# Annatk26/wire

Hardware: AMD Instinct MI355X
Metric: coord-samples/sec fwd+bwd, 4x256 complex WIRE MLP (higher is better)
Workload: dtype f32 (2xfp16 split operands with power-of-two scales, f16 MFMA, fp32 accumulate)

## Files before the change

wire_amd/csrc/wire_api.hip:

```cpp
#include <cmath>
#include <cstdarg>
#include <cstdio>
#include <string>

#include "wire_plan.h"

static thread_local std::string g_err;
int fail(int code, const char* fmt, ...) {
  char buf[512];
  va_list ap;
  va_start(ap, fmt);
  vsnprintf(buf, sizeof buf, fmt, ap);
  va_end(ap);
  g_err = buf;
  return code;
}
int wire_fail_(int code, const char* msg) { return fail(code, "%s", msg); }

extern "C" int wire_abi_version(void) { return WIRE_ABI_VERSION; }
extern "C" const char* wire_last_error(void) { return g_err.c_str(); }

std::mutex g_prof_mu;
std::atomic<bool> g_prof_on{false};
std::vector<ProfRec> g_prof_recs;
// ... 329 lines not shown
  const float* A; float* Sx;
  float* gcur = nullptr; float* gnext = nullptr;
  int chain_rows = 0;

  const float* out_l(int l) const { return A + a.out0 + (int64_t)l * a.np * p.P; }
  const float* lin_l(int l) const { return l == 0 ? A + a.lin0 : A + a.lin1 + (int64_t)(l - 1) * a.np * p.Pl; }
  const float* first(int q) const { return packed + first_native_off(p, q); }
  unsigned* gslots(int l) const { return reinterpret_cast<unsigned*>(Sx + sc.gamax) + l * WIRE_AMAX_SLOTS; }
  const unsigned* oslots(int l) const { return reinterpret_cast<const unsigned*>(A + a.amax) + l * WIRE_AMAX_SLOTS; }
  float* grad(int t) const { return grads ? (float*)grads[t] : nullptr; }
  void done(int t, int count) const { if (ready) ready(user, t, count); }
  int64_t crp_set() const { return (int64_t)prereduce_room(colreduce_blocks(n)) * p.ldu * 5; }
  int final_stage();
  int first_point();
  int chain();
  int wgrad_batch();
  int layers();
  int coords_grad();
  int first_params();
  hipError_t hidden_tn(int l);
};

int Bwd::final_stage() {
  ProfScope ps(s, 3, 0);
  if (!r.fuse) {
    const float wL = (p.L == 0) ? p.w1 : p.w;
    if (p.L == 0 && p.cplx)
      HIPCHK(launch_final_bwd(s, p.kind, 1, g_y, n, p.O, packed + p.off_wf, nullptr, out_l(0), p.K, p.P, wL, p.s, gcur,
                              Sx + sc.fpw, Sx + sc.fpb));
    else
      for (int k = 0; k < p.S2; ++k) {
        const int64_t ro = (int64_t)k * n1, bo = (int64_t)k * final_bwd_blocks(n1);
        HIPCHK(launch_final_bwd(s, p.kind, 0, g_y + ro * p.O, n1, p.O, packed + p.off_wf, lin_l(p.L) + ro * p.Pl,
                                out_l(p.L) + ro * p.P, p.K, p.P, wL, pass_c(p, k), gcur + ro * p.P,
                                Sx + sc.fpw + bo * p.O * p.P, Sx + sc.fpb + bo * p.O,
                                r.fam == FAM_X2 ? gslots(p.L) : nullptr));
      }
    if (!grads) return WIRE_OK;
  }
  const int nbf = r.fused_final ? (int)((n + 127) / 128) : p.S2 * final_bwd_blocks(n1);
  HIPCHK(launch_final_reduce(s, p.kind, Sx + sc.fpw, Sx + sc.fpb, nbf, p.O, p.K, p.P, grad(p.ntens - 2),
                             grad(p.ntens - 1)));
  done(p.ntens - 2, 2);
  return WIRE_OK;
}

int Bwd::first_point() {
  ProfScope ps(s, 3, 0);
  if (p.kind == WIRE_KIND_WIRE)
    HIPCHK(launch_gabor_bwd_first_point(s, gcur, out_l(0), coords, p.D, first(0), first(1), n, p.K, p.P, p.w1, p.s,
                                        Sx + sc.gu, p.ldu));
  else
    HIPCHK(launch_gabor2d_bwd_first_point(s, gcur, out_l(0), coords, p.D, first(0), first(1), first(2), first(3), n, p.K,
                                          p.P, p.w1, p.s, Sx + sc.gu, p.ldu));
  return WIRE_OK;
}

int Bwd::chain() {
  const bool relu = p.kind == WIRE_KIND_RELU;
  FusedBwdParams bp;
  bp.n = n;
  bp.g = Sx + sc.gch; bp.g_stride = sc.gch_stride;
  bp.gamax = gslots(0);
  bp.aux = relu ? A + a.out0 : A + a.lin1 - a.np * p.Pl;
  bp.aux_stride = relu ? a.np * p.P : a.np * p.Pl;
  bp.wimg = reinterpret_cast<const unsigned char*>(packed + p.off_fxd);
  bp.wamax = wamax_of(p, packed, 1); bp.wamax_stride = WIRE_AMAX_SLOTS;
  bp.L = p.L; bp.w = p.w; bp.s = p.s;
  bp.rstore = r.rstore ? 1 : 0; bp.c_hidden = fused_pre_scale(p.kind, p.w, p.s);
  bp.aux0 = relu ? A + a.out0 : A + a.lin0;
  bp.w1 = p.w1;
  if (!p.first_gemm) { bp.coords = coords; bp.D = p.D; bp.crp = Sx + sc.crp; bp.C = p.K; }
  if (p.m2) {
    bp.n = n1;
    for (int k = 0; k < p.S2; ++k) {
      const int64_t ro = (int64_t)k * n1;
      FusedBwdParams b = bp;
      b.g = bp.g + ro * p.P; b.aux = bp.aux + ro * p.P; b.aux0 = bp.aux0 + ro * p.P;
      b.s = pass_c(p, k); b.c_hidden = fused_pre_scale(p.kind, p.w, pass_c(p, k));
      if (k > 0) b.crp = bp.crp + (int64_t)k * ((n1 + chain_rows - 1) / chain_rows) * p.K * 5;
      ProfScope ps(s, 1, 2.0 * n1 * p.Pl * p.P * p.L);
      HIPCHK(launch_fused_bwd(s, p.kind, p.P, b, &chain_rows));
    }
    return WIRE_OK;
  }
  ProfScope ps(s, 1, 2.0 * n * p.Pl * p.P * p.L);
  HIPCHK(launch_fused_bwd(s, p.kind, p.P, bp, &chain_rows));
  return WIRE_OK;
}

static int rstore_zmode(int kind) { return kind == WIRE_KIND_SIREN ? 2 : kind == WIRE_KIND_GAUSS ? 3 : 4; }

int Bwd::wgrad_batch() {
  const int l0 = r.wb_l0, nb = r.wb_n;
  const bool rs = r.rstore;
  const float s_z = rs ? 0.f : r.out_scale[l0 - 1];
  ProfScope ps(s, 2, 2.0 * n * p.Pl * p.P * nb);
  HIPCHK(launch_gemmx2_tn(s, Sx + sc.gch + l0 * sc.gch_stride, p.Pl, rs ? lin_l(l0 - 1) : out_l(l0 - 1), rs ? p.Pl : p.P,
                          n, p.Pl, p.P, r.wb_S, Sx + sc.slab, Sx + sc.bslab, gslots(l0), oslots(l0 - 1),
                          rs ? 1.f / 16384.f : (s_z != 0.f ? 1.f / s_z : 0.f), rs ? rstore_zmode(p.kind) : 0,
                          nb, sc.gch_stride, rs ? a.np * p.Pl : a.np * p.P, WIRE_AMAX_SLOTS));
  return WIRE_OK;
}

hipError_t Bwd::hidden_tn(int l) {
  const int S = r.tn_S;
  float* slab = Sx + sc.slab;
  float* bslab = Sx + sc.bslab;
  switch (r.tn_fam) {
    case FAM_3M: return launch_gemm3m_tn(s, gcur, p.P, out_l(l - 1), p.P, n, p.Kp, p.Kp, S, slab, bslab);
    case FAM_X2:
      if (r.rstore)
        return launch_gemmx2_tn(s, gcur, p.Pl, lin_l(l - 1), p.Pl, n, p.Pl, p.P, S, slab, bslab, gslots(l), nullptr,
                                1.f / 16384.f, rstore_zmode(p.kind));
      return launch_gemmx2_tn(s, gcur, p.Pl, out_l(l - 1), p.P, n, p.Pl, p.P, S, slab, bslab, gslots(l), oslots(l - 1),
                              r.out_scale[l - 1] != 0.f ? 1.f / r.out_scale[l - 1] : 0.f);
    case FAM_X3: return launch_gemmx3_tn(s, gcur, p.Pl, out_l(l - 1), p.P, n, p.Pl, p.P, S, slab, bslab);
    default: return launch_gemm_tn(s, gcur, p.Pl, out_l(l - 1), p.P, n, p.Pl, p.P, S, slab, bslab);
  }
}

int Bwd::layers() {
  const int pl = p.per_layer;
  for (int l = p.L; l >= 1; --l) {
    if (r.chain) gcur = Sx + sc.gch + (int64_t)l * sc.gch_stride;
    if (grads) {
      const bool own = l < r.wb_l0;
      if (own) {
        ProfScope ps(s, 2, 2.0 * n * p.Pl * p.P);
        HIPCHK(hidden_tn(l));
      }
      const int S = own ? r.tn_S : r.wb_S;
      const int64_t m = own ? 0 : l - r.wb_l0;
      float* const slab = Sx + sc.slab + m * S * p.Pl * p.P;
      float* const bslab = Sx + sc.bslab + m * S * p.Pl;
      auto g = [&](int q) { return q < pl ? grad(p.t0 + pl * l + q) : nullptr; };
      ProfScope ps(s, 3, 0);
      if (r.tn_fam == FAM_3M)
        HIPCHK(launch_wgrad3m_reduce(s, slab, bslab, S, p.K, p.K, p.Kp, p.Kp, g(0), g(1)));
      else
        HIPCHK(launch_wgrad_reduce(s, p.kind, slab, bslab, S, p.K, p.K, p.Pl, p.P, g(0), g(1), g(2), g(3)));
      done(p.t0 + pl * l, pl);
    }
    if (r.chain) continue;
    const bool first_sums = grads && r.first_sums;
    GemmEpiParams ep;
    ep.scale = p.s; ep.kvalid = p.K; ep.ld1 = p.P; ep.i1 = out_l(l - 1);
    int epi;
    if (l > 1 || !p.cplx) {
      epi = epi_bwd(p.kind);
      ep.omega = (l - 1 == 0) ? p.w1 : p.w;
      ep.i0 = lin_l(l - 1); ep.o0 = gnext; ep.ld0 = p.Pl;
      ep.recompute_out = r.recompute_out && l >= 2;
      if (l == 1 && first_sums) { ep.coords = coords; ep.D = p.D; ep.cr_partial = Sx + sc.crp; ep.cr_C = p.K; }
    } else {
      epi = (p.kind == WIRE_KIND_WIRE) ? EPI_GABOR_BWD_FIRST : EPI_GABOR2D_BWD_FIRST;
      ep.omega = p.w1;
      ep.coords = coords; ep.D = p.D; ep.ldu = p.ldu; ep.o0 = Sx + sc.gu;
      if (first_sums) { ep.cr_partial = Sx + sc.crp; ep.cr_C = p.K; ep.cr_set = crp_set(); }
      ep.recompute_out = r.recompute_out0;
      ep.W0 = first(0); ep.b0 = first(1);
      if (pl == 4) { ep.W0b = first(2); ep.b0b = first(3); }
    }
    if (!p.cplx && l == 1) ep.ld0 = p.P;
    if (l == 1 && g_coords && r.cg_epi) {
      ep.cg_partial = Sx + cl.cgp; ep.D = p.D;
      if (!p.cplx) ep.W0 = first(0);
    }
    for (int k = 0; k < p.S2; ++k) {
      const int64_t ro = (int64_t)k * n1;
      GemmEpiParams e = ep;
      if (k > 0) { e.scale = pass_c(p, k); e.i0 += ro * p.Pl; e.i1 += ro * p.P; e.o0 += ro * e.ld0; }
      ProfScope ps(s, 1, 2.0 * n1 * p.Pl * p.P);
      HIPCHK(layer_nt(s, p, r.fam, packed, l, true, epi, gcur + ro * p.Pl, n1, e, gslots(l), wamax_of(p, packed, l),
                      l >= 2 || r.tn0 == FAM_X2 ? gslots(l - 1) : nullptr));
    }
    float* t = gcur; gcur = gnext; gnext = t;
  }
  return WIRE_OK;
}

int Bwd::coords_grad() {
  if (!g_coords) return WIRE_OK;
  const float* gu = Sx + sc.gu;
  if (r.cg_epi) {
    HIPCHK(launch_coordgrad_reduce(s, Sx + cl.cgp, cl.ntiles, n, p.D, g_coords));
  } else if (p.kind == WIRE_KIND_WIRE) {
    HIPCHK(launch_coordgrad_rows(s, gu, p.ldu, nullptr, first(0), nullptr, p.K, p.D, n, g_coords));
  } else if (p.kind == WIRE_KIND_WIRE2D) {
    HIPCHK(launch_coordgrad_rows(s, gu, 2 * p.ldu, gu + p.ldu, first(0), first(2), p.K, p.D, n, g_coords));
  } else if (p.m2) {
    HIPCHK(launch_coordgrad_rows(s, gcur, p.P, nullptr, first(0), nullptr, p.K, p.D, n, Sx + cl.cgp));
    HIPCHK(launch_m2_sum_passes(s, Sx + cl.cgp, p.S2, n1, p.D, g_coords));
  } else if (!p.first_gemm) {
    HIPCHK(launch_coordgrad_rows(s, gcur, p.P, nullptr, first(0), nullptr, p.K, p.D, n, g_coords));
  } else {
    GemmEpiParams ep;
    ep.o0 = Sx + cl.gpe; ep.ld0 = p.Pin0;
    HIPCHK(layer_nt(s, p, FAM_4M, packed, 0, true, EPI_STORE, gcur, n, ep));
    HIPCHK(launch_posenc_bwd(s, coords, n, p.D, p.F, Sx + cl.gpe, p.Pin0, g_coords));
  }
  return WIRE_OK;
}

int Bwd::first_params() {
  if (!grads) return WIRE_OK;
  float* const crp = Sx + sc.crp;
  if (p.cplx) {
    const float* gu = Sx + sc.gu;
    if (r.first_sums) {
      HIPCHK(launch_colreduce_final(s, p.K, p.D, n, crp, grad(0), grad(1)));
      if (p.kind == WIRE_KIND_WIRE2D) HIPCHK(launch_colreduce_final(s, p.K, p.D, n, crp + crp_set(), grad(2), grad(3)));
    } else if (p.kind == WIRE_KIND_WIRE) {
      HIPCHK(launch_colreduce(s, gu, p.ldu, p.K, coords, p.D, n, crp, grad(0), grad(1)));
    } else {
      HIPCHK(launch_colreduce(s, gu, 2 * p.ldu, p.K, coords, p.D, n, crp, grad(0), grad(1)));
      HIPCHK(launch_colreduce(s, gu + p.ldu, 2 * p.ldu, p.K, coords, p.D, n, crp, grad(2), grad(3)));
    }
  } else if (!p.first_gemm && r.chain) {
    HIPCHK(launch_colreduce_final_blocks(s, p.K, p.D, p.S2 * (int)((n1 + chain_rows - 1) / chain_rows), crp, grad(p.t0),
                                         grad(p.t0 + 1)));
  } else if (!p.first_gemm && r.first_sums) {
    HIPCHK(launch_colreduce_final(s, p.K, p.D, n, crp, grad(0), grad(1)));
  } else if (!p.first_gemm) {
    HIPCHK(launch_colreduce(s, gcur, p.P, p.K, coords, p.D, n, crp, grad(p.t0), grad(p.t0 + 1)));
  } else if (r.tn0 == FAM_X2) {
    const int S = gemmx2_tn_splits(n, p.P, p.Pin0, sc.S);
    HIPCHK(launch_gemmx2_tn(s, gcur, p.P, A + a.pe, p.Pin0, n, p.P, p.Pin0, S, Sx + sc.slab, Sx + sc.bslab, gslots(0),
                            nullptr, 1.f / r.pe_split));
    HIPCHK(launch_wgrad_reduce(s, p.kind, Sx + sc.slab, Sx + sc.bslab, S, p.K, p.Din, p.P, p.Pin0, grad(p.t0),
                               grad(p.t0 + 1), nullptr, nullptr));
  } else {
    const float* g0 = r.chain ? Sx + sc.gch : gcur;
    const bool x3 = r.tn0 == FAM_X3;
    const int S = x3 ? gemmx3_tn_splits(n, p.P, p.Pin0, sc.S) : gemm_tn_splits(n, p.P, p.Pin0, sc.S);
    HIPCHK(x3 ? launch_gemmx3_tn(s, g0, p.P, A + a.pe, p.Pin0, n, p.P, p.Pin0, S, Sx + sc.slab, Sx + sc.bslab)
              : launch_gemm_tn(s, g0, p.P, A + a.pe, p.Pin0, n, p.P, p.Pin0, S, Sx + sc.slab, Sx + sc.bslab));
    HIPCHK(launch_wgrad_reduce(s, p.kind, Sx + sc.slab, Sx + sc.bslab, S, p.K, p.Din, p.P, p.Pin0, grad(p.t0),
                               grad(p.t0 + 1), nullptr, nullptr));
  }
  done(p.t0, p.per_layer);
  if (p.ms) done(0, 2);
  return WIRE_OK;
}
}

static int mlp_bwd_core(void* stream, const Plan& p, const Route& r, const float* packed, const float* coords, int64_t n,
                        const float* g_y, const void* act, int64_t act_bytes, void* scratch, int64_t scratch_bytes,
                        void* const* grads, wire_grad_ready_fn ready = nullptr, void* user = nullptr,
                        float* g_coords = nullptr, bool comb_done = false) {
  if (n <= 0) return fail(WIRE_ERR_ARG, "backward needs n > 0");
  if (!packed || !coords || (!r.fuse && !g_y && !comb_done) || !act || !scratch || (!grads && !g_coords))
    return fail(WIRE_ERR_ARG, "null pointer");
  if (grads)
    for (int i = p.ms ? p.t0 : 0; i < p.ntens; ++i) if (!grads[i]) return fail(WIRE_ERR_ARG, "grads[%d] is null", i);
  if (p.ms && g_coords) return fail(WIRE_ERR_ARG, "no coordinate gradient through the frozen first stage of kind %d",
                                    (int)WIRE_KIND_BSPLINE_MS);
  Bwd c{p, r, (hipStream_t)stream, packed, coords, n * p.S2, n, g_y, grads, g_coords, ready, user, act_layout(p, n, 1),
        scratch_layout(p, n), coord_layout(p, n), (const float*)act, (float*)scratch};
  const int64_t need = g_coords ? c.cl.total : c.sc.total;
  if (act_bytes < c.a.total * 4) return fail(WIRE_ERR_SIZE, "act buffer too small");
  if (scratch_bytes < need * 4) return fail(WIRE_ERR_SIZE, "scratch %lld < %lld bytes",
                                            (long long)scratch_bytes, (long long)need * 4);
  c.gcur = c.Sx + c.sc.ga;
  c.gnext = c.Sx + c.sc.gb;
  if (p.m2) {
    ProfScope ps(c.s, 3, 0);
    float* const part = c.Sx + c.sc.cpart;
    if (!comb_done)
      HIPCHK(launch_m2_comb_bwd(c.s, comb_of(p, packed), p.S2, p.O, c.A + c.a.ytr, n, M2Loss{}, g_y, c.Sx + c.sc.gtr,
                                grads ? part : nullptr, nullptr));
    if (r.chain) c.gcur = c.Sx + c.sc.gch + (int64_t)p.L * c.sc.gch_stride;
    if (grads) {
      HIPCHK(launch_m2_comb_reduce(c.s, part, n, p.S2, p.O,
                                   M2Grads{c.grad(0), c.grad(1), c.grad(2), c.grad(3)}));
      c.done(0, 4);
      for (int k = 0; k < p.S2 && !r.chain; ++k)
        HIPCHK(hipMemcpyAsync(c.Sx + c.sc.crep + (int64_t)k * n * p.D, coords, (size_t)n * p.D * sizeof(float),
                              hipMemcpyDeviceToDevice, c.s));
      if (!r.chain) c.coords = c.Sx + c.sc.crep;
    }
    c.g_y = c.Sx + c.sc.gtr;
  }
  if (r.fam == FAM_X2 && !r.fuse)
    HIPCHK(hipMemsetAsync(c.gslots(0), 0, (size_t)(p.L + 2) * WIRE_AMAX_SLOTS * sizeof(unsigned), c.s));
  int rc = c.final_stage();
  if (!rc && p.L == 0 && p.cplx) rc = c.first_point();
  if (!rc && r.chain) rc = c.chain();
  if (!rc && r.wb_n > 0) rc = c.wgrad_batch();
  if (!rc) rc = c.layers();
  if (rc) return rc;
  ProfScope ps(c.s, 3, 0);
  rc = c.coords_grad();
  return rc ? rc : c.first_params();
}

extern "C" int wire_mlp_bwd(void* stream, const wire_net_desc* d, const float* packed,
                            const float* coords, int64_t n, const float* g_y, const void* act,
                            int64_t act_bytes, void* scratch, int64_t scratch_bytes,
                            void* const* grads) {
  Plan p; if (int rc = make_plan(d, p)) return rc;
  if (!grads) return fail(WIRE_ERR_ARG, "null pointer");
  if (p.hier)
    return hier_bwd_core(stream, p, hier_route(p, n, MODE_AUTOGRAD), packed, coords, n, g_y, act, act_bytes, scratch,
                         scratch_bytes, grads, nullptr, nullptr, nullptr);
  if (p.mfn)
    return mfn_bwd_core(stream, p, mfn_route(p, n, MODE_AUTOGRAD), packed, coords, n, g_y, act, act_bytes, scratch,
                        scratch_bytes, grads, nullptr, nullptr, nullptr);
  return mlp_bwd_core(stream, p, make_route(p, n, MODE_AUTOGRAD), packed, coords, n, g_y, act, act_bytes, scratch,
                      scratch_bytes, grads);
}

extern "C" int wire_mlp_bwd_coords(void* stream, const wire_net_desc* d, const float* packed, const float* coords,
// ... 110 lines not shown
```

wire_amd/csrc/wire_gemm.h:

```cpp
#pragma once
#include <hip/hip_runtime.h>
#include <stdint.h>

#include "wire_knobs.h"

enum WireFamily { FAM_4M = 0, FAM_3M = 1, FAM_X3 = 2, FAM_X2 = 3 };
WireFamily wire_family_(int kind);

enum WireEpi {
  EPI_STORE = 0,
  EPI_GABOR_FWD = 1,
  EPI_GABOR_BWD = 2,
  EPI_GABOR_BWD_FIRST = 3,
  EPI_SIREN_FWD = 4, EPI_GAUSS_FWD = 5, EPI_RELU_FWD = 6,
  EPI_SIREN_BWD = 7, EPI_GAUSS_BWD = 8, EPI_RELU_BWD = 9,
  EPI_GABOR2D_FWD = 10,
  EPI_GABOR2D_BWD = 11,
  EPI_GABOR2D_BWD_FIRST = 12,
  EPI_BSPLINE_FWD = 13,
  EPI_BSPLINE_BWD = 14,
  EPI_MFN_FWD = 15,
  EPI_MFN_BWD = 16,
  EPI_CG = 64
};

constexpr bool epi_real_fwd(int e) {
  return e == EPI_SIREN_FWD || e == EPI_GAUSS_FWD || e == EPI_RELU_FWD || e == EPI_BSPLINE_FWD;
}
constexpr bool epi_real_bwd(int e) {
  return e == EPI_SIREN_BWD || e == EPI_GAUSS_BWD || e == EPI_RELU_BWD || e == EPI_BSPLINE_BWD;
}
constexpr int epi_real_act(int e) {
  return (e == EPI_BSPLINE_FWD || e == EPI_BSPLINE_BWD) ? 3 : epi_real_fwd(e) ? e - EPI_SIREN_FWD : e - EPI_SIREN_BWD;
}

struct GemmEpiParams {
  const float* bias = nullptr;
  float* o0 = nullptr;
  float* o1 = nullptr;
  const float* i0 = nullptr;
  const float* i1 = nullptr;
  int ld0 = 0;
  int ld1 = 0;
  float omega = 0.f, scale = 0.f;
  int kvalid = 0;
  const float* coords = nullptr;
  const float* W0 = nullptr;
  const float* b0 = nullptr;
  const float* W0b = nullptr;
  const float* b0b = nullptr;
  int D = 0;
  int ldu = 0;
  int wide = 0;
  float* cr_partial = nullptr;
  int cr_C = 0;
  int64_t cr_set = 0;
  float* cg_partial = nullptr;
  int recompute_out = 0;
  int stagger = 0, stagger_lo = 0, stagger_hi = 0;
  const unsigned* amax_a = nullptr;
  const unsigned* amax_b = nullptr;
  unsigned* amax_out = nullptr;
  float o1_split = 0.f;
  float a_split_inv = 0.f;
  const float* ftab = nullptr;
#ifdef WIRE_ABLATE
  int ablate = 0;
#endif
};

hipError_t launch_gemm_nt(hipStream_t s, int epi, const float* A, int lda, const float* Bt,
                          int ldb, int64_t M, int Nc, int Kd, const GemmEpiParams& ep);

int gemm_tn_splits(int64_t n, int Pm, int Pn, int max_splits);
hipError_t launch_gemm_tn(hipStream_t s, const float* G, int ldg, const float* Z, int ldz,
                          int64_t n, int Pm, int Pn, int splits, float* slab, float* bslab);

hipError_t launch_gemm3m_nt(hipStream_t s, int epi, const float* A, int lda, const float* B, int ldb,
                            int64_t M, int Kp_out, int Kp_in, const GemmEpiParams& ep);
int gemm3m_tn_splits(int64_t n, int Kp_o, int Kp_i, int max_splits);
hipError_t launch_gemm3m_tn(hipStream_t s, const float* G, int ldg, const float* Z, int ldz, int64_t n,
                            int Kp_o, int Kp_i, int splits, float* slab, float* bslab);

int64_t gemmx3_b_image_floats(int Nc, int Kd);
hipError_t launch_x3_split_b(hipStream_t s, const float* Bt, int ldb, int Nc, int Kd, void* Bx3);
#define X3_SPLIT_MAXB 32
struct X3SplitBatch { const float* src[X3_SPLIT_MAXB]; void* dst[X3_SPLIT_MAXB]; };
hipError_t launch_x3_split_b_batch(hipStream_t s, const X3SplitBatch& sb, int nb, int ldb, int Nc, int Kd);
hipError_t launch_gemmx3_nt(hipStream_t s, int epi, const float* A, int lda, const void* Bx3, int64_t M,
                            int Nc, int Kd, const GemmEpiParams& ep);
bool gemmx3_nt_is_h16(int epi, int64_t M);
int gemmx3_tn_splits(int64_t n, int Pm, int Pn, int max_splits);
int gemmx3_tn_splits_max(int64_t n, int Pm, int Pn, int max_splits);
hipError_t launch_gemmx3_tn(hipStream_t s, const float* G, int ldg, const float* Z, int ldz, int64_t n,
                            int Pm, int Pn, int splits, float* slab, float* bslab);

void gemmx3_register_glds(bool (*handles)(int, int64_t),
                          hipError_t (*launch)(hipStream_t, int, const float*, int, const void*, int64_t, int, int,
                                               const GemmEpiParams&),
                          int (*tune)(const char*, int));
extern int (*g_glds_tune)(const char*, int);
bool gemmx3g_handles(int epi, int64_t M);
int gemmx3g_tune_set(const char* key, int value);
int gemmx3g_mode();
hipError_t launch_gemmx3g_nt(hipStream_t s, int epi, const float* A, int lda, const void* Bx3, int64_t M,
                             int Nc, int Kd, const GemmEpiParams& ep);

bool gemmx3h_handles(int epi, int64_t M);
hipError_t launch_gemmx3h_nt(hipStream_t s, int epi, const float* A, int lda, const void* Bx3, int64_t M,
                             int Nc, int Kd, const GemmEpiParams& ep);

#define X2_AMAX_MAXB 32
struct X2AmaxBatch { const float* src[X2_AMAX_MAXB]; unsigned* slots[X2_AMAX_MAXB]; };
hipError_t launch_amax_batch(hipStream_t s, const X2AmaxBatch& ab, int nb, int64_t count);
hipError_t launch_amax(hipStream_t s, const float* src, int64_t count, unsigned* slots);
int64_t gemmx2_b_image_floats(int Nc, int Kd);
#define X2_SPLIT_MAXB 32
struct X2SplitBatch { const float* src[X2_SPLIT_MAXB]; void* dst[X2_SPLIT_MAXB]; const unsigned* slots[X2_SPLIT_MAXB]; };
hipError_t launch_x2_split_b_batch(hipStream_t s, const X2SplitBatch& sb, int nb, int ldb, int Nc, int Kd);
hipError_t launch_gemmx2h_nt(hipStream_t s, int epi, const float* A, int lda, const void* Bx2, int64_t M, int Nc,
                             int Kd, const GemmEpiParams& ep);
bool gemmx2_tn_applies(int Pm, int Pn);
int gemmx2_tn_splits(int64_t n, int Pm, int Pn, int max_splits);
hipError_t launch_gemmx2_tn(hipStream_t s, const float* G, int ldg, const float* Z, int ldz, int64_t n, int Pm,
                            int Pn, int splits, float* slab, float* bslab, const unsigned* amax_g,
                            const unsigned* amax_z, float z_pre_inv = 0.f, int z_act = 0, int batch = 1,
                            long long g_step = 0, long long z_step = 0, int amax_step = 0);
int gemmx2_tn_batch_splits(int64_t n, int Pm, int Pn, int max_splits, int batch);

#define FX_SPLIT_MAXB 32
struct FxSplitBatch { const float* src[FX_SPLIT_MAXB]; void* dst[FX_SPLIT_MAXB]; const unsigned* slots[FX_SPLIT_MAXB]; };
int64_t fused_b_image_floats(int P);
hipError_t launch_fx_split_b_batch(hipStream_t s, const FxSplitBatch& sb, int nb, int ldb, int P, float c, int Kd = 0);
struct FusedFwdParams {
  const float* coords = nullptr; long long n = 0;
  const float* W0 = nullptr; const float* b0 = nullptr;
  const unsigned char* wimg = nullptr;
  const float* bias = nullptr; long long bias_stride = 0;
  const unsigned* wamax = nullptr; int wamax_stride = 0;
  const float* wf = nullptr; const float* bfr = nullptr;
  float* y = nullptr;
  int D = 0, K = 0, L = 0, O = 0;
  float w1 = 0.f, w = 0.f, s = 0.f;
  float c_first = 1.f, c_hidden = 1.f, k2_first = 0.f, k2 = 0.f;
  float* lin0 = nullptr;
  float* lin = nullptr; long long lin_stride = 0;
  float* out = nullptr; long long out_stride = 0;
  unsigned* amax_out = nullptr;
  float inv_c_first = 1.f, inv_c_hidden = 1.f;
  int pe_F = 0; const float* bias0 = nullptr; const unsigned* wamax0 = nullptr;
  int rstore = 0;
  const float* target = nullptr; const int64_t* idx = nullptr; long long first = 0; float gscale = 0.f;
  float* rec = nullptr;
  float* g_lin = nullptr;
  float* part_w = nullptr; float* part_b = nullptr;
  float* loss_partial = nullptr;
  unsigned* amax_g = nullptr;
};
float fused_pre_scale(int kind, float omega0, float scale0);
bool fused_fwd_shape(int kind, int P);
hipError_t launch_fused_fwd(hipStream_t s, int kind, int P, const FusedFwdParams& fp);

struct FusedBwdParams {
  long long n = 0;
  float* g = nullptr; long long g_stride = 0;
  unsigned* gamax = nullptr;
  const float* aux = nullptr; long long aux_stride = 0;
  const float* aux0 = nullptr;
  const unsigned char* wimg = nullptr;
  const unsigned* wamax = nullptr; int wamax_stride = 0;
  int L = 0;
  float w = 0.f, s = 0.f;
  int rstore = 0; float c_hidden = 1.f;
  float w1 = 0.f;
  const float* coords = nullptr; int D = 0;
  float* crp = nullptr; int C = 0;
};
bool fused_bwd_shape(int kind, int P);
hipError_t launch_fused_bwd(hipStream_t s, int kind, int P, const FusedBwdParams& fp, int* tile_rows);
```

wire_amd/csrc/wire_gemmh_epi.h:

```cpp
#pragma once
#include "wire_dev.h"
#include "wire_gemm.h"

WIRE_DEVINL void h_pair_rows(const f32x4& X, const f32x4& Y, f32x4& Xp, f32x4& Yp) {
#pragma unroll
  for (int q = 0; q < 4; ++q) {
    const int x = __float_as_int(X[q]), y = __float_as_int(Y[q]);
    Xp[q] = __int_as_float(__builtin_amdgcn_update_dpp(x, y, 0x128, 0xf, 0xc, false));
    Yp[q] = __int_as_float(__builtin_amdgcn_update_dpp(y, x, 0x128, 0xf, 0x3, false));
  }
}

WIRE_DEVINL void h_amax4(float& m, const f32x4& v) {
  m = __builtin_fmaxf(m, __builtin_fmaxf(__builtin_fmaxf(__builtin_fabsf(v[0]), __builtin_fabsf(v[1])),
                                         __builtin_fmaxf(__builtin_fabsf(v[2]), __builtin_fabsf(v[3]))));
}

WIRE_DEVINL void h_cg_add(float (&cg)[4], const float (&t)[4], const int e, const int lane) {
#pragma unroll
  for (int d = 0; d < 4; ++d) {
    float v = t[d];
    v += __shfl_xor(v, 8); v += __shfl_xor(v, 16); v += __shfl_xor(v, 32);
    cg[d] += (lane >> 3) == e ? v : 0.f;
  }
}
template <int NRB>
WIRE_DEVINL void h_cg_store(const float (&cg)[4], const GemmEpiParams& ep, const int M, const int m_w, const int n_w,
                            const int lane) {
  const int j = lane >> 3;
  if (j >= 2 * NRB) return;
  const int row = m_w + 16 * (j >> 1) + 8 * (j & 1) + (lane & 7);
  if (row >= M) return;
  float* dst = ep.cg_partial + ((size_t)(n_w >> 7) * (size_t)M + (size_t)row) * ep.D;
  for (int d = 0; d < ep.D; ++d) dst[d] = cg[d];
}

template <int EPIX, bool X2 = false, int NRB = 4>
WIRE_DEVINL void h_epilogue(f32x4 (&acc)[NRB][8], const GemmEpiParams& ep, const int M, const int m_w, const int n_w,
                            const int Nc, const int lane, unsigned char* lds, const int wave, const int rt,
                            const float acc_scale = 1.f) {
  constexpr int EPI = EPIX & ~EPI_CG;
  constexpr bool CG = (EPIX & EPI_CG) != 0;
  const int rr = lane & 7, ch = (lane >> 3) & 1, g = lane >> 4;
  float amx = 0.f;
  if constexpr (X2) {
#pragma unroll
    for (int i = 0; i < NRB; ++i)
#pragma unroll
      for (int j = 0; j < 8; ++j)
#pragma unroll
        for (int q = 0; q < 4; ++q) acc[i][j][q] *= acc_scale;
  }
  const int cq = 16 * ch + 4 * g;
  if constexpr (EPI == EPI_STORE) {
#pragma unroll
    for (int sp = 0; sp < 4; ++sp) {
      const int col = n_w + 32 * sp + cq;
      if (n_w + 32 * sp >= Nc) continue;
#pragma unroll
      for (int rb = 0; rb < NRB; ++rb) {
        f32x4 xp, yp;
        h_pair_rows(acc[rb][2 * sp], acc[rb][2 * sp + 1], xp, yp);
        const int row = m_w + 16 * rb + rr;
        if (row < M) *reinterpret_cast<f32x4*>(ep.o0 + (size_t)row * ep.ld0 + col) = xp;
        if (row + 8 < M) *reinterpret_cast<f32x4*>(ep.o0 + (size_t)(row + 8) * ep.ld0 + col) = yp;
      }
    }
  } else if constexpr (epi_real_fwd(EPI)) {
    constexpr int ACT = epi_real_act(EPI);
#pragma unroll
    for (int sp = 0; sp < 4; ++sp) {
      if (n_w + 32 * sp >= Nc) continue;
      const int col = n_w + 32 * sp + cq;
      const f32x4 bv = *reinterpret_cast<const f32x4*>(ep.bias + col);
#pragma unroll
      for (int rb = 0; rb < NRB; ++rb) {
        f32x4 a2[2];
        h_pair_rows(acc[rb][2 * sp], acc[rb][2 * sp + 1], a2[0], a2[1]);
#pragma unroll
        for (int hr = 0; hr < 2; ++hr) {
          const int row = m_w + 16 * rb + 8 * hr + rr;
          f32x4 lin;
#pragma unroll
          for (int q = 0; q < 4; ++q) lin[q] = a2[hr][q] + bv[q];
          if (ep.o0 && row < M) *reinterpret_cast<f32x4*>(ep.o0 + (size_t)row * ep.ld0 + col) = lin;
          if (ep.o1) {
            f32x4 o;
#pragma unroll
            for (int q = 0; q < 4; ++q) {
              const float v = real_act_fwd_lean<ACT>(lin[q], ep.omega, ep.scale);
              o[q] = col + q < ep.kvalid ? v : 0.f;
            }
            if constexpr (X2) h_amax4(amx, o);
            if (row < M) wire_store_out4(ep.o1 + (size_t)row * ep.ld1 + col, o, X2 ? ep.o1_split : 0.f);
          }
        }
      }
    }
  } else if constexpr (epi_real_bwd(EPI)) {
    constexpr int ACT = epi_real_act(EPI);
    float cg[4] = {0.f, 0.f, 0.f, 0.f};
#pragma unroll
    for (int sp = 0; sp < 4; ++sp) {
      if (n_w + 32 * sp >= Nc) continue;
      const int col = n_w + 32 * sp + cq;
      float crs[4][5];
#pragma unroll
      for (int q = 0; q < 4; ++q)
#pragma unroll
        for (int d = 0; d < 5; ++d) crs[q][d] = 0.f;
#pragma unroll
      for (int rp = 0; rp < NRB; rp += 2) {
        f32x4 lv[4], ov[4], a2[4];
#pragma unroll
        for (int r2 = 0; r2 < 2; ++r2) {
          h_pair_rows(acc[rp + r2][2 * sp], acc[rp + r2][2 * sp + 1], a2[2 * r2], a2[2 * r2 + 1]);
#pragma unroll
          for (int hr = 0; hr < 2; ++hr) {
            int row = m_w + 16 * (rp + r2) + 8 * hr + rr;
            row = row < M ? row : M - 1;
            lv[2 * r2 + hr] = (ACT != ACT_RELU) ? *reinterpret_cast<const f32x4*>(ep.i0 + (size_t)row * ep.ld0 + col)
                                                : f32x4{0.f, 0.f, 0.f, 0.f};
            const bool load_out = ACT == ACT_RELU || (ACT == ACT_GAUSS && !ep.recompute_out);
            ov[2 * r2 + hr] = load_out ? *reinterpret_cast<const f32x4*>(ep.i1 + (size_t)row * ep.ld1 + col)
                                       : f32x4{0.f, 0.f, 0.f, 0.f};
          }
        }
        if (ACT == ACT_GAUSS && ep.recompute_out) {
#pragma unroll
          for (int e = 0; e < 4; ++e)
#pragma unroll
            for (int q = 0; q < 4; ++q) {
              const float v = real_act_fwd_lean<ACT>(lv[e][q], ep.omega, ep.scale);
              ov[e][q] = col + q < ep.kvalid ? v : 0.f;
            }
        }
#pragma unroll
        for (int e = 0; e < 4; ++e) {
          const int row = m_w + 16 * (rp + (e >> 1)) + 8 * (e & 1) + rr;
          f32x4 gl;
#pragma unroll
          for (int q = 0; q < 4; ++q) gl[q] = real_act_bwd_lean<ACT>(a2[e][q], lv[e][q], ov[e][q], ep.omega, ep.scale);
          if constexpr (X2) h_amax4(amx, gl);
          if constexpr (CG) {
            float t[4] = {0.f, 0.f, 0.f, 0.f};
            if (row < M) {
#pragma unroll
              for (int q = 0; q < 4; ++q) {
                if (col + q >= ep.kvalid) continue;
                for (int d = 0; d < ep.D; ++d) t[d] = __builtin_fmaf(gl[q], ep.W0[(col + q) * ep.D + d], t[d]);
              }
            }
            h_cg_add(cg, t, 2 * (rp + (e >> 1)) + (e & 1), lane);
          }
          if (row < M) {
            if (ep.cr_partial) {
              float x[4] = {0.f, 0.f, 0.f, 0.f};
              for (int d = 0; d < ep.D; ++d) x[d] = ep.coords[(size_t)row * ep.D + d];
#pragma unroll
              for (int q = 0; q < 4; ++q) {
#pragma unroll
                for (int d = 0; d < 4; ++d) crs[q][d] = __builtin_fmaf(gl[q], x[d], crs[q][d]);
                crs[q][4] += gl[q];
              }
            } else {
              *reinterpret_cast<f32x4*>(ep.o0 + (size_t)row * ep.ld0 + col) = gl;
            }
          }
        }
      }
      if (ep.cr_partial) {
        float* red = reinterpret_cast<float*>(lds);
#pragma unroll
        for (int q = 0; q < 4; ++q)
#pragma unroll
          for (int d = 0; d < 5; ++d) {
            float v = crs[q][d];
            v += __shfl_xor(v, 1); v += __shfl_xor(v, 2); v += __shfl_xor(v, 4);
            if (rr == 0) red[(wave * 128 + 32 * sp + cq + q) * 5 + d] = v;
          }
      }
    }
    if (ep.cr_partial) {
      __syncthreads();
      const float* red = reinterpret_cast<const float*>(lds);
      for (int e = threadIdx.x; e < 128 * 5; e += 256) {
        const int c = e / 5, d = e - 5 * c;
        const float v = (red[e] + red[128 * 5 + e]) + (red[2 * 128 * 5 + e] + red[3 * 128 * 5 + e]);
        if (n_w + c < ep.cr_C) ep.cr_partial[((size_t)rt * ep.cr_C + n_w + c) * 5 + d] = v;
      }
    }
    if constexpr (CG) h_cg_store<NRB>(cg, ep, M, m_w, n_w, lane);
  } else if constexpr (EPI == EPI_MFN_FWD || EPI == EPI_MFN_BWD) {
#pragma unroll 1
    for (int sp = 0; sp < 4; ++sp) {
      if (n_w + 32 * sp >= Nc) continue;
      const int col = n_w + 32 * sp + cq;
      const bool filt = EPI == EPI_MFN_FWD || ep.i0 != nullptr;
      MfnCol fc[4];
      f32x4 bv = {0.f, 0.f, 0.f, 0.f};
      if (filt) {
#pragma unroll
        for (int q = 0; q < 4; ++q) fc[q] = mfn_load(ep.ftab, col + q);
      }
      if constexpr (EPI == EPI_MFN_FWD) bv = *reinterpret_cast<const f32x4*>(ep.bias + col);
#pragma unroll
      for (int rb = 0; rb < NRB; ++rb) {
        f32x4 a2[2];
        f32x4 ax = acc[rb][0], ay = acc[rb][1];
        if (sp == 1) { ax = acc[rb][2]; ay = acc[rb][3]; }
        if (sp == 2) { ax = acc[rb][4]; ay = acc[rb][5]; }
        if (sp == 3) { ax = acc[rb][6]; ay = acc[rb][7]; }
        h_pair_rows(ax, ay, a2[0], a2[1]);
#pragma unroll
        for (int hr = 0; hr < 2; ++hr) {
          const int row = m_w + 16 * rb + 8 * hr + rr;
          const int rowc = row < M ? row : M - 1;
          float x[4] = {0.f, 0.f, 0.f, 0.f};
          f32x4 g = {0.f, 0.f, 0.f, 0.f};
          if (filt) {
            mfn_load_x(ep.coords, rowc, ep.D, x);
#pragma unroll
            for (int q = 0; q < 4; ++q) g[q] = mfn_g(fc[q], x);
          }
          if constexpr (EPI == EPI_MFN_FWD) {
            f32x4 lin, o;
#pragma unroll
            for (int q = 0; q < 4; ++q) {
              lin[q] = a2[hr][q] + bv[q];
              o[q] = col + q < ep.kvalid ? lin[q] * g[q] : 0.f;
            }
            if constexpr (X2) h_amax4(amx, o);
            if (row < M) {
              if (ep.o0) *reinterpret_cast<f32x4*>(ep.o0 + (size_t)row * ep.ld0 + col) = lin;
              *reinterpret_cast<f32x4*>(ep.o1 + (size_t)row * ep.ld1 + col) = o;
            }
          } else {
            if (filt) {
              const f32x4 lin = *reinterpret_cast<const f32x4*>(ep.i0 + (size_t)rowc * ep.ld0 + col);
              f32x4 gl, hh;
#pragma unroll
              for (int q = 0; q < 4; ++q) { gl[q] = a2[hr][q] * g[q]; hh[q] = a2[hr][q] * lin[q]; }
              if constexpr (X2) h_amax4(amx, gl);
              if (row < M) {
                *reinterpret_cast<f32x4*>(ep.o0 + (size_t)row * ep.ld0 + col) = gl;
                *reinterpret_cast<f32x4*>(ep.o1 + (size_t)row * ep.ld1 + col) = hh;
              }
            } else if (row < M) {
              *reinterpret_cast<f32x4*>(ep.o1 + (size_t)row * ep.ld1 + col) = a2[hr];
            }
          }
        }
      }
    }
  } else if constexpr (EPI == EPI_GABOR2D_FWD) {
    const int grp = n_w >> 7;
    const int f0 = (grp << 5) + cq;
    const int oc = (grp << 6) + cq;
    f32x4 bv[4];
#pragma unroll
    for (int k = 0; k < 4; ++k) bv[k] = *reinterpret_cast<const f32x4*>(ep.bias + n_w + 32 * k + cq);
#pragma unroll
    for (int rb = 0; rb < NRB; ++rb) {
      f32x4 part[4][2];
#pragma unroll
      for (int k = 0; k < 4; ++k) h_pair_rows(acc[rb][2 * k], acc[rb][2 * k + 1], part[k][0], part[k][1]);
#pragma unroll
      for (int hr = 0; hr < 2; ++hr) {
        const int row = m_w + 16 * rb + 8 * hr + rr;
        f32x4 u, v, pp, qq;
#pragma unroll
        for (int q = 0; q < 4; ++q) {
          u[q] = part[0][hr][q] + bv[0][q];
          v[q] = part[1][hr][q] + bv[1][q];
          pp[q] = part[2][hr][q] + bv[2][q];
          qq[q] = part[3][hr][q] + bv[3][q];
        }
        if (ep.o0 && row < M) {
          float* Lp = ep.o0 + (size_t)row * ep.ld0 + n_w + cq;
          *reinterpret_cast<f32x4*>(Lp) = u;
          *reinterpret_cast<f32x4*>(Lp + 32) = v;
          *reinterpret_cast<f32x4*>(Lp + 64) = pp;
          *reinterpret_cast<f32x4*>(Lp + 96) = qq;
        }
        if (ep.o1) {
          f32x4 o_re, o_im;
#pragma unroll
          for (int q = 0; q < 4; ++q) {
            float a, b;
            gabor2d_fwd_lean(u[q], v[q], pp[q], qq[q], ep.omega, ep.scale, a, b);
            const bool valid = f0 + q < ep.kvalid;
            o_re[q] = valid ? a : 0.f;
            o_im[q] = valid ? b : 0.f;
          }
          if constexpr (X2) { h_amax4(amx, o_re); h_amax4(amx, o_im); }
          if (row < M) {
            float* Op = ep.o1 + (size_t)row * ep.ld1 + oc;
            wire_store_out4(Op, o_re, X2 ? ep.o1_split : 0.f);
            wire_store_out4(Op + 32, o_im, X2 ? ep.o1_split : 0.f);
          }
        }
      }
    }
  } else if constexpr (EPI == EPI_GABOR2D_BWD || EPI == EPI_GABOR2D_BWD_FIRST) {
    const float m2s2 = -2.f * ep.scale * ep.scale, w0 = ep.omega;
    float cg[4] = {0.f, 0.f, 0.f, 0.f};
#pragma unroll
    for (int G = 0; G < 2; ++G) {
      if (n_w + 64 * G >= Nc) continue;
      const int c0 = n_w + 64 * G + cq;
      const int grp = c0 >> 6;
      const int f0 = (grp << 5) + (c0 & 31);
      const int lc = (grp << 7) + (c0 & 31);
      float w[4][4], wv[4][4], bb[4], bv2[4];
      float cru[4][5], crp2[4][5];
#pragma unroll
      for (int q = 0; q < 4; ++q)
#pragma unroll
        for (int d = 0; d < 5; ++d) { cru[q][d] = 0.f; crp2[q][d] = 0.f; }
      if constexpr (EPI == EPI_GABOR2D_BWD_FIRST) {
#pragma unroll
        for (int q = 0; q < 4; ++q) {
          const bool valid = f0 + q < ep.kvalid;
          bb[q] = valid ? ep.b0[f0 + q] : 0.f;
          bv2[q] = valid ? ep.b0b[f0 + q] : 0.f;
#pragma unroll
          for (int d = 0; d < 4; ++d) {
            w[q][d] = (valid && d < ep.D) ? ep.W0[(f0 + q) * ep.D + d] : 0.f;
            wv[q][d] = (valid && d < ep.D) ? ep.W0b[(f0 + q) * ep.D + d] : 0.f;
          }
        }
      }
#pragma unroll
      for (int rb = 0; rb < NRB; ++rb) {
        f32x4 are[2], aim[2];
        h_pair_rows(acc[rb][4 * G], acc[rb][4 * G + 1], are[0], are[1]);
        h_pair_rows(acc[rb][4 * G + 2], acc[rb][4 * G + 3], aim[0], aim[1]);
        f32x4 u[2], v[2], pp[2], qq[2], pr[2], pi[2];
        float xs[2][4];
#pragma unroll
        for (int hr = 0; hr < 2; ++hr) {
          int row = m_w + 16 * rb + 8 * hr + rr;
          row = row < M ? row : M - 1;
          const bool recompute = EPI == EPI_GABOR2D_BWD && ep.recompute_out != 0;
          if (!recompute) {
            const float* Op = ep.i1 + (size_t)row * ep.ld1 + c0;
            pr[hr] = *reinterpret_cast<const f32x4*>(Op);
            pi[hr] = *reinterpret_cast<const f32x4*>(Op + 32);
          }
          if constexpr (EPI == EPI_GABOR2D_BWD) {
            const float* Lp = ep.i0 + (size_t)row * ep.ld0 + lc;
            u[hr] = *reinterpret_cast<const f32x4*>(Lp);
            v[hr] = *reinterpret_cast<const f32x4*>(Lp + 32);
            pp[hr] = *reinterpret_cast<const f32x4*>(Lp + 64);
            qq[hr] = *reinterpret_cast<const f32x4*>(Lp + 96);
            if (recompute) {
#pragma unroll
              for (int q = 0; q < 4; ++q) {
                float a, b;
                gabor2d_fwd_lean(u[hr][q], v[hr][q], pp[hr][q], qq[hr][q], ep.omega, ep.scale, a, b);
                const bool valid = f0 + q < ep.kvalid;
                pr[hr][q] = valid ? a : 0.f;
                pi[hr][q] = valid ? b : 0.f;
              }
            }
          } else {
            float x[4] = {0.f, 0.f, 0.f, 0.f};
            for (int d = 0; d < ep.D; ++d) x[d] = ep.coords[(size_t)row * ep.D + d];
#pragma unroll
            for (int d = 0; d < 4; ++d) xs[hr][d] = x[d];
#pragma unroll
            for (int q = 0; q < 4; ++q) {
              float uu = bb[q], p2 = bv2[q];
#pragma unroll
              for (int d = 0; d < 4; ++d) { uu = __builtin_fmaf(x[d], w[q][d], uu); p2 = __builtin_fmaf(x[d], wv[q][d], p2); }
              u[hr][q] = uu; pp[hr][q] = p2; v[hr][q] = 0.f; qq[hr][q] = 0.f;
            }
          }
        }
#pragma unroll
        for (int hr = 0; hr < 2; ++hr) {
          const int row = m_w + 16 * rb + 8 * hr + rr;
          f32x4 g0, g1, g2, g3;
#pragma unroll
          for (int q = 0; q < 4; ++q) {
            const float gr = are[hr][q], gi = aim[hr][q];
            const float c_r = __builtin_fmaf(pr[hr][q], gr, pi[hr][q] * gi);
            const float c_i = __builtin_fmaf(pr[hr][q], gi, -(pi[hr][q] * gr));
            const float tt = m2s2 * c_r;
            g0[q] = __builtin_fmaf(tt, u[hr][q], w0 * c_i);
            g1[q] = __builtin_fmaf(tt, v[hr][q], -(w0 * c_r));
            g2[q] = tt * pp[hr][q];
            g3[q] = tt * qq[hr][q];
          }
          if constexpr (X2 && EPI == EPI_GABOR2D_BWD) { h_amax4(amx, g0); h_amax4(amx, g1); h_amax4(amx, g2); h_amax4(amx, g3); }
          if constexpr (EPI == EPI_GABOR2D_BWD_FIRST) {
            if constexpr (CG) {
              float t[4] = {0.f, 0.f, 0.f, 0.f};
              if (row < M) {
#pragma unroll
                for (int q = 0; q < 4; ++q)
#pragma unroll
                  for (int d = 0; d < 4; ++d) t[d] = __builtin_fmaf(g2[q], wv[q][d], __builtin_fmaf(g0[q], w[q][d], t[d]));
              }
              h_cg_add(cg, t, 2 * rb + hr, lane);
            }
          }
          if (row < M) {
            if constexpr (EPI == EPI_GABOR2D_BWD) {
              float* Gp = ep.o0 + (size_t)row * ep.ld0 + lc;
              *reinterpret_cast<f32x4*>(Gp) = g0;
              *reinterpret_cast<f32x4*>(Gp + 32) = g1;
              *reinterpret_cast<f32x4*>(Gp + 64) = g2;
              *reinterpret_cast<f32x4*>(Gp + 96) = g3;
            } else {
#pragma unroll
              for (int q = 0; q < 4; ++q)
                if (!(f0 + q < ep.kvalid)) { g0[q] = 0.f; g2[q] = 0.f; }
              if (ep.cr_partial) {
#pragma unroll
                for (int q = 0; q < 4; ++q) {
#pragma unroll
                  for (int d = 0; d < 4; ++d) {
                    cru[q][d] = __builtin_fmaf(g0[q], xs[hr][d], cru[q][d]);
                    crp2[q][d] = __builtin_fmaf(g2[q], xs[hr][d], crp2[q][d]);
                  }
                  cru[q][4] += g0[q];
                  crp2[q][4] += g2[q];
                }
              } else {
                float* Gp = ep.o0 + (size_t)row * (2 * ep.ldu);
                *reinterpret_cast<f32x4*>(Gp + f0) = g0;
                *reinterpret_cast<f32x4*>(Gp + ep.ldu + f0) = g2;
              }
            }
          }
        }
      }
      if constexpr (EPI == EPI_GABOR2D_BWD_FIRST) {
        if (ep.cr_partial) {
          float* red = reinterpret_cast<float*>(lds);
#pragma unroll
          for (int q = 0; q < 4; ++q)
#pragma unroll
            for (int d = 0; d < 5; ++d) {
              float a = cru[q][d], b = crp2[q][d];
              a += __shfl_xor(a, 1); a += __shfl_xor(a, 2); a += __shfl_xor(a, 4);
              b += __shfl_xor(b, 1); b += __shfl_xor(b, 2); b += __shfl_xor(b, 4);
              if (rr == 0) {
                red[(wave * 64 + 32 * G + cq + q) * 5 + d] = a;
                red[4 * 64 * 5 + (wave * 64 + 32 * G + cq + q) * 5 + d] = b;
              }
            }
        }
      }
    }
// ... 224 lines not shown
```

wire_amd/csrc/wire_gemmx2h.hip:

```cpp
#include <cstdlib>
#include <atomic>
#include <cstring>

#include "wire_dev.h"
#include "wire_gemm.h"
#include "wire_gemmh_epi.h"

typedef _Float16 f16x8 __attribute__((ext_vector_type(8)));
typedef _Float16 f16x2 __attribute__((ext_vector_type(2)));
typedef unsigned x2u32x4 __attribute__((ext_vector_type(4)));
typedef unsigned x2u32x2 __attribute__((ext_vector_type(2)));

#define X2_BK 32
#define X2_TBM 256
#define X2_TBN 128
#define X2_AWAVE (64 * 128)
#define X2_ABYTES (4 * X2_AWAVE)
#define X2_BPLANE (X2_TBN * 64)
#define X2_BSTAGE (2 * X2_BPLANE)

#define X2_MFMA(a, b, c) c = __builtin_amdgcn_mfma_f32_16x16x32_f16(a, b, c, 0, 0, 0)

WIRE_DEVINL void x2_dma16(const void* gsrc, unsigned char* lds_piece) {
#ifdef WIRE_X2_DMA_BUILTIN
// ... 188 lines not shown
        x2_split2(ar[rb][0][0], ar[rb][0][1], s_a, H[0], L[0]);
        x2_split2(ar[rb][0][2], ar[rb][0][3], s_a, H[1], L[1]);
        x2_split2(ar[rb][1][0], ar[rb][1][1], s_a, H[2], L[2]);
        x2_split2(ar[rb][1][2], ar[rb][1][3], s_a, H[3], L[3]);
        ah[rb] = __builtin_bit_cast(f16x8, x2u32x4{H[0], H[1], H[2], H[3]});
        al[rb] = __builtin_bit_cast(f16x8, x2u32x4{L[0], L[1], L[2], L[3]});
      }
      __builtin_amdgcn_sched_barrier(0);
      const bool more = kt + 2 < nk;
      if (more) { issue(kt + 2, (kt + 2) % 3); aload_to(ar, kt + 2); }
      __builtin_amdgcn_sched_barrier(0);
      const unsigned char* S = smem + b_rd + (kt % 3) * X2_BSTAGE;
#pragma unroll
      for (int hb = 0; hb < 2; ++hb) {
        if (hb == 1 && half_tile) break;
        f16x8 bh[4], bl[4];
#pragma unroll
        for (int cq = 0; cq < 4; ++cq) {
          bh[cq] = *reinterpret_cast<const f16x8*>(S + (4 * hb + cq) * 1024);
          bl[cq] = *reinterpret_cast<const f16x8*>(S + X2_BPLANE + (4 * hb + cq) * 1024);
        }
#pragma unroll
        for (int rb = 0; rb < NRB; ++rb)
#pragma unroll
          for (int cq = 0; cq < 4; ++cq) {
            X2_MFMA(bl[cq], ah[rb], acc[rb][4 * hb + cq]);
            X2_MFMA(bh[cq], al[rb], acc[rb][4 * hb + cq]);
            X2_MFMA(bh[cq], ah[rb], acc[rb][4 * hb + cq]);
          }
      }
      __builtin_amdgcn_sched_barrier(0);
      if (more) asm volatile("s_waitcnt vmcnt(8)" ::: "memory");
      else asm volatile("s_waitcnt vmcnt(0)" ::: "memory");
      __builtin_amdgcn_s_barrier();
      __builtin_amdgcn_sched_barrier(0);
    };
    static_assert(2 * NRB + 4 == 8, "the in-flight count of the end-of-stage wait");
    issue(0, 0); aload_to(araw, 0);
    issue(1, 1); aload_to(ar1, 1);
    asm volatile("s_waitcnt vmcnt(8)" ::: "memory");
    __builtin_amdgcn_s_barrier();
    for (int kt = 0; kt < nk; kt += 2) {
      half_stage(araw, kt);
      half_stage(ar1, kt + 1);
    }
    h_epilogue<EPI, true, NRB>(acc, ep, M, m_base + wave * (16 * NRB), n_base, Nc, lane, smem, wave, rt, inv_a * inv_b);
    return;
  }

  issue(0, 0);
  if constexpr (BRING) { if (nk > 1) issue(1, 1); }
  if constexpr (AMODE == 1) aload(0);
  asm volatile("s_waitcnt vmcnt(0)" ::: "memory");
  __builtin_amdgcn_s_barrier();

  int buf = 0;
  for (int kt = 0; kt < nk; ++kt) {
    if constexpr (AMODE == 0 || AMODE == 2) {
#pragma unroll
      for (int rb = 0; rb < NRB; ++rb) {
        if constexpr (AMODE == 2) {
          araw[rb][0] = *reinterpret_cast<const f32x4*>(smem + a2_rd0 + rb * 2048);
          araw[rb][1] = *reinterpret_cast<const f32x4*>(smem + a2_rd1 + rb * 2048);
        } else {
          araw[rb][0] = *reinterpret_cast<const f32x4*>(smem + a_rd + rb * 2048);
          araw[rb][1] = *reinterpret_cast<const f32x4*>(smem + a_rd + rb * 2048 + 256);
        }
      }
      asm volatile("s_waitcnt lgkmcnt(0)" ::: "memory");
      __builtin_amdgcn_sched_barrier(0);
      if (kt + 1 < nk) issue(kt + 1, buf ^ 1);
      __builtin_amdgcn_sched_barrier(0);
    }
    f16x8 ah[NRB], al[NRB];
#pragma unroll
    for (int rb = 0; rb < NRB; ++rb) {
      if constexpr (APRE) {
        const x2u32x4 u0 = __builtin_bit_cast(x2u32x4, araw[rb][0]), u1 = __builtin_bit_cast(x2u32x4, araw[rb][1]);
        ah[rb] = __builtin_bit_cast(f16x8, x2u32x4{u0[0], u0[1], u1[0], u1[1]});
        al[rb] = __builtin_bit_cast(f16x8, x2u32x4{u0[2], u0[3], u1[2], u1[3]});
      } else {
        unsigned H[4], L[4];
        x2_split2(araw[rb][0][0], araw[rb][0][1], s_a, H[0], L[0]);
        x2_split2(araw[rb][0][2], araw[rb][0][3], s_a, H[1], L[1]);
        x2_split2(araw[rb][1][0], araw[rb][1][1], s_a, H[2], L[2]);
        x2_split2(araw[rb][1][2], araw[rb][1][3], s_a, H[3], L[3]);
        ah[rb] = __builtin_bit_cast(f16x8, x2u32x4{H[0], H[1], H[2], H[3]});
        al[rb] = __builtin_bit_cast(f16x8, x2u32x4{L[0], L[1], L[2], L[3]});
      }
    }
    if constexpr (AMODE == 1) {
      __builtin_amdgcn_sched_barrier(0);
      if constexpr (BRING) {
        if (kt + 1 < nk) aload(kt + 1);
        __builtin_amdgcn_sched_barrier(0);
        if (kt + 2 < nk) issue(kt + 2, buf == 0 ? 2 : buf - 1);
      } else
      if (kt + 1 < nk) { issue(kt + 1, buf ^ 1); aload(kt + 1); }
      __builtin_amdgcn_sched_barrier(0);
    }
    const unsigned char* S = smem + b_rd + buf * X2_BSTAGE;
#pragma unroll
    for (int hb = 0; hb < 2; ++hb) {
      if (hb == 1 && half_tile) break;
      f16x8 bh[4], bl[4];
#pragma unroll
      for (int cq = 0; cq < 4; ++cq) {
        bh[cq] = *reinterpret_cast<const f16x8*>(S + (4 * hb + cq) * 1024);
        bl[cq] = *reinterpret_cast<const f16x8*>(S + X2_BPLANE + (4 * hb + cq) * 1024);
      }
#pragma unroll
      for (int rb = 0; rb < NRB; ++rb)
#pragma unroll
        for (int cq = 0; cq < 4; ++cq) {
          X2_MFMA(bl[cq], ah[rb], acc[rb][4 * hb + cq]);
          X2_MFMA(bh[cq], al[rb], acc[rb][4 * hb + cq]);
          X2_MFMA(bh[cq], ah[rb], acc[rb][4 * hb + cq]);
        }
    }
    __builtin_amdgcn_sched_barrier(0);
    {
    if (BRING && kt + 2 < nk) asm volatile("s_waitcnt vmcnt(4)" ::: "memory");
    else asm volatile("s_waitcnt vmcnt(0)" ::: "memory");
    __builtin_amdgcn_s_barrier();
    }
    __builtin_amdgcn_sched_barrier(0);
    if constexpr (BRING) buf = buf == 2 ? 0 : buf + 1; else buf ^= 1;
  }
  h_epilogue<EPI, true, NRB>(acc, ep, M, m_base + wave * (16 * NRB), n_base, Nc, lane, smem, wave, rt, inv_a * inv_b);
}

template <int EPI>
static hipError_t launchx2h_t(hipStream_t s, const float* A, int lda, const unsigned short* Bx2, int64_t M, int Nc,
                              int Kd, const GemmEpiParams& ep) {
  const int tbm = X2_TBM;
  const int tiles_m = (int)((M + tbm - 1) / tbm);
  const int tiles_n = (Nc + X2_TBN - 1) / X2_TBN;
  const int tiles_m_pad = (tiles_m + 7) & ~7;
  const dim3 grid((unsigned)(tiles_m_pad * tiles_n));
  if (ep.a_split_inv != 0.f) {
    if constexpr (EPI == EPI_STORE || EPI == EPI_GABOR_FWD || EPI == EPI_GABOR2D_FWD || EPI == EPI_SIREN_FWD ||
                  EPI == EPI_GAUSS_FWD || EPI == EPI_BSPLINE_FWD) {
      if (knob(K_X2_AMODE) == 2)
        hipLaunchKernelGGL((gemmx2h_nt_kernel<EPI, 2, 4, 1, true>), grid, dim3(256), 0, s, A, lda, Bx2, (int)M, Nc, Kd, tiles_m,
                           tiles_n, ep);
      else
        hipLaunchKernelGGL((gemmx2h_nt_kernel<EPI, 1, 4, 1, true>), grid, dim3(256), 0, s, A, lda, Bx2, (int)M, Nc, Kd, tiles_m,
                           tiles_n, ep);
      return hipGetLastError();
    } else {
      return hipErrorInvalidValue;
    }
  }
  if (knob(K_X2_AMODE) == 2)
    hipLaunchKernelGGL((gemmx2h_nt_kernel<EPI, 2, 4>), grid, dim3(256), 0, s, A, lda, Bx2, (int)M, Nc, Kd, tiles_m, tiles_n, ep);
  else if (knob(K_X2_AMODE) == 1)
    hipLaunchKernelGGL((gemmx2h_nt_kernel<EPI, 1, 4>), grid, dim3(256), 0, s, A, lda, Bx2, (int)M, Nc, Kd, tiles_m, tiles_n, ep);
  else
    hipLaunchKernelGGL((gemmx2h_nt_kernel<EPI, 0, 4>), grid, dim3(256), 0, s, A, lda, Bx2, (int)M, Nc, Kd, tiles_m, tiles_n, ep);
  return hipGetLastError();
}

hipError_t launch_gemmx2h_nt(hipStream_t s, int epi, const float* A, int lda, const void* Bx2v, int64_t M, int Nc,
                             int Kd, const GemmEpiParams& ep) {
  if (M <= 0) return hipSuccess;
  if ((Nc & 63) || (Kd & 31) || (lda & 3) || M > 0x7fffff00LL || (!ep.amax_a && ep.a_split_inv == 0.f) || !ep.amax_b)
    return hipErrorInvalidValue;
  if ((int64_t)lda * 4 * X2_TBM > 0x7fffffffLL) return hipErrorInvalidValue;
  const unsigned short* Bx2 = (const unsigned short*)Bx2v;
  switch (epi) {
    case EPI_STORE: return launchx2h_t<EPI_STORE>(s, A, lda, Bx2, M, Nc, Kd, ep);
    case EPI_GABOR_FWD: return launchx2h_t<EPI_GABOR_FWD>(s, A, lda, Bx2, M, Nc, Kd, ep);
    case EPI_GABOR_BWD: return launchx2h_t<EPI_GABOR_BWD>(s, A, lda, Bx2, M, Nc, Kd, ep);
    case EPI_GABOR_BWD_FIRST:
      return ep.cg_partial ? launchx2h_t<EPI_GABOR_BWD_FIRST | EPI_CG>(s, A, lda, Bx2, M, Nc, Kd, ep)
                           : launchx2h_t<EPI_GABOR_BWD_FIRST>(s, A, lda, Bx2, M, Nc, Kd, ep);
    case EPI_SIREN_FWD: return launchx2h_t<EPI_SIREN_FWD>(s, A, lda, Bx2, M, Nc, Kd, ep);
    case EPI_GAUSS_FWD: return launchx2h_t<EPI_GAUSS_FWD>(s, A, lda, Bx2, M, Nc, Kd, ep);
    case EPI_RELU_FWD: return launchx2h_t<EPI_RELU_FWD>(s, A, lda, Bx2, M, Nc, Kd, ep);
    case EPI_SIREN_BWD:
      return ep.cg_partial ? launchx2h_t<EPI_SIREN_BWD | EPI_CG>(s, A, lda, Bx2, M, Nc, Kd, ep)
                           : launchx2h_t<EPI_SIREN_BWD>(s, A, lda, Bx2, M, Nc, Kd, ep);
    case EPI_GAUSS_BWD:
      return ep.cg_partial ? launchx2h_t<EPI_GAUSS_BWD | EPI_CG>(s, A, lda, Bx2, M, Nc, Kd, ep)
                           : launchx2h_t<EPI_GAUSS_BWD>(s, A, lda, Bx2, M, Nc, Kd, ep);
    case EPI_RELU_BWD:
      return ep.cg_partial ? launchx2h_t<EPI_RELU_BWD | EPI_CG>(s, A, lda, Bx2, M, Nc, Kd, ep)
                           : launchx2h_t<EPI_RELU_BWD>(s, A, lda, Bx2, M, Nc, Kd, ep);
    case EPI_BSPLINE_FWD: return launchx2h_t<EPI_BSPLINE_FWD>(s, A, lda, Bx2, M, Nc, Kd, ep);
    case EPI_BSPLINE_BWD:
      return ep.cg_partial ? launchx2h_t<EPI_BSPLINE_BWD | EPI_CG>(s, A, lda, Bx2, M, Nc, Kd, ep)
                           : launchx2h_t<EPI_BSPLINE_BWD>(s, A, lda, Bx2, M, Nc, Kd, ep);
    case EPI_MFN_FWD: return launchx2h_t<EPI_MFN_FWD>(s, A, lda, Bx2, M, Nc, Kd, ep);
    case EPI_MFN_BWD: return launchx2h_t<EPI_MFN_BWD>(s, A, lda, Bx2, M, Nc, Kd, ep);
    case EPI_GABOR2D_FWD:
      if (Nc & 127) return hipErrorInvalidValue;
      return launchx2h_t<EPI_GABOR2D_FWD>(s, A, lda, Bx2, M, Nc, Kd, ep);
    case EPI_GABOR2D_BWD: return launchx2h_t<EPI_GABOR2D_BWD>(s, A, lda, Bx2, M, Nc, Kd, ep);
    case EPI_GABOR2D_BWD_FIRST:
      return ep.cg_partial ? launchx2h_t<EPI_GABOR2D_BWD_FIRST | EPI_CG>(s, A, lda, Bx2, M, Nc, Kd, ep)
                           : launchx2h_t<EPI_GABOR2D_BWD_FIRST>(s, A, lda, Bx2, M, Nc, Kd, ep);
    default: return hipErrorInvalidValue;
  }
}

typedef short x2s16x4 __attribute__((ext_vector_type(4)));
#define X2T_TK 32

WIRE_DEVINL x2s16x4 x2_lds_tr16(const unsigned char* p) {
  return __builtin_amdgcn_ds_read_tr16_b64_v4i16(
      (x2s16x4 __attribute__((address_space(3)))*)(const_cast<unsigned char*>(p)));
}

template <int WM, int WN, int ZMODE, int RB = 4>
__global__ __launch_bounds__(64 * WM * WN, 2) void gemmx2_tn16_kernel(
    const float* __restrict__ G, int ldg, const float* __restrict__ Z, int ldz, long long n, int Pm, int Pn,
    int tiles_n, int nsplit, long long chunk, float* __restrict__ slab, float* __restrict__ bslab, int tiles,
    const unsigned* __restrict__ amax_g, const unsigned* __restrict__ amax_z, const float z_pre_inv,
    const long long g_step, const long long z_step, const int amax_step) {
  {
    const int by = blockIdx.y;
    G += (size_t)by * g_step; Z += (size_t)by * z_step;
    slab += (size_t)by * nsplit * Pm * Pn;
    if (bslab) bslab += (size_t)by * nsplit * Pm;
    amax_g += by * amax_step;
    if (amax_z) amax_z += by * amax_step;
  }
  constexpr int NW = WM * WN;
  constexpr int TM = 16 * RB * WM, TN = 128 * WN;
  constexpr bool G3 = RB == 3;
  static_assert(RB == 4 || (RB == 3 && WM == 8 && WN == 1), "wave tiles: 64 x 128, or 48 x 128 in the 8-wave P = 384 shape");
  constexpr int GPLANE = X2T_TK * TM * 2, ZPLANE = X2T_TK * TN * 2;
  constexpr int STAGE = 2 * GPLANE + 2 * ZPLANE;
  constexpr int UG = TM / 8, UZ = 16 * WN;
  constexpr int IG = (UG + NW - 1) / NW, IZ = (UZ + NW - 1) / NW;
  constexpr int PG = TM / 32, PZ = TN / 32;
  extern __shared__ __attribute__((aligned(16))) unsigned char smem_t[];
  const int tid = threadIdx.x;
  const int lane = tid & 63, wave = tid >> 6;
  const int wave_m = wave / WN, wave_n = wave % WN;
  const int bb = blockIdx.x;
  const int xcd = bb & 7, idx = bb >> 3;
  const int tile = idx % tiles;
  const int split = (idx / tiles) * 8 + xcd;
  if (split >= nsplit) return;
  const int tm = tile / tiles_n, tn = tile % tiles_n;
  const int m_base = tm * TM, n_base = tn * TN;
  const long long row0 = (long long)split * chunk;
  long long row1 = row0 + chunk;
  if (row1 > n) row1 = n;
  if (row1 <= row0) return;

  float s_g, inv_g, s_z, inv_z;
  wire_x2_scales(wire_amax_read(amax_g, lane), s_g, inv_g);
  constexpr bool ZPRE = ZMODE == 1;
  if constexpr (ZMODE >= 1) { s_z = 1.f / z_pre_inv; inv_z = z_pre_inv; }
  else wire_x2_scales(wire_amax_read(amax_z, lane), s_z, inv_z);

  const int l_hb = lane >> 5, l_rs = (lane >> 2) & 7, l_p = lane & 3;
  const int l_row0 = (l_rs & 3) + 8 * (l_rs >> 2);
  auto pass_row = [](const int t) { return 16 * (t & 1) + 4 * (t >> 1); };
  const int l_feat = 16 * l_hb + 4 * l_p;
  const int l_st = l_hb * 1024 + l_rs * 32 + l_p * 8;
  const bool do_bias = (bslab != nullptr) && (tn == 0);
  const bool z_edge = WN == 1 && n_base + TN > Pn;

  f32x4 acc[RB][8];
#pragma unroll
  for (int i = 0; i < RB; ++i)
#pragma unroll
    for (int j = 0; j < 8; ++j) acc[i][j] = f32x4{0.f, 0.f, 0.f, 0.f};
  static_assert(G3 || (PG % NW == 0 && IG == 4 * (PG / NW)), "the block pairs of G must deal out evenly to the waves");
  static_assert(!G3 || (PG == 12 && IG == 6), "8 waves x 6 units = 12 block pairs x 4 passes");
  static_assert(PZ == NW || PZ == 4, "Z units: one block pair per wave, or 4 block pairs dealt round-robin");
  constexpr int NB = G3 ? 3 : PG / NW;
  const int hiw = wave >= 4 ? 1 : 0;
  const int g3_pb = hiw ? wave - 4 : wave + 8;
  auto g3_pair = [&](const int i) { return (i % 3) == 0 ? wave : ((i % 3) == 1 ? g3_pb : wave + 4); };
  auto g3_row = [&](const int i) { return (i % 3) == 1 ? 16 * hiw + (i >= 3 ? 4 : 0) : (i == 0 ? 0 : i == 2 ? 16 : i == 3 ? 4 : 20); };
  auto g3_pass = [&](const int i) { return (i % 3) == 1 ? hiw + (i >= 3 ? 2 : 0) : (i == 0 ? 0 : i == 2 ? 1 : i == 3 ? 2 : 3); };
  constexpr bool ZFIX = (PZ == NW);
  f32x4 bsum[NB];
#pragma unroll
  for (int i = 0; i < NB; ++i) bsum[i] = f32x4{0.f, 0.f, 0.f, 0.f};

  const int nrows = (int)(row1 - row0);
  const int nk = (nrows + X2T_TK - 1) / X2T_TK;
  const int nk_full = nrows / X2T_TK;
  const f32x4 zero4 = {0.f, 0.f, 0.f, 0.f};

  struct Staged { f32x4 g[IG], z[IZ]; };
  Staged st;
  const unsigned g_off = (unsigned)l_row0 * (unsigned)ldg + (unsigned)(m_base + l_feat);
  const unsigned z_off = (unsigned)l_row0 * (unsigned)ldz + (unsigned)(n_base + l_feat);
  const float* const g_base = G + (size_t)row0 * ldg;
  const float* const z_base = Z + (size_t)row0 * ldz;
  auto gload = [&](Staged& R, int kt, const bool tail) {
    int ks = tail ? nk_full : (kt < nk_full ? kt : nk_full - 1);
    ks = ks < 0 ? 0 : ks;
    const float* gb = g_base + (size_t)ks * (X2T_TK * (size_t)ldg);
    const float* zb = z_base + (size_t)ks * (X2T_TK * (size_t)ldz);
    const int rbase = ks * X2T_TK + l_row0;
#pragma unroll
    for (int i = 0; i < IG; ++i) {
      if constexpr (G3) {
        const int fp = g3_pair(i), pr = g3_row(i);
        const bool ok = !tail || rbase + pr < nrows;
        R.g[i] = ok ? *reinterpret_cast<const f32x4*>(gb + (size_t)pr * ldg + 32 * fp + g_off) : zero4;
      } else {
        const int fp = wave + NW * (i % NB), t = i / NB;
        const bool ok = !tail || rbase + pass_row(t) < nrows;
        R.g[i] = ok ? *reinterpret_cast<const f32x4*>(gb + (size_t)pass_row(t) * ldg + 32 * fp + g_off) : zero4;
      }
    }
#pragma unroll
    for (int i = 0; i < IZ; ++i) {
      const int u = wave + NW * i;
      if (ZFIX || u < UZ) {
        const int fp = ZFIX ? wave : (u & 3), t = ZFIX ? i : (u >> 2);
        bool ok = !tail || rbase + pass_row(t) < nrows;
        if (z_edge) ok = ok && (n_base + 32 * fp + l_feat < Pn);
        R.z[i] = ok ? *reinterpret_cast<const f32x4*>(zb + (size_t)pass_row(t) * ldz + 32 * fp + z_off) : zero4;
      }
    }
  };
  auto lstore = [&](const Staged& R, int buf) {
    unsigned char* S = smem_t + buf * STAGE + l_st;
#pragma unroll
    for (int i = 0; i < IG; ++i) {
      const int fp = G3 ? g3_pair(i) : wave + NW * (i % NB), t = G3 ? g3_pass(i) : i / NB;
      const f32x4 gv = R.g[i];
      unsigned h0, l0, h1, l1;
      x2_split2(gv[0], gv[1], s_g, h0, l0);
      x2_split2(gv[2], gv[3], s_g, h1, l1);
      unsigned char* d = S + fp * 2048 + t * 256;
      *reinterpret_cast<x2u32x2*>(d) = x2u32x2{h0, h1};
      *reinterpret_cast<x2u32x2*>(d + GPLANE) = x2u32x2{l0, l1};
      if (do_bias) { bsum[i % NB][0] += gv[0]; bsum[i % NB][1] += gv[1]; bsum[i % NB][2] += gv[2]; bsum[i % NB][3] += gv[3]; }
    }
#pragma unroll
    for (int i = 0; i < IZ; ++i) {
      const int u = wave + NW * i;
      if (ZFIX || u < UZ) {
        const int fp = ZFIX ? wave : (u & 3), t = ZFIX ? i : (u >> 2);
        const f32x4 zv = R.z[i];
        unsigned h0, l0, h1, l1;
        if constexpr (ZPRE) {
          const x2u32x4 zu = __builtin_bit_cast(x2u32x4, zv);
          h0 = zu[0]; h1 = zu[1]; l0 = zu[2]; l1 = zu[3];
        } else {
          f32x4 zz = zv;
          if constexpr (ZMODE == 2) {
#pragma unroll
            for (int e = 0; e < 4; ++e) zz[e] = __builtin_amdgcn_sinf(__builtin_amdgcn_fractf(zv[e]));
// ... 229 lines not shown
```

wire_amd/csrc/wire_gemmx3h.hip:

```cpp
#include <cstdlib>
#include <atomic>
#include <cstring>

#include "wire_dev.h"
#include "wire_gemm.h"
#include "wire_gemmh_epi.h"

typedef __bf16 hbf16x8 __attribute__((ext_vector_type(8)));
typedef __bf16 hbf16x2 __attribute__((ext_vector_type(2)));
typedef unsigned hu32x4 __attribute__((ext_vector_type(4)));

#define H_BK 16
#define H_TBM 256
#define H_TBN 128
#define H_ABYTES (H_TBM * 64)
#define H_BPLANE (H_TBN * 32)
#define H_STAGE (H_ABYTES + 3 * H_BPLANE)
#define H_PPW 7

WIRE_DEVINL unsigned h_cvt_pk_bf16(float a, float b) {
  const hbf16x2 v = {(__bf16)a, (__bf16)b};
  return __builtin_bit_cast(unsigned, v);
}
WIRE_DEVINL float h_bf16_lo(unsigned packed) {
// ... 13 lines not shown
  a = r[0];
  b = r[1];
}
WIRE_DEVINL int h_gray(int x) { return x ^ (x >> 1); }

#define H_MFMA(a, b, c) c = __builtin_amdgcn_mfma_f32_16x16x32_bf16(a, b, c, 0, 0, 0)

WIRE_DEVINL void h_dma16(const void* gsrc, unsigned char* lds_piece) {
  __builtin_amdgcn_global_load_lds((const __attribute__((address_space(1))) void*)gsrc,
                                   (__attribute__((address_space(3))) void*)lds_piece, 16, 0, 0);
}

template <int EPI>
__global__ __launch_bounds__(256, 2) void gemmx3h_nt_kernel(const float* __restrict__ A, int lda,
                                                            const unsigned short* __restrict__ Bu, int M, int Nc,
                                                            int Kd, int tiles_m, int tiles_n, GemmEpiParams ep) {
  __shared__ __attribute__((aligned(1024))) unsigned char smem[2 * H_STAGE];
  const int tid = threadIdx.x;
  const int lane = tid & 63, wave = __builtin_amdgcn_readfirstlane(tid >> 6);
  const int up = lane >> 5, r16 = lane & 15, kc = (lane >> 4) & 1;

  const int b = blockIdx.x;
  const int xcd = b & 7, idx = b >> 3;
  const int ct = idx % tiles_n;
  const int rt = (idx / tiles_n) * 8 + xcd;
  if (rt >= tiles_m) return;
  const int m_base = rt * H_TBM, n_base = ct * H_TBN;
  const int nk = Kd / H_BK;
  if (ep.stagger > 0 && b >= ep.stagger_lo && b < ep.stagger_hi) {
    const unsigned long long t0 = __builtin_amdgcn_s_memrealtime();
    while (__builtin_amdgcn_s_memrealtime() - t0 < (unsigned long long)ep.stagger) __builtin_amdgcn_s_sleep(32);
  }

  const char* src[H_PPW];
  int adv[H_PPW], loff[H_PPW];
#pragma unroll
  for (int j = 0; j < H_PPW; ++j) {
    const int q = wave + 4 * j;
    if (q < 16) {
      const int r = 16 * q + (lane >> 2);
      const int c = (lane & 3) ^ h_gray((r >> 2) & 3);
      int row = m_base + r;
      row = row < M ? row : M - 1;
      src[j] = reinterpret_cast<const char*>(A + (size_t)row * lda + c * 4);
      adv[j] = H_BK * 4;
      loff[j] = q * 1024;
    } else {
      const int bq = q - 16;
      const int p = bq >> 2, cb = bq & 3;
      src[j] = reinterpret_cast<const char*>(Bu + ((size_t)ct * nk * 3 + p) * (128 * 16) + cb * (32 * 16) + lane * 8);
      adv[j] = 3 * 128 * 16 * 2;
      loff[j] = H_ABYTES + p * H_BPLANE + cb * 1024;
    }
  }
  auto issue = [&](int kt, int buf) {
    unsigned char* S = smem + buf * H_STAGE;
#pragma unroll
    for (int j = 0; j < H_PPW; ++j) h_dma16(src[j] + (size_t)kt * adv[j], S + loff[j]);
  };

  f32x4 acc[4][8];
#pragma unroll
  for (int i = 0; i < 4; ++i)
#pragma unroll
    for (int j = 0; j < 8; ++j) acc[i][j] = f32x4{0.f, 0.f, 0.f, 0.f};

  int a_rd[2][2];
#pragma unroll
  for (int p = 0; p < 2; ++p) {
    const int rr = wave * 64 + p * 32 + up * 16 + r16;
    const int sw = h_gray((rr >> 2) & 3);
    a_rd[p][0] = rr * 64 + (((2 * kc) ^ sw) << 4);
    a_rd[p][1] = rr * 64 + (((2 * kc + 1) ^ sw) << 4);
  }
  const int b_col = H_ABYTES + r16 * 32 + kc * 16;
  const int b_g1 = b_col + (up ? 0 : 2 * H_BPLANE);
  const int b_g2 = b_col + H_BPLANE;
  const int b_g3 = b_col;

  issue(0, 0);
  asm volatile("s_waitcnt vmcnt(0)" ::: "memory");
  __builtin_amdgcn_s_barrier();

  int buf = 0;
  for (int kt = 0; kt < nk; ++kt) {
    const unsigned char* S = smem + buf * H_STAGE;
    f32x4 araw[2][2];
#pragma unroll
    for (int p = 0; p < 2; ++p) {
      araw[p][0] = *reinterpret_cast<const f32x4*>(S + a_rd[p][0]);
      araw[p][1] = *reinterpret_cast<const f32x4*>(S + a_rd[p][1]);
    }
    __builtin_amdgcn_sched_barrier(0);
    if (kt + 1 < nk) issue(kt + 1, buf ^ 1);
    __builtin_amdgcn_sched_barrier(0);
    hbf16x8 f1[4], f2[4];
#pragma unroll
    for (int p = 0; p < 2; ++p) {
      unsigned H[4], Mi[4], L[4], H2[4];
      h_split2(araw[p][0][0], araw[p][0][1], H[0], Mi[0], L[0]);
      h_split2(araw[p][0][2], araw[p][0][3], H[1], Mi[1], L[1]);
      h_split2(araw[p][1][0], araw[p][1][1], H[2], Mi[2], L[2]);
      h_split2(araw[p][1][2], araw[p][1][3], H[3], Mi[3], L[3]);
#pragma unroll
      for (int e = 0; e < 4; ++e) {
        H2[e] = H[e];
        h_swap_halves(H[e], L[e]);
        h_swap_halves(Mi[e], H2[e]);
      }
      f1[2 * p] = __builtin_bit_cast(hbf16x8, hu32x4{H[0], H[1], H[2], H[3]});
      f1[2 * p + 1] = __builtin_bit_cast(hbf16x8, hu32x4{L[0], L[1], L[2], L[3]});
      f2[2 * p] = __builtin_bit_cast(hbf16x8, hu32x4{Mi[0], Mi[1], Mi[2], Mi[3]});
      f2[2 * p + 1] = __builtin_bit_cast(hbf16x8, hu32x4{H2[0], H2[1], H2[2], H2[3]});
    }
#pragma unroll
    for (int hb = 0; hb < 2; ++hb) {
      hbf16x8 g1[4], g2[4], g3[4];
#pragma unroll
      for (int cq = 0; cq < 4; ++cq) {
        const int cb = 4 * hb + cq;
        g1[cq] = *reinterpret_cast<const hbf16x8*>(S + b_g1 + cb * 512);
        g2[cq] = *reinterpret_cast<const hbf16x8*>(S + b_g2 + cb * 512);
        g3[cq] = *reinterpret_cast<const hbf16x8*>(S + b_g3 + cb * 512);
      }
#pragma unroll
      for (int rb = 0; rb < 4; ++rb)
#pragma unroll
        for (int cq = 0; cq < 4; ++cq) {
          H_MFMA(g1[cq], f1[rb], acc[rb][4 * hb + cq]);
          H_MFMA(g2[cq], f2[rb], acc[rb][4 * hb + cq]);
          H_MFMA(g3[cq], f2[rb], acc[rb][4 * hb + cq]);
        }
    }
    __builtin_amdgcn_sched_barrier(0);
    asm volatile("s_waitcnt vmcnt(0)" ::: "memory");
    __builtin_amdgcn_s_barrier();
    __builtin_amdgcn_sched_barrier(0);
    buf ^= 1;
  }
  h_epilogue<EPI, true>(acc, ep, M, m_base + wave * 64, n_base, Nc, lane, smem, wave, rt, 1.f);
}

template <int EPI>
static hipError_t launchx3h_t(hipStream_t s, const float* A, int lda, const unsigned short* Bu, int64_t M, int Nc,
                              int Kd, const GemmEpiParams& ep) {
  const int tiles_m = (int)((M + H_TBM - 1) / H_TBM);
  const int tiles_n = (Nc + H_TBN - 1) / H_TBN;
  const int tiles_m_pad = (tiles_m + 7) & ~7;
  hipLaunchKernelGGL((gemmx3h_nt_kernel<EPI>), dim3((unsigned)(tiles_m_pad * tiles_n)), dim3(256), 0, s, A, lda, Bu,
                     (int)M, Nc, Kd, tiles_m, tiles_n, ep);
  return hipGetLastError();
}

bool gemmx3h_handles(int epi, int64_t M) {
  const int h16 = knob(K_X3_H16);
  if (!h16 || M < 4096) return false;
  if (epi == EPI_STORE || epi == EPI_GABOR_FWD) return (h16 & 1) != 0;
  if (epi == EPI_GABOR_BWD || epi == EPI_GABOR_BWD_FIRST) return (h16 & 2) != 0;
  if (epi_real_fwd(epi) || epi_real_bwd(epi) || epi == EPI_MFN_FWD || epi == EPI_MFN_BWD) return (h16 & 4) != 0;
  if (epi >= EPI_GABOR2D_FWD && epi <= EPI_GABOR2D_BWD_FIRST) return (h16 & 8) != 0;
  return false;
}

hipError_t launch_gemmx3h_nt(hipStream_t s, int epi, const float* A, int lda, const void* Bx3, int64_t M, int Nc,
                             int Kd, const GemmEpiParams& ep_in) {
  if (M <= 0) return hipSuccess;
  if ((Nc & 63) || (Kd & 31) || (lda & 3) || M > 0x7fffff00LL) return hipErrorInvalidValue;
  GemmEpiParams ep = ep_in;
  ep.stagger = knob(K_X3H_STAGGER); ep.stagger_lo = 256; ep.stagger_hi = 512;
  const unsigned short* Bu = (const unsigned short*)Bx3 + (size_t)gemmx3_b_image_floats(Nc, Kd);
  switch (epi) {
    case EPI_STORE: return launchx3h_t<EPI_STORE>(s, A, lda, Bu, M, Nc, Kd, ep);
    case EPI_GABOR_FWD: return launchx3h_t<EPI_GABOR_FWD>(s, A, lda, Bu, M, Nc, Kd, ep);
    case EPI_GABOR_BWD: return launchx3h_t<EPI_GABOR_BWD>(s, A, lda, Bu, M, Nc, Kd, ep);
    case EPI_GABOR_BWD_FIRST:
      return ep.cg_partial ? launchx3h_t<EPI_GABOR_BWD_FIRST | EPI_CG>(s, A, lda, Bu, M, Nc, Kd, ep)
                           : launchx3h_t<EPI_GABOR_BWD_FIRST>(s, A, lda, Bu, M, Nc, Kd, ep);
    case EPI_SIREN_FWD: return launchx3h_t<EPI_SIREN_FWD>(s, A, lda, Bu, M, Nc, Kd, ep);
    case EPI_GAUSS_FWD: return launchx3h_t<EPI_GAUSS_FWD>(s, A, lda, Bu, M, Nc, Kd, ep);
    case EPI_RELU_FWD: return launchx3h_t<EPI_RELU_FWD>(s, A, lda, Bu, M, Nc, Kd, ep);
    case EPI_SIREN_BWD:
      return ep.cg_partial ? launchx3h_t<EPI_SIREN_BWD | EPI_CG>(s, A, lda, Bu, M, Nc, Kd, ep)
                           : launchx3h_t<EPI_SIREN_BWD>(s, A, lda, Bu, M, Nc, Kd, ep);
    case EPI_GAUSS_BWD:
      return ep.cg_partial ? launchx3h_t<EPI_GAUSS_BWD | EPI_CG>(s, A, lda, Bu, M, Nc, Kd, ep)
                           : launchx3h_t<EPI_GAUSS_BWD>(s, A, lda, Bu, M, Nc, Kd, ep);
    case EPI_RELU_BWD:
      return ep.cg_partial ? launchx3h_t<EPI_RELU_BWD | EPI_CG>(s, A, lda, Bu, M, Nc, Kd, ep)
                           : launchx3h_t<EPI_RELU_BWD>(s, A, lda, Bu, M, Nc, Kd, ep);
    case EPI_BSPLINE_FWD: return launchx3h_t<EPI_BSPLINE_FWD>(s, A, lda, Bu, M, Nc, Kd, ep);
    case EPI_BSPLINE_BWD:
      return ep.cg_partial ? launchx3h_t<EPI_BSPLINE_BWD | EPI_CG>(s, A, lda, Bu, M, Nc, Kd, ep)
                           : launchx3h_t<EPI_BSPLINE_BWD>(s, A, lda, Bu, M, Nc, Kd, ep);
    case EPI_MFN_FWD: return launchx3h_t<EPI_MFN_FWD>(s, A, lda, Bu, M, Nc, Kd, ep);
    case EPI_MFN_BWD: return launchx3h_t<EPI_MFN_BWD>(s, A, lda, Bu, M, Nc, Kd, ep);
    case EPI_GABOR2D_FWD:
      if (Nc & 127) return hipErrorInvalidValue;
      return launchx3h_t<EPI_GABOR2D_FWD>(s, A, lda, Bu, M, Nc, Kd, ep);
    case EPI_GABOR2D_BWD: return launchx3h_t<EPI_GABOR2D_BWD>(s, A, lda, Bu, M, Nc, Kd, ep);
    case EPI_GABOR2D_BWD_FIRST:
      return ep.cg_partial ? launchx3h_t<EPI_GABOR2D_BWD_FIRST | EPI_CG>(s, A, lda, Bu, M, Nc, Kd, ep)
                           : launchx3h_t<EPI_GABOR2D_BWD_FIRST>(s, A, lda, Bu, M, Nc, Kd, ep);
    default: return hipErrorInvalidValue;
  }
}
```

wire_amd/csrc/wire_hier_api.hip:

```cpp
#include "wire_plan.h"

static inline int hier_sets(const Plan& p) { return p.HS * (p.HL + 2); }
HierAct hier_act(const Plan& p, int64_t n, int save) {
  HierAct a;
  const int S = p.HS, per = p.HL + 2;
  const int64_t nP = n * p.P;
  int64_t off = 0;
  a.amax = off; off += (int64_t)hier_sets(p) * WIRE_AMAX_SLOTS;
  a.lin.resize(S); a.out.resize(S); a.cat.assign(S, -1);
  int64_t tmp[2] = {-1, -1}, catb[2] = {-1, -1};
  if (!save) {
    tmp[0] = off; off += nP; tmp[1] = off; off += nP;
    if (S > 1) { catb[0] = off; off += 2 * nP; catb[1] = off; off += 2 * nP; }
  }
  for (int st = 1; st < S; ++st) {
    if (save) { a.cat[st] = off; off += 2 * nP; } else a.cat[st] = catb[st & 1];
  }
  for (int st = 0; st < S; ++st) {
    const int last = hier_last(p, st);
    a.lin[st].assign(last + 1, -1);
    a.out[st].resize(last + 1);
    for (int l = 0; l <= last; ++l) {
      if (save) { a.lin[st][l] = off; off += nP; }
      HierOut o{};
// ... 80 lines not shown
  unsigned* const slots = reinterpret_cast<unsigned*>(A + a.amax);
  auto sl = [&](int aset) -> unsigned* { return (x2 && aset >= 0) ? slots + (int64_t)aset * WIRE_AMAX_SLOTS : nullptr; };
  if (x2) HIPCHK(hipMemsetAsync(slots, 0, (size_t)hier_sets(p) * WIRE_AMAX_SLOTS * sizeof(unsigned), s));
  for (int st = 0; st < p.HS; ++st) {
    const float c = p.sc_c[st];
    const HierNat nat = hier_nat(p, packed, st);
    const int last = hier_last(p, st);
    auto lin = [&](int l) -> float* { return a.lin[st][l] >= 0 ? A + a.lin[st][l] : nullptr; };
    {
      const HierOut& o = a.out[st][0];
      ProfScope ps(s, 3, 0);
      HIPCHK(launch_hier_first_fwd(s, coords, n, p.D, nat.W0, nat.b0, p.K, p.P, c, lin(0), A + o.off, o.ld, sl(o.aset)));
    }
    for (int l = 1; l <= last; ++l) {
      const HierOut& o = a.out[st][l];
      GemmEpiParams ep;
      ep.o0 = lin(l); ep.o1 = A + o.off; ep.ld0 = p.P; ep.ld1 = o.ld; ep.omega = p.w; ep.scale = c; ep.kvalid = p.K;
      if (st > 0 && l == 1) {
        ep.bias = packed + p.hj_bias[st];
        ProfScope ps(s, 0, 2.0 * n * p.P * 2 * p.P);
        HIPCHK(hier_join_nt(s, p, r.fam, packed, st, A + a.cat[st], n, ep, sl(a.out[st][0].aset), sl(o.aset)));
      } else {
        const int v = hier_v(p, st, l);
        const HierOut& in = a.out[st][l - 1];
        ep.bias = packed + p.off_bias[v];
        ProfScope ps(s, 0, 2.0 * n * p.P * p.P);
        HIPCHK(layer_nt(s, p, r.fam, packed, v, false, EPI_BSPLINE_FWD, A + in.off, n, ep, sl(in.aset), wamax_of(p, packed, v),
                        sl(o.aset)));
      }
    }
    const HierOut& xl = a.out[st][last];
    const bool fin = loss && st == p.HS - 1;
    ProfScope ps(s, 3, 0);
    HIPCHK(launch_hier_head_fwd(s, A + xl.off, xl.ld, nat.Wh, nat.bh, n, p.K, p.P, p.O, st > 0, y, fin ? *loss : M2Loss{},
                                fin ? loss_part : nullptr));
  }
  return WIRE_OK;
}

int hier_bwd_core(void* stream, const Plan& p, const Route& r, const float* packed, const float* coords, int64_t n,
                  const float* g_y, const void* act, int64_t act_bytes, void* scratch, int64_t scratch_bytes,
                  void* const* grads, wire_grad_ready_fn ready, void* user, float* g_coords) {
  if (n <= 0) return fail(WIRE_ERR_ARG, "backward needs n > 0");
  if (!packed || !coords || !g_y || !act || !scratch || (!grads && !g_coords)) return fail(WIRE_ERR_ARG, "null pointer");
  if (grads)
    for (int i = 0; i < p.ntens; ++i) if (!grads[i]) return fail(WIRE_ERR_ARG, "grads[%d] is null", i);
  const HierAct a = hier_act(p, n, 1);
  const HierScratch sc = hier_scratch(p, n);
  const int64_t need = g_coords ? sc.total_coords : sc.total;
  if (act_bytes < a.total * 4) return fail(WIRE_ERR_SIZE, "act buffer too small");
  if (scratch_bytes < need * 4) return fail(WIRE_ERR_SIZE, "scratch %lld < %lld bytes", (long long)scratch_bytes,
                                            (long long)need * 4);
  hipStream_t s = (hipStream_t)stream;
  const float* A = (const float*)act;
  float* Sx = (float*)scratch;
  const int S = p.HS, per = p.HL + 2;
  const bool x2 = r.fam == FAM_X2;
  const WireFamily tnj = (x2 && gemmx2_tn_applies(p.P, 2 * p.P)) ? FAM_X2 : p.x3 ? FAM_X3 : FAM_4M;
  const WireFamily tnk = r.tn_fam == FAM_3M ? FAM_4M : r.tn_fam;
  const int tnk_S = hier_tn_splits(tnk, n, p.P, p.P, sc.S), tnj_S = hier_tn_splits(tnj, n, p.P, 2 * p.P, sc.S);
  unsigned* const gs = reinterpret_cast<unsigned*>(Sx + sc.gamax);
  const unsigned* const os = reinterpret_cast<const unsigned*>(A + a.amax);
  auto gsl = [&](int st, int l) -> unsigned* { return x2 ? gs + (int64_t)(st * per + l) * WIRE_AMAX_SLOTS : nullptr; };
  auto osl = [&](int aset) -> const unsigned* { return (x2 && aset >= 0) ? os + (int64_t)aset * WIRE_AMAX_SLOTS : nullptr; };
  auto grad = [&](int t) -> float* { return (float*)grads[t]; };
  auto done = [&](int t, int cnt) { if (ready) ready(user, t, cnt); };
  if (x2) HIPCHK(hipMemsetAsync(gs, 0, (size_t)hier_sets(p) * WIRE_AMAX_SLOTS * sizeof(unsigned), s));
  if (grads) {
    ProfScope ps(s, 3, 0);
    for (int st = 0; st < S; ++st) {
      const HierOut& xl = a.out[st][hier_last(p, st)];
      HIPCHK(launch_hier_head_bwd(s, g_y, n, p.O, hier_nat(p, packed, st).Wh, A + xl.off, xl.ld, nullptr, nullptr, p.K, p.P,
                                  p.sc_c[st], nullptr, Sx + sc.fpw, Sx + sc.fpb, nullptr));
      HIPCHK(launch_final_reduce(s, WIRE_KIND_BSPLINE, Sx + sc.fpw, Sx + sc.fpb, final_bwd_blocks(n), p.O, p.K, p.P,
                                 grad(hier_th(p, st)), grad(hier_th(p, st) + 1)));
    }
    done(hier_th(p, 0), 2 * S);
  }
  float* gcur = Sx + sc.g[0];
  float* gnext = Sx + sc.g[1];
  float* const T = Sx + sc.g[2];
  for (int st = S - 1; st >= 0; --st) {
    const float c = p.sc_c[st];
    const HierNat nat = hier_nat(p, packed, st);
    const int last = hier_last(p, st);
    {
      ProfScope ps(s, 3, 0);
      HIPCHK(launch_hier_head_bwd(s, g_y, n, p.O, nat.Wh, nullptr, 0, A + a.lin[st][last], st + 1 < S ? T : nullptr, p.K,
                                  p.P, c, gcur, nullptr, nullptr, gsl(st, last)));
    }
    for (int l = last; l >= 1; --l) {
      const bool join = st > 0 && l == 1;
      if (grads) {
        const int t = hier_t(p, st, l);
        if (join) {
          { ProfScope ps(s, 2, 2.0 * n * p.P * 2 * p.P);
            HIPCHK(hier_tn(s, p, tnj, gcur, A + a.cat[st], 2 * p.P, 2 * p.P, n, tnj_S, Sx + sc.slab, Sx + sc.bslab, gsl(st, l),
                           osl(st * per))); }
          ProfScope ps(s, 3, 0);
          HIPCHK(launch_hier_join_reduce(s, Sx + sc.slab, Sx + sc.bslab, tnj_S, p.K, p.P, grad(t), grad(t + 1)));
        } else {
          const HierOut& in = a.out[st][l - 1];
          { ProfScope ps(s, 2, 2.0 * n * p.P * p.P);
            HIPCHK(hier_tn(s, p, tnk, gcur, A + in.off, in.ld, p.P, n, tnk_S, Sx + sc.slab, Sx + sc.bslab, gsl(st, l),
                           osl(in.aset))); }
          ProfScope ps(s, 3, 0);
          HIPCHK(launch_wgrad_reduce(s, WIRE_KIND_BSPLINE, Sx + sc.slab, Sx + sc.bslab, tnk_S, p.K, p.K, p.P, p.P, grad(t),
                                     grad(t + 1), nullptr, nullptr));
        }
        done(t, 2);
      }
      GemmEpiParams ep;
      ep.kvalid = p.K; ep.ld0 = p.P; ep.ld1 = p.P; ep.omega = p.w;
      if (join) {
        ep.scale = c; ep.i0 = A + a.lin[st][0]; ep.o0 = gnext;
        { ProfScope ps(s, 1, 2.0 * n * p.P * p.P);
          const int v = hier_vhalf(p, st, 0);
          HIPCHK(layer_nt(s, p, r.fam, packed, v, true, EPI_BSPLINE_BWD, gcur, n, ep, gsl(st, l), wamax_of(p, packed, v),
                          nullptr)); }
        ep.scale = p.sc_c[st - 1]; ep.i0 = A + a.lin[st - 1][hier_last(p, st - 1)]; ep.o0 = T;
        ProfScope ps(s, 1, 2.0 * n * p.P * p.P);
        const int v = hier_vhalf(p, st, 1);
        HIPCHK(layer_nt(s, p, r.fam, packed, v, true, EPI_BSPLINE_BWD, gcur, n, ep, gsl(st, l), wamax_of(p, packed, v),
                        nullptr));
      } else {
        ep.scale = c; ep.i0 = A + a.lin[st][l - 1]; ep.o0 = gnext;
        const int v = hier_v(p, st, l);
        ProfScope ps(s, 1, 2.0 * n * p.P * p.P);
        HIPCHK(layer_nt(s, p, r.fam, packed, v, true, EPI_BSPLINE_BWD, gcur, n, ep, gsl(st, l), wamax_of(p, packed, v),
                        l >= 2 ? gsl(st, l - 1) : nullptr));
      }
      float* t = gcur; gcur = gnext; gnext = t;
    }
    ProfScope ps(s, 3, 0);
    if (grads) {
      HIPCHK(launch_colreduce(s, gcur, p.P, p.K, coords, p.D, n, Sx + sc.crp, grad(hier_t(p, st, 0)),
                              grad(hier_t(p, st, 0) + 1)));
      done(hier_t(p, st, 0), 2);
    }
    if (g_coords)
      HIPCHK(launch_coordgrad_rows(s, gcur, p.P, nullptr, nat.W0, nullptr, p.K, p.D, n,
                                   S == 1 ? g_coords : Sx + sc.cgp + (int64_t)st * n * p.D));
  }
  if (g_coords && S > 1) {
    ProfScope ps(s, 3, 0);
    HIPCHK(launch_m2_sum_passes(s, Sx + sc.cgp, S, n, p.D, g_coords));
  }
  return WIRE_OK;
}

Route hier_route(const Plan& p, int64_t n, RouteMode mode) {
  Route r = make_route(p, n, mode);
  r.fused_fwd = r.fuse = r.fused_train = r.fused_final = r.chain = r.rstore = r.skip_out_L = false;
  r.first_sums = r.cg_epi = false;
  r.wb_l0 = p.L + 1; r.wb_n = 0;
  for (float& v : r.out_scale) v = 0.f;
  return r;
}

int hier_pack(hipStream_t s, const Plan& p, const void* const* params, float* packed) {
  std::vector<const float*> hW(p.L + 1, nullptr), hb(p.L + 1, nullptr);
  HIPCHK(hipMemsetAsync(packed + p.hj_wamax, 0, (size_t)p.HS * WIRE_AMAX_SLOTS * sizeof(float), s));
  for (int l = 1; l <= p.HL; ++l) {
    hW[l] = (const float*)params[hier_t(p, 0, l)]; hb[l] = (const float*)params[hier_t(p, 0, l) + 1];
  }
  for (int st = 1; st < p.HS; ++st) {
    const float* Wj = (const float*)params[hier_t(p, st, 1)];
    const float* bj = (const float*)params[hier_t(p, st, 1) + 1];
    float* Wa = packed + p.hj_half[st];
    float* Wb = Wa + rup(p.K * p.K, 4);
    float* img = packed + p.hj_fwd[st];
    HIPCHK(launch_hier_pack_join(s, Wj, bj, p.K, p.P, img, packed + p.hj_bias[st], Wa, Wb));
    HIPCHK(launch_x3_split_b(s, img, 2 * p.P, p.P, 2 * p.P, packed + p.hj_fwd_x3[st]));
    X2AmaxBatch ab{};
    X2SplitBatch xf{};
    ab.src[0] = xf.src[0] = img;
    ab.slots[0] = reinterpret_cast<unsigned*>(packed + p.hj_wamax) + st * WIRE_AMAX_SLOTS;
    xf.dst[0] = packed + p.hj_fwd_x2[st]; xf.slots[0] = ab.slots[0];
    HIPCHK(launch_amax_batch(s, ab, 1, (int64_t)p.P * 2 * p.P));
    HIPCHK(launch_x2_split_b_batch(s, xf, 1, 2 * p.P, p.P, 2 * p.P));
    hW[hier_v(p, st, 2)] = (const float*)params[hier_t(p, st, 2)];
    hb[hier_v(p, st, 2)] = (const float*)params[hier_t(p, st, 2) + 1];
    hW[hier_vhalf(p, st, 0)] = Wa; hb[hier_vhalf(p, st, 0)] = bj;
    hW[hier_vhalf(p, st, 1)] = Wb; hb[hier_vhalf(p, st, 1)] = bj;
  }
  if (int rc = pack_hidden(s, p, params, packed, hW, hb)) return rc;
  for (int st = 0; st < p.HS; ++st) {
    const HierNat h = hier_nat(p, packed, st);
    const float* dst[4] = {h.W0, h.b0, h.Wh, h.bh};
    const int src[4] = {hier_t(p, st, 0), hier_t(p, st, 0) + 1, hier_th(p, st), hier_th(p, st) + 1};
    for (int q = 0; q < 4; ++q)
      HIPCHK(hipMemcpyAsync(const_cast<float*>(dst[q]), params[src[q]], p.tfloats[src[q]] * 4, hipMemcpyDeviceToDevice,
                            s));
  }
  return WIRE_OK;
}
```

wire_amd/csrc/wire_knobs.h:

```cpp
#pragma once
#include <atomic>

enum Knob {
  K_COMPLEX_3M, K_SPLIT_BF16, K_SPLIT_F16, K_SPLIT_OUT, K_RECOMPUTE_OUT, K_FIRST_SUMS, K_FUSED_RSTORE, K_WGRAD_BATCH,
  K_FUSED_FWD, K_FUSED_TRAIN, K_FUSED_TRAIN_P384, K_FUSED_FINAL, K_FUSED_BWD, K_FUSED_BWD_W,
  K_NT_BK, K_X2_AMODE, K_X2_TN_ROWS, K_X2_TN_P384, K_X3_TALL, K_X3_TALL_REAL, K_X3_TN_TALL, K_X3_TN16, K_X3_H16,
  K_X3H_STAGGER,
  K_FX_ABLATE, K_FXB_ABLATE, K_TN_ABL,
  K_COUNT
};

extern std::atomic<int> g_knob[K_COUNT];
inline int knob(Knob k) { return g_knob[k].load(std::memory_order_relaxed); }

int knob_get(const char* key);
int knob_set(const char* key, int value);
```

wire_amd/csrc/wire_knobs.hip:

```cpp
#include <cerrno>
#include <climits>
#include <cstdio>
#include <cstdlib>
#include <cstring>
#include <string>

#include "wire_knobs.h"

std::atomic<int> g_knob[K_COUNT];

namespace {
struct KnobDef {
  Knob id;
  const char* key;
  const char* env;
  int dflt;
  bool flag;
  int lo, hi;
  int a, b;
};
constexpr KnobDef flag_knob(Knob id, const char* key, const char* env, int dflt) { return {id, key, env, dflt, true, 0, 1, -1, -1}; }
constexpr KnobDef range_knob(Knob id, const char* key, const char* env, int dflt, int lo, int hi, int a = -1) {
  return {id, key, env, dflt, false, lo, hi, a, -1};
}
constexpr KnobDef choice_knob(Knob id, const char* key, const char* env, int dflt, int a, int b) { return {id, key, env, dflt, false, 1, 0, a, b}; }
constexpr bool accepts(const KnobDef& d, int v) {
  return d.flag || (d.lo <= v && v <= d.hi) || (v >= 0 && (v == d.a || v == d.b));
}
#ifdef WIRE_FX_ABLATE
#define FX_ABLATE_KEY(k) k
#else
#define FX_ABLATE_KEY(k) nullptr
#endif

constexpr KnobDef kKnobs[] = {
    flag_knob(K_COMPLEX_3M, "complex_3m", nullptr, 1),
    flag_knob(K_SPLIT_BF16, "split_bf16", "WIRE_SPLIT_BF16", 1),
    flag_knob(K_SPLIT_F16, "split_f16", "WIRE_SPLIT_F16", 1),
    flag_knob(K_SPLIT_OUT, "split_out", "WIRE_SPLIT_OUT", 1),
    flag_knob(K_RECOMPUTE_OUT, "recompute_out", "WIRE_RECOMPUTE_OUT", 1),
    flag_knob(K_FIRST_SUMS, "first_sums", "WIRE_FIRST_SUMS", 1),
    flag_knob(K_FUSED_RSTORE, "fused_rstore", "WIRE_FUSED_RSTORE", 1),
    flag_knob(K_WGRAD_BATCH, "wgrad_batch", "WIRE_WGRAD_BATCH", 1),
    range_knob(K_FUSED_FWD, "fused_fwd", "WIRE_FUSED_FWD", 1, 0, 1),
    range_knob(K_FUSED_TRAIN, "fused_train", "WIRE_FUSED_TRAIN", 1, 0, 1),
    flag_knob(K_FUSED_TRAIN_P384, "fused_train_p384", "WIRE_FUSED_TRAIN_P384", 0),
    range_knob(K_FUSED_FINAL, "fused_final", "WIRE_FUSED_FINAL", 0, 0, 1),
    range_knob(K_FUSED_BWD, "fused_bwd", "WIRE_FUSED_BWD", 1, 0, 1),
    choice_knob(K_FUSED_BWD_W, "fused_bwd_w", "WIRE_FUSED_BWD_W", 8, 4, 8),
    choice_knob(K_NT_BK, "nt_bk", "WIRE_NT_BK", 16, 16, 32),
    range_knob(K_X2_AMODE, "x2_amode", "WIRE_X2_AMODE", 2, 0, 2),
    range_knob(K_X2_TN_ROWS, "x2_tn_rows", "WIRE_X2_TN_ROWS", 0, 256, INT_MAX, 0),
    choice_knob(K_X2_TN_P384, "x2_tn_p384", "WIRE_X2_TN_P384", 8, 6, 8),
    range_knob(K_X3_TALL, "x3_tall", "WIRE_X3_TALL", 1, 0, 1),
    range_knob(K_X3_TALL_REAL, "x3_tall_real", "WIRE_X3_TALL_REAL", 0, 0, 1),
    range_knob(K_X3_TN_TALL, "x3_tn_tall", "WIRE_X3_TN_TALL", 0, 0, 1),
    range_knob(K_X3_TN16, "x3_tn16", "WIRE_X3_TN16", 1, 0, 1),
    range_knob(K_X3_H16, "x3_h16", "WIRE_X3_H16", 15, 0, 15),
    range_knob(K_X3H_STAGGER, "x3h_stagger", "WIRE_X3H_STAGGER", 0, 0, INT_MAX),
    range_knob(K_FX_ABLATE, FX_ABLATE_KEY("fx_ablate"), nullptr, 0, 0, 15),
    range_knob(K_FXB_ABLATE, FX_ABLATE_KEY("fxb_ablate"), nullptr, 0, 0, 127),
    range_knob(K_TN_ABL, nullptr, "WIRE_TN_ABL", 0, 0, 15),
};

constexpr bool rows_valid() {
  for (int i = 0; i < K_COUNT; ++i)
    if (kKnobs[i].id != i || !accepts(kKnobs[i], kKnobs[i].dflt)) return false;
  return true;
}
static_assert(sizeof kKnobs / sizeof kKnobs[0] == K_COUNT && rows_valid(), "one row per Knob, in enum order, default accepted");

const KnobDef* find(const char* key) {
  for (const KnobDef& d : kKnobs)
    if (d.key && !strcmp(d.key, key)) return &d;
  return nullptr;
}
std::string accepted(const KnobDef& d) {
  if (d.flag) return "any integer, 0 = off";
  std::string s;
  for (const int v : {d.a, d.b})
    if (v >= 0) s += (s.empty() ? "" : " or ") + std::to_string(v);
  if (d.lo <= d.hi) s += (s.empty() ? "" : " or ") + std::to_string(d.lo) + (d.hi == INT_MAX ? ".." : ".." + std::to_string(d.hi));
  return s;
}
int from_env(const KnobDef& d) {
  const char* s = d.env ? getenv(d.env) : nullptr;
  if (!s) return d.dflt;
  char* end = nullptr;
  errno = 0;
  const long v = strtol(s, &end, 10);
  if (end != s && *end == '\0' && errno == 0 && v >= INT_MIN && v <= INT_MAX && accepts(d, (int)v))
    return d.flag ? v != 0 : (int)v;
  fprintf(stderr, "libwire_hip: ignoring %s=%s (accepted: %s); using the default %d\n", d.env, s, accepted(d).c_str(), d.dflt);
  return d.dflt;
}
struct KnobLoader {
  KnobLoader() {
    for (const KnobDef& d : kKnobs) g_knob[d.id].store(from_env(d), std::memory_order_relaxed);
  }
} g_knob_loader;
}

int knob_get(const char* key) {
  const KnobDef* d = find(key);
  return d ? knob(d->id) : -1;
}
int knob_set(const char* key, int value) {
  const KnobDef* d = find(key);
  if (!d || !accepts(*d, value)) return -1;
  g_knob[d->id].store(d->flag ? value != 0 : value, std::memory_order_relaxed);
  return 0;
}
```

wire_amd/csrc/wire_mfn_api.hip:

```cpp
#include "wire_plan.h"

Route mfn_route(const Plan& p, int64_t n, RouteMode mode) {
  Route r = make_route(p, n, mode);
  r.fused_fwd = r.fuse = r.fused_train = r.fused_final = r.chain = r.rstore = r.skip_out_L = false;
  r.first_sums = r.cg_epi = r.recompute_out = r.recompute_out0 = false;
  r.wb_l0 = p.L + 1; r.wb_n = 0;
  for (float& v : r.out_scale) v = 0.f;
  return r;
}

int mfn_pack(hipStream_t s, const Plan& p, const void* const* params, float* packed) {
  std::vector<const float*> hW(p.L + 1, nullptr), hb(p.L + 1, nullptr);
  for (int l = 1; l <= p.L; ++l) { hW[l] = (const float*)params[mfn_tw(p, l)]; hb[l] = (const float*)params[mfn_tw(p, l) + 1]; }
  if (int rc = pack_hidden(s, p, params, packed, hW, hb)) return rc;
  HIPCHK(launch_pack_final(s, p.kind, (const float*)params[p.ntens - 2], (const float*)params[p.ntens - 1], p.K, p.P, p.O,
                           packed + p.off_wf, packed + p.off_bf));
  for (int i = 0; i <= p.L; ++i)
    HIPCHK(launch_mfn_pack_table(s, (const float*)params[4 * i], (const float*)params[4 * i + 1],
                                 (const float*)params[4 * i + 2], (const float*)params[4 * i + 3], p.K, p.D, p.P,
                                 const_cast<float*>(mfn_tab(p, packed, i))));
  return WIRE_OK;
}

int mfn_fwd_core(void* stream, const Plan& p, const Route& r, const float* packed, const float* coords, int64_t n, float* y,
                 void* act, int64_t act_bytes) {
  const bool save = r.mode != MODE_INFER;
  if (n < 0) return fail(WIRE_ERR_ARG, "negative n");
  if (n == 0) return WIRE_OK;
  if (!packed || !coords || !y || !act) return fail(WIRE_ERR_ARG, "null pointer");
  const ActLayout a = act_layout(p, n, save);
  if (act_bytes < a.total * 4) return fail(WIRE_ERR_SIZE, "act buffer %lld < %lld bytes", (long long)act_bytes,
                                           (long long)a.total * 4);
  hipStream_t s = (hipStream_t)stream;
  float* A = (float*)act;
  const bool x2 = r.fam == FAM_X2;
  unsigned* const amax = reinterpret_cast<unsigned*>(A + a.amax);
  if (x2) HIPCHK(hipMemsetAsync(amax, 0, (size_t)(p.L + 2) * WIRE_AMAX_SLOTS * sizeof(unsigned), s));
  auto z_l = [&](int l) { return save ? A + a.out0 + (int64_t)l * a.np * p.P : A + ((l & 1) ? a.pong : a.ping); };
  auto lin_l = [&](int l) -> float* { return save ? A + a.lin1 + (int64_t)(l - 1) * a.np * p.Pl : nullptr; };
  {
    ProfScope ps(s, 3, 0);
    HIPCHK(launch_mfn_filter_fwd(s, mfn_tab(p, packed, 0), coords, n, p.D, p.K, p.P, nullptr, z_l(0), x2 ? amax : nullptr));
  }
  for (int l = 1; l <= p.L; ++l) {
    GemmEpiParams ep;
    ep.bias = packed + p.off_bias[l]; ep.o0 = lin_l(l); ep.o1 = z_l(l); ep.ld0 = p.P; ep.ld1 = p.P; ep.kvalid = p.K;
    ep.coords = coords; ep.D = p.D; ep.ftab = mfn_tab(p, packed, l);
    ProfScope ps(s, 0, 2.0 * n * p.P * p.P);
    HIPCHK(layer_nt(s, p, r.fam, packed, l, false, EPI_MFN_FWD, z_l(l - 1), n, ep, amax + (l - 1) * WIRE_AMAX_SLOTS,
                    wamax_of(p, packed, l), amax + l * WIRE_AMAX_SLOTS));
  }
  ProfScope ps(s, 3, 0);
  HIPCHK(launch_final_fwd(s, z_l(p.L), n, p.P, p.O, packed + p.off_wf, packed + p.off_bf, y));
  return WIRE_OK;
}

int mfn_bwd_core(void* stream, const Plan& p, const Route& r, const float* packed, const float* coords, int64_t n,
                 const float* g_y, const void* act, int64_t act_bytes, void* scratch, int64_t scratch_bytes,
                 void* const* grads, wire_grad_ready_fn ready, void* user, float* g_coords) {
  if (n <= 0) return fail(WIRE_ERR_ARG, "backward needs n > 0");
  if (!packed || !coords || !g_y || !act || !scratch || (!grads && !g_coords)) return fail(WIRE_ERR_ARG, "null pointer");
  if (grads)
    for (int i = 0; i < p.ntens; ++i) if (!grads[i]) return fail(WIRE_ERR_ARG, "grads[%d] is null", i);
  const ActLayout a = act_layout(p, n, 1);
  const ScratchLayout sc = scratch_layout(p, n);
  const int64_t need = g_coords ? coord_layout(p, n).total : sc.total;
  if (act_bytes < a.total * 4) return fail(WIRE_ERR_SIZE, "act buffer too small");
  if (scratch_bytes < need * 4) return fail(WIRE_ERR_SIZE, "scratch %lld < %lld bytes", (long long)scratch_bytes,
                                            (long long)need * 4);
  hipStream_t s = (hipStream_t)stream;
  const float* A = (const float*)act;
  float* Sx = (float*)scratch;
  const bool x2 = r.fam == FAM_X2;
  auto z_l = [&](int l) { return A + a.out0 + (int64_t)l * a.np * p.P; };
  auto lin_l = [&](int l) { return A + a.lin1 + (int64_t)(l - 1) * a.np * p.Pl; };
  auto gslots = [&](int l) { return reinterpret_cast<unsigned*>(Sx + sc.gamax) + l * WIRE_AMAX_SLOTS; };
  auto oslots = [&](int l) { return reinterpret_cast<const unsigned*>(A + a.amax) + l * WIRE_AMAX_SLOTS; };
  auto grad = [&](int t) -> float* { return (float*)grads[t]; };
  auto done = [&](int t, int cnt) { if (ready) ready(user, t, cnt); };
  float* gcur = Sx + sc.ga;
  float* gnext = Sx + sc.gb;
  float* const H = Sx + sc.mh;
  bool gx_started = false;
  auto filter = [&](int i) -> int {
    ProfScope ps(s, 3, 0);
    if (grads)
      HIPCHK(launch_mfn_filter_sums(s, mfn_tab(p, packed, i), coords, n, p.D, p.K, H, p.P, Sx + sc.mfp, grad(4 * i),
                                    grad(4 * i + 1), grad(4 * i + 2), grad(4 * i + 3)));
    if (g_coords) {
      HIPCHK(launch_mfn_filter_gx(s, mfn_tab(p, packed, i), coords, n, p.D, p.K, H, p.P, gx_started ? 1 : 0, g_coords));
      gx_started = true;
    }
    return WIRE_OK;
  };
  if (x2) HIPCHK(hipMemsetAsync(gslots(0), 0, (size_t)(p.L + 2) * WIRE_AMAX_SLOTS * sizeof(unsigned), s));
  {
    ProfScope ps(s, 3, 0);
    HIPCHK(launch_mfn_final_bwd(s, g_y, n, p.O, packed + p.off_wf, z_l(p.L), p.L >= 1 ? lin_l(p.L) : nullptr,
                                mfn_tab(p, packed, p.L), coords, p.D, p.P, gcur, H, grads ? Sx + sc.fpw : nullptr,
                                grads ? Sx + sc.fpb : nullptr, x2 ? gslots(p.L) : nullptr));
    if (grads) {
      HIPCHK(launch_final_reduce(s, p.kind, Sx + sc.fpw, Sx + sc.fpb, final_bwd_blocks(n), p.O, p.K, p.P, grad(p.ntens - 2),
                                 grad(p.ntens - 1)));
      done(p.ntens - 2, 2);
    }
  }
  if (int rc = filter(p.L)) return rc;
  for (int l = p.L; l >= 1; --l) {
    if (grads) {
      {
        ProfScope ps(s, 2, 2.0 * n * p.P * p.P);
        float* slab = Sx + sc.slab;
        float* bslab = Sx + sc.bslab;
        switch (r.tn_fam) {
          case FAM_X2:
            HIPCHK(launch_gemmx2_tn(s, gcur, p.P, z_l(l - 1), p.P, n, p.P, p.P, r.tn_S, slab, bslab, gslots(l), oslots(l - 1)));
            break;
          case FAM_X3: HIPCHK(launch_gemmx3_tn(s, gcur, p.P, z_l(l - 1), p.P, n, p.P, p.P, r.tn_S, slab, bslab)); break;
          default: HIPCHK(launch_gemm_tn(s, gcur, p.P, z_l(l - 1), p.P, n, p.P, p.P, r.tn_S, slab, bslab)); break;
        }
      }
      ProfScope ps(s, 3, 0);
      HIPCHK(launch_wgrad_reduce(s, p.kind, Sx + sc.slab, Sx + sc.bslab, r.tn_S, p.K, p.K, p.P, p.P, grad(mfn_tw(p, l)),
                                 grad(mfn_tw(p, l) + 1), nullptr, nullptr));
      done(mfn_tw(p, l), 2);
      done(4 * l, 4);
    }
    {
      GemmEpiParams ep;
      ep.kvalid = p.K; ep.ld0 = p.P; ep.ld1 = p.P; ep.coords = coords; ep.D = p.D;
      ep.i0 = l >= 2 ? lin_l(l - 1) : nullptr; ep.o0 = gnext; ep.o1 = H; ep.ftab = mfn_tab(p, packed, l - 1);
      ProfScope ps(s, 1, 2.0 * n * p.P * p.P);
      HIPCHK(layer_nt(s, p, r.fam, packed, l, true, EPI_MFN_BWD, gcur, n, ep, gslots(l), wamax_of(p, packed, l),
                      l >= 2 ? gslots(l - 1) : nullptr));
    }
    if (int rc = filter(l - 1)) return rc;
    float* t = gcur; gcur = gnext; gnext = t;
  }
  if (grads) done(0, 4);
  return WIRE_OK;
}

static int mfn_layer_args(int64_t n, int D, int K) {
  if (n <= 0) return fail(WIRE_ERR_ARG, "wire_mfn_filter: n must be positive");
  if (D < 1 || D > 4) return fail(WIRE_ERR_ARG, "in_features %d outside 1..4", D);
  if (K < 1 || K > 4096) return fail(WIRE_ERR_ARG, "out_features %d outside 1..4096", K);
  return WIRE_OK;
}
extern "C" int wire_mfn_filter_fwd(void* stream, const float* x, const float* mu, const float* gamma, const float* w,
                                   const float* c, int64_t n, int in_features, int out_features, float* out) {
  if (int rc = mfn_layer_args(n, in_features, out_features)) return rc;
  if (!x || !mu || !gamma || !w || !c || !out) return fail(WIRE_ERR_ARG, "null pointer");
  hipStream_t s = (hipStream_t)stream;
  ProfScope ps(s, 3, 0);
  HIPCHK(launch_mfn_filter_fwd_native(s, mu, gamma, w, c, x, n, in_features, out_features, out));
  return WIRE_OK;
}
extern "C" int64_t wire_mfn_filter_ws_bytes(int64_t n, int out_features) {
// ... 19 lines not shown
```

wire_amd/csrc/wire_plan.h:

```cpp
#pragma once
#include <hip/hip_runtime.h>

#include <atomic>
#include <mutex>
#include <utility>
#include <vector>

#include "../../include/wire_hip.h"
#include "wire_gemm.h"
#include "wire_point.h"

#ifndef WIRE_AMAX_SLOTS
#define WIRE_AMAX_SLOTS 64
#endif

int fail(int code, const char* fmt, ...);
int wire_fail_(int code, const char* msg);
#define HIPCHK(expr)                                                                   \
  do {                                                                                 \
    hipError_t e_ = (expr);                                                            \
    if (e_ != hipSuccess)                                                              \
      return fail(WIRE_ERR_HIP, "%s failed: %s (%s:%d)", #expr, hipGetErrorString(e_), \
                  __FILE__, __LINE__);                                                 \
  } while (0)

struct ProfRec { hipEvent_t a, b; int cls; double flops; };
extern std::mutex g_prof_mu;
extern std::atomic<bool> g_prof_on;
extern std::vector<ProfRec> g_prof_recs;
extern std::vector<std::pair<hipEvent_t, hipEvent_t>> g_prof_pool;

struct ProfScope {
  hipStream_t s; int cls; double flops; bool on; hipEvent_t a{}, b{};
  ProfScope(hipStream_t s_, int cls_, double flops_) : s(s_), cls(cls_), flops(flops_), on(false) {
    if (!g_prof_on.load(std::memory_order_relaxed)) return;
    std::lock_guard<std::mutex> lk(g_prof_mu);
    if (!g_prof_on.load(std::memory_order_relaxed)) return;
    on = true;
    if (!g_prof_pool.empty()) {
      a = g_prof_pool.back().first; b = g_prof_pool.back().second; g_prof_pool.pop_back();
    } else {
      (void)hipEventCreate(&a); (void)hipEventCreate(&b);
    }
    (void)hipEventRecord(a, s);
  }
  ~ProfScope() {
    if (!on) return;
    (void)hipEventRecord(b, s);
    std::lock_guard<std::mutex> lk(g_prof_mu);
    g_prof_recs.push_back({a, b, cls, flops});
  }
};

inline int rup(int v, int m) { return (v + m - 1) / m * m; }

struct Plan {
  int kind, D, K, L, O, F;
  float w1, w, s;
  bool cplx, first_gemm, m3, x3, x2;
  int P, Pl, Din, Pin0, ldu, ntens, per_layer, Kp;
  int nsc = 0;
  float sc_c[WIRE_MS_MAX_SCALES] = {};
  bool ms = false;
  int SHF = 0, T = 0, ms_split = 0, t0 = 0;
  bool m2 = false;
  int S2 = 1;
  int64_t off_comb = -1;
  bool hier = false;
  int HS = 0, HL = 0;
  int64_t hj_fwd[WIRE_MS_MAX_SCALES] = {}, hj_fwd_x3[WIRE_MS_MAX_SCALES] = {}, hj_fwd_x2[WIRE_MS_MAX_SCALES] = {},
          hj_bias[WIRE_MS_MAX_SCALES] = {}, hj_half[WIRE_MS_MAX_SCALES] = {}, hj_wamax = -1, h_nat = -1;
  bool mfn = false;
  int64_t mf_tab = -1;
  std::vector<int64_t> off_fwd, off_dg, off_bias, off_fwd_x3, off_dg_x3, off_fwd_3m, off_dg_3m, off_fwd_x2, off_dg_x2;
  int64_t off_wf, off_bf, off_first, off_wamax, total_packed;
  int64_t off_fx;
  bool k_split_out, k_recompute_out, k_first_sums, k_rstore, k_wgrad_batch, k_fused_fwd, k_fused_train, k_fused_bwd, k_fused_final,
       k_fused_train_p384;
  int64_t off_fxd;
  std::vector<int64_t> tfloats;
};

inline int first_tensor(const Plan& p, int q) { return p.ms ? q : p.t0 + q; }

inline int mfn_tw(const Plan& p, int l) { return 4 * (p.L + 1) + 2 * (l - 1); }
inline const float* mfn_tab(const Plan& p, const float* packed, int i) { return packed + p.mf_tab + (int64_t)i * p.P * 12; }

inline int hier_last(const Plan& p, int st) { return st == 0 ? p.HL : 2; }
inline int hier_t(const Plan& p, int st, int l) {
  return st == 0 ? 2 * l : 2 * (p.HL + 1) + 6 * (st - 1) + 2 * l;
}
inline int hier_th(const Plan& p, int st) { return 2 * (p.HL + 1) + 6 * (p.HS - 1) + 2 * st; }
inline int hier_v(const Plan& p, int st, int l) { return st == 0 ? l : p.HL + 3 * (st - 1) + 1; }
inline int hier_vhalf(const Plan& p, int st, int half) { return p.HL + 3 * (st - 1) + 2 + half; }
inline int64_t hier_nat_stride(const Plan& p) {
  return rup(p.K * p.D, 4) + rup(p.K, 4) + rup(p.O * p.K, 4) + rup(p.O, 4);
}
struct HierNat { const float* W0; const float* b0; const float* Wh; const float* bh; };
inline HierNat hier_nat(const Plan& p, const float* packed, int st) {
  HierNat h;
  const float* c = packed + p.h_nat + (int64_t)st * hier_nat_stride(p);
  h.W0 = c; c += rup(p.K * p.D, 4);
  h.b0 = c; c += rup(p.K, 4);
  h.Wh = c; c += rup(p.O * p.K, 4);
  h.bh = c;
  return h;
}

int make_plan(const wire_net_desc* d, Plan& p);

inline int64_t fx_hidden_off(const Plan& p) { return p.off_fx + (p.first_gemm ? (int64_t)p.P * p.Pin0 : 0); }
inline int64_t fx_pass_off(const Plan& p, int k) { return fx_hidden_off(p) + (int64_t)k * p.L * fused_b_image_floats(p.P); }
inline float pass_c(const Plan& p, int k) { return p.m2 ? p.sc_c[k] : p.s; }
inline int64_t first_native_off(const Plan& p, int q) {
  int64_t off = p.off_first;
  for (int i = 0; i < q; ++i) off += rup((int)p.tfloats[first_tensor(p, i)], 4);
  return off;
}
inline M2Comb comb_of(const Plan& p, const float* packed) {
  M2Comb w;
  const float* c = packed + p.off_comb;
  w.W1 = c; c += rup((int)p.tfloats[0], 4);
  w.b1 = c; c += rup((int)p.tfloats[1], 4);
  w.W2 = c; c += rup((int)p.tfloats[2], 4);
  w.b2 = c;
  return w;
}

struct ActLayout {
  int64_t pe, out0, lin0, lin1, total;
  int64_t ping, pong;
  int64_t amax;
  int64_t pe_amax;
  int64_t ytr;
  int64_t np;
};
ActLayout act_layout(const Plan& p, int64_t n1, int save);

struct ScratchLayout { int64_t ga, gb, gu, slab, bslab, fpw, fpb, crp, gamax, gch, gch_stride, gtr, cpart, crep, mh, mfp, total; int S; };
ScratchLayout scratch_layout(const Plan& p, int64_t n1);

struct CoordLayout { int64_t cgp, gpe, total; int ntiles; };
CoordLayout coord_layout(const Plan& p, int64_t n);

int epi_fwd(int kind);
int epi_bwd(int kind);

enum RouteMode { MODE_INFER, MODE_AUTOGRAD, MODE_TRAIN };
struct Route {
  RouteMode mode;
  WireFamily fam;
  WireFamily fam0;
  WireFamily tn0;
  float pe_split;
  WireFamily tn_fam;
  int tn_S;
  bool fused_fwd;
  bool fuse;
  bool fused_train;
  bool fused_final;
  bool chain;
  bool rstore;
  bool skip_out_L;
  bool recompute_out;
  bool recompute_out0;
  bool first_sums;
  bool cg_epi;
  int wb_l0, wb_n, wb_S;
  float act_scale;
  float out_scale[65];
};
Route make_route(const Plan& p, int64_t n, RouteMode mode);

inline const unsigned* wamax_of(const Plan& p, const float* packed, int l) {
  return reinterpret_cast<const unsigned*>(packed + p.off_wamax + (int64_t)l * WIRE_AMAX_SLOTS);
}
hipError_t layer_nt(hipStream_t s, const Plan& p, WireFamily f, const float* packed, int l, bool dg, int epi,
                    const float* A, int64_t n, GemmEpiParams ep, const unsigned* amax_a = nullptr,
                    const unsigned* amax_b = nullptr, unsigned* amax_out = nullptr);

Route mfn_route(const Plan& p, int64_t n, RouteMode mode);
int mfn_pack(hipStream_t s, const Plan& p, const void* const* params, float* packed);
int mfn_fwd_core(void* stream, const Plan& p, const Route& r, const float* packed, const float* coords, int64_t n, float* y,
                 void* act, int64_t act_bytes);
int mfn_bwd_core(void* stream, const Plan& p, const Route& r, const float* packed, const float* coords, int64_t n,
                 const float* g_y, const void* act, int64_t act_bytes, void* scratch, int64_t scratch_bytes,
                 void* const* grads, wire_grad_ready_fn ready, void* user, float* g_coords);

struct HierOut { int64_t off; int ld; int aset; };
struct HierAct {
  int64_t amax, total;
  std::vector<std::vector<int64_t>> lin;
  std::vector<std::vector<HierOut>> out;
  std::vector<int64_t> cat;
};
struct HierScratch { int64_t gamax, g[3], slab, bslab, fpw, fpb, crp, lpart, total, cgp, total_coords; int S; };

HierAct hier_act(const Plan& p, int64_t n, int save);
HierScratch hier_scratch(const Plan& p, int64_t n);
Route hier_route(const Plan& p, int64_t n, RouteMode mode);
int pack_hidden(hipStream_t s, const Plan& p, const void* const* params, float* packed, const std::vector<const float*>& hW,
                const std::vector<const float*>& hb);
int hier_pack(hipStream_t s, const Plan& p, const void* const* params, float* packed);
int hier_fwd_core(void* stream, const Plan& p, const Route& r, const float* packed, const float* coords, int64_t n, float* y,
                  void* act, int64_t act_bytes, const M2Loss* loss = nullptr, float* loss_part = nullptr);
int hier_bwd_core(void* stream, const Plan& p, const Route& r, const float* packed, const float* coords, int64_t n,
                  const float* g_y, const void* act, int64_t act_bytes, void* scratch, int64_t scratch_bytes,
                  void* const* grads, wire_grad_ready_fn ready, void* user, float* g_coords);
```

wire_amd/csrc/wire_plan.hip:

```cpp
#include <cmath>

#include "wire_plan.h"

static int read_scales(const wire_net_desc_ms* m, int kind, int lo, Plan& p) {
  if (kind == WIRE_KIND_BSPLINE_MS) {
    p.SHF = m->first_width;
    if (p.SHF < 1 || p.SHF > 4096) return fail(WIRE_ERR_ARG, "first_width %d outside 1..4096", p.SHF);
  } else if (m->first_width != 0) {
    return fail(WIRE_ERR_ARG, "first_width %d: kind %d has no first stage", m->first_width, kind);
  }
  p.nsc = m->nscales;
  if (p.nsc < lo || p.nsc > WIRE_MS_MAX_SCALES)
    return fail(WIRE_ERR_ARG, "nscales %d outside %d..%d", p.nsc, lo, WIRE_MS_MAX_SCALES);
  if (p.SHF > 256) {
    p.ms_split = (p.SHF - 256) / (p.nsc - 1);
    if (p.ms_split < 1 || 256 + (p.nsc - 1) * p.ms_split != p.SHF)
      return fail(WIRE_ERR_ARG, "first_width %d is not 256 + %d equal column groups", p.SHF, p.nsc - 1);
  }
  for (int k = 0; k < p.nsc; ++k) {
    const float sk = m->scales[k];
    if (!(std::isfinite(sk) && sk != 0.f)) return fail(WIRE_ERR_ARG, "scales[%d] %g is zero or not finite", k, (double)sk);
    p.sc_c[k] = (float)(1.0 / fabs((double)sk));
  }
  return WIRE_OK;
}

int make_plan(const wire_net_desc* d, Plan& p) {
  if (!d) return fail(WIRE_ERR_ARG, "null descriptor");
  p.kind = d->kind; p.D = d->in_features; p.K = d->width; p.L = d->hidden_layers;
  p.O = d->out_features; p.F = d->posenc_freqs;
  p.w1 = d->first_omega0; p.w = d->hidden_omega0; p.s = d->scale0;
  if (p.kind < WIRE_KIND_WIRE || (p.kind > WIRE_KIND_BSPLINE_MS && p.kind != WIRE_KIND_BSPLINE_M2 &&
                                  p.kind != WIRE_KIND_BSPLINE_HIER && p.kind != WIRE_KIND_MFN))
    return fail(WIRE_ERR_ARG, "unknown kind %d", p.kind);
  if (p.kind == WIRE_KIND_MFN) {
    p.mfn = true;
    p.kind = WIRE_KIND_RELU;
    p.F = 0;
  }
  if (p.kind == WIRE_KIND_BSPLINE_HIER) {
    const wire_net_desc_ms* m = reinterpret_cast<const wire_net_desc_ms*>(d);
    if (int rc = read_scales(m, WIRE_KIND_BSPLINE_HIER, 1, p)) return rc;
    p.HS = p.nsc;
    p.HL = p.L;
    if (p.HL < 1 || p.HL > 40) return fail(WIRE_ERR_ARG, "hidden_layers %d outside 1..40 (kind %d)", p.HL,
                                           (int)WIRE_KIND_BSPLINE_HIER);
    if (p.HL == 1 && p.HS > 1)
      return fail(WIRE_ERR_ARG, "hidden_layers 1 with %d scales: a later stage runs its layers 0, 1 and 2", p.HS);
    if (p.O >= 1 && p.O <= 8 && p.K >= 1 && p.K <= 4096 && (int64_t)p.O * rup(p.K, 64) > 16384)
      return fail(WIRE_ERR_ARG, "out_features %d x padded width %d > 16384 (kind %d)", p.O, rup(p.K, 64),
                  (int)WIRE_KIND_BSPLINE_HIER);
    p.hier = true;
    p.kind = WIRE_KIND_BSPLINE;
    p.s = m->scales[0];
    p.L = p.HL + 3 * (p.HS - 1);
  }
  if (p.kind == WIRE_KIND_BSPLINE_M2) {
    const wire_net_desc_ms* m = reinterpret_cast<const wire_net_desc_ms*>(d);
    if (int rc = read_scales(m, WIRE_KIND_BSPLINE_M2, 1, p)) return rc;
    p.S2 = p.nsc;
    p.m2 = true;
    p.kind = WIRE_KIND_BSPLINE;
    p.s = m->scales[0];
    p.t0 = 4;
  }
  if (p.kind == WIRE_KIND_BSPLINE_MS) {
    const wire_net_desc_ms* m = reinterpret_cast<const wire_net_desc_ms*>(d);
    if (int rc = read_scales(m, WIRE_KIND_BSPLINE_MS, 2, p)) return rc;
    p.ms = true; p.T = p.nsc;
    if (p.L < 0 || p.L > 65) return fail(WIRE_ERR_ARG, "hidden_layers %d outside 0..65", p.L);
    p.L = p.L > 1 ? p.L - 1 : 0;
    p.kind = WIRE_KIND_BSPLINE;
    p.t0 = 2;
  }
  if (p.kind == WIRE_KIND_BSPLINE) {
    if (!(std::isfinite(p.s) && p.s != 0.f)) return fail(WIRE_ERR_ARG, "bspline scale0 %g is zero or not finite", (double)p.s);
    p.s = (float)(1.0 / fabs((double)p.s));
  }
  if (p.D < 1 || p.D > 4) return fail(WIRE_ERR_ARG, "in_features %d outside 1..4", p.D);
  if (p.K < 1 || p.K > 4096) return fail(WIRE_ERR_ARG, "width %d outside 1..4096", p.K);
  if (p.L < 0 || p.L > 64) return fail(WIRE_ERR_ARG, "hidden_layers %d outside 0..64", p.L);
  if (p.O < 1 || p.O > 8) return fail(WIRE_ERR_ARG, "out_features %d outside 1..8", p.O);
  if (p.F < 0 || (p.F > 0 && p.kind != WIRE_KIND_RELU)) return fail(WIRE_ERR_ARG, "posenc only with relu");
  p.cplx = (p.kind == WIRE_KIND_WIRE || p.kind == WIRE_KIND_WIRE2D);
  p.P = p.cplx ? rup(2 * p.K, 64) : rup(p.K, 64);
  p.Pl = (p.kind == WIRE_KIND_WIRE2D) ? 2 * p.P : p.P;
  p.ldu = p.P / 2;
  p.Kp = p.P / 2;
  p.x3 = knob(K_SPLIT_BF16) != 0;
  p.x2 = p.x3 && knob(K_SPLIT_F16) != 0;
  p.m3 = (p.kind == WIRE_KIND_WIRE) && knob(K_COMPLEX_3M) && !p.x3;
  p.k_split_out = knob(K_SPLIT_OUT) != 0; p.k_recompute_out = knob(K_RECOMPUTE_OUT) != 0;
  p.k_first_sums = knob(K_FIRST_SUMS) != 0; p.k_rstore = knob(K_FUSED_RSTORE) != 0; p.k_wgrad_batch = knob(K_WGRAD_BATCH) != 0;
  p.k_fused_fwd = knob(K_FUSED_FWD) != 0; p.k_fused_train = p.k_fused_fwd && knob(K_FUSED_TRAIN);
  p.k_fused_train_p384 = knob(K_FUSED_TRAIN_P384) != 0;
  p.k_fused_bwd = p.k_fused_train && knob(K_FUSED_BWD); p.k_fused_final = p.k_fused_train && knob(K_FUSED_FINAL);
  p.first_gemm = p.F > 0 || p.ms;
  p.Din = p.ms ? p.SHF : p.first_gemm ? p.D + 2 * p.D * p.F : p.D;
  p.Pin0 = p.first_gemm ? rup(p.Din, 64) : 0;
  p.per_layer = (p.kind == WIRE_KIND_WIRE2D) ? 4 : 2;
  p.ntens = p.t0 + p.per_layer * (p.L + 1) + 2;
  p.tfloats.assign(p.ntens, 0);
  if (p.ms) { p.tfloats[0] = (int64_t)p.SHF * p.D; p.tfloats[1] = p.SHF; }
  if (p.m2) {
    p.tfloats[0] = (int64_t)M2_H * p.S2 * p.O; p.tfloats[1] = M2_H; p.tfloats[2] = (int64_t)p.O * M2_H; p.tfloats[3] = p.O;
  }
  const int64_t K = p.K, cm = p.cplx ? 2 : 1;
  for (int l = 0; l <= p.L; ++l) {
    const int64_t in = (l == 0) ? p.Din : K;
    const int64_t m = (l == 0) ? 1 : cm;
    for (int q = 0; q < p.per_layer; q += 2) {
      p.tfloats[p.t0 + p.per_layer * l + q] = m * K * in;
      p.tfloats[p.t0 + p.per_layer * l + q + 1] = m * K;
    }
  }
  p.tfloats[p.ntens - 2] = cm * p.O * K;
  p.tfloats[p.ntens - 1] = cm * p.O;
  if (p.mfn) {
    p.ntens = 4 * (p.L + 1) + 2 * p.L + 2;
    p.tfloats.assign(p.ntens, 0);
    for (int i = 0; i <= p.L; ++i) {
      p.tfloats[4 * i] = K * p.D; p.tfloats[4 * i + 1] = K; p.tfloats[4 * i + 2] = K * p.D; p.tfloats[4 * i + 3] = K;
    }
    for (int l = 1; l <= p.L; ++l) { p.tfloats[mfn_tw(p, l)] = K * K; p.tfloats[mfn_tw(p, l) + 1] = K; }
    p.tfloats[p.ntens - 2] = p.O * K; p.tfloats[p.ntens - 1] = p.O;
  }
  if (p.hier) {
    p.ntens = 2 * (p.HL + 1) + 6 * (p.HS - 1) + 2 * p.HS;
    p.tfloats.assign(p.ntens, 0);
    for (int st = 0; st < p.HS; ++st)
      for (int l = 0; l <= hier_last(p, st); ++l) {
        p.tfloats[hier_t(p, st, l)] = K * (l == 0 ? p.D : (st > 0 && l == 1) ? 2 * K : K);
        p.tfloats[hier_t(p, st, l) + 1] = K;
      }
    for (int st = 0; st < p.HS; ++st) { p.tfloats[hier_th(p, st)] = p.O * K; p.tfloats[hier_th(p, st) + 1] = p.O; }
  }
  int64_t off = 0;
  p.off_fwd.assign(p.L + 1, -1); p.off_dg.assign(p.L + 1, -1); p.off_bias.assign(p.L + 1, -1);
  p.off_fwd_x3.assign(p.L + 1, -1); p.off_dg_x3.assign(p.L + 1, -1);
  p.off_fwd_3m.assign(p.L + 1, -1); p.off_dg_3m.assign(p.L + 1, -1);
  p.off_fwd_x2.assign(p.L + 1, -1); p.off_dg_x2.assign(p.L + 1, -1);
  for (int l = p.first_gemm ? 0 : 1; l <= p.L; ++l) {
    const int64_t pin = (l == 0) ? p.Pin0 : p.P;
    const int64_t img = (int64_t)p.Pl * pin;
    p.off_fwd[l] = off; off += img;
    p.off_dg[l] = off; off += img;
    p.off_bias[l] = off; off += p.Pl;
    p.off_fwd_x3[l] = off; off += gemmx3_b_image_floats(p.Pl, (int)pin);
    p.off_dg_x3[l] = off; off += gemmx3_b_image_floats((int)pin, p.Pl);
    if (p.kind == WIRE_KIND_WIRE && l >= 1) {
      p.off_fwd_3m[l] = off; off += (int64_t)p.Kp * p.P;
      p.off_dg_3m[l] = off; off += (int64_t)p.Kp * p.P;
    }
    if (l >= 1) {
      p.off_fwd_x2[l] = off; off += gemmx2_b_image_floats(p.Pl, (int)pin);
      p.off_dg_x2[l] = off; off += gemmx2_b_image_floats((int)pin, p.Pl);
    } else if (p.ms) {
      p.off_fwd_x2[l] = off; off += gemmx2_b_image_floats(p.Pl, (int)pin);
    }
  }
  p.off_wamax = off; off += (int64_t)(p.L + 1) * WIRE_AMAX_SLOTS;
  p.off_fx = -1;
  const bool fx_ok = !p.hier && !p.mfn && p.L >= 1 && fused_fwd_shape(p.kind, p.P) &&
                     (!p.first_gemm || (p.kind == WIRE_KIND_RELU && p.Pin0 == 64));
  if (fx_ok) {
    p.off_fx = off;
    off += (p.first_gemm ? (int64_t)p.P * p.Pin0 : 0) + (int64_t)p.S2 * p.L * fused_b_image_floats(p.P);
  }
  p.off_fxd = -1;
  if (fx_ok && p.L >= 1 && fused_bwd_shape(p.kind, p.P)) { p.off_fxd = off; off += (int64_t)p.L * fused_b_image_floats(p.P); }
  p.off_wf = off; off += (int64_t)p.O * p.P;
  p.off_bf = off; off += 64;
  p.off_first = off;
  if (p.hier) {
    for (int st = 1; st < p.HS; ++st) {
      const int64_t img = (int64_t)p.P * 2 * p.P;
      p.hj_fwd[st] = off; off += img;
      p.hj_bias[st] = off; off += p.P;
      p.hj_fwd_x3[st] = off; off += gemmx3_b_image_floats(p.P, 2 * p.P);
      p.hj_fwd_x2[st] = off; off += gemmx2_b_image_floats(p.P, 2 * p.P);
      p.hj_half[st] = off; off += 2 * rup(p.K * p.K, 4);
    }
    p.hj_wamax = off; off += (int64_t)p.HS * WIRE_AMAX_SLOTS;
    p.h_nat = off;
    off += (int64_t)p.HS * hier_nat_stride(p);
  } else if (p.mfn) {
    p.mf_tab = off; off += (int64_t)(p.L + 1) * p.P * 12;
  } else if (!p.first_gemm || p.ms) {
    for (int q = 0; q < p.per_layer; ++q) off += rup((int)p.tfloats[first_tensor(p, q)], 4);
  }
  if (p.m2) {
    p.off_comb = off;
    for (int q = 0; q < 4; ++q) off += rup((int)p.tfloats[q], 4);
  }
  p.total_packed = off;
  return WIRE_OK;
}

ActLayout act_layout(const Plan& p, int64_t n1, int save) {
  ActLayout a{};
  int64_t off = 0;
  const int64_t n = n1 * p.S2;
  a.np = (n + 127) / 128 * 128 + (p.m2 ? 128 : 0);
  a.amax = off; off += (int64_t)(p.L + 2) * WIRE_AMAX_SLOTS;
  a.pe_amax = off; if (p.ms) off += WIRE_AMAX_SLOTS;
  a.pe = off; if (p.first_gemm) off += n * p.Pin0;
  if (save) {
    a.out0 = off; off += a.np * p.P * (p.L + 1);
    a.lin0 = off; if (!p.cplx && !p.mfn) off += a.np * p.P;
    a.lin1 = off; off += a.np * p.Pl * p.L;
  } else {
    a.ping = off; off += n * p.P;
    a.pong = off; off += n * p.P;
  }
  a.ytr = off; if (p.m2) off += n * p.O;
  a.total = off;
  return a;
}

ScratchLayout scratch_layout(const Plan& p, int64_t n1) {
  ScratchLayout s{};
  int64_t off = 0;
  const int64_t n = n1 * p.S2;
  s.gamax = off; off += (int64_t)(p.L + 2) * WIRE_AMAX_SLOTS;
  s.ga = off; off += n * p.Pl;
  s.gb = off; off += n * p.Pl;
  s.gch = -1; s.gch_stride = ((n + 127) / 128 * 128 + (p.m2 ? 128 : 0)) * p.Pl;
  if (p.off_fxd >= 0) { s.gch = off; off += (int64_t)(p.L + 1) * s.gch_stride; }
  s.gu = off; if (p.cplx) off += n * p.ldu * (p.kind == WIRE_KIND_WIRE2D ? 2 : 1);
  const int64_t pn = p.first_gemm && p.Pin0 > p.P ? p.Pin0 : p.P;
  const int s_x3k = gemmx3_tn_splits_max(n, p.Pl, (int)pn, 256), s_4m = gemm_tn_splits(n, p.Pl, (int)pn, 64);
  const int s_x2 = gemmx2_tn_splits(n, p.Pl, (int)pn, 256);
  const int s_x3 = s_x3k > s_x2 ? s_x3k : s_x2;
  const int s_max = s_x3 > s_4m ? s_x3 : s_4m;
  if (p.m3) {
    s.S = gemm3m_tn_splits(n, p.Kp, p.Kp, 64);
    int64_t need = (int64_t)s.S * 3 * p.Kp * p.Kp, full = (int64_t)s_max * p.Pl * pn;
    s.slab = off; off += need > full ? need : full;
    need = (int64_t)s.S * 2 * p.Kp; full = (int64_t)s_max * p.Pl;
    s.bslab = off; off += need > full ? need : full;
  } else {
    s.S = p.x3 ? s_x3 : s_4m;
    int64_t need3 = 0, needb3 = 0;
    if (p.kind == WIRE_KIND_WIRE) {
      const int s3 = gemm3m_tn_splits(n, p.Kp, p.Kp, 64);
      need3 = (int64_t)s3 * 3 * p.Kp * p.Kp; needb3 = (int64_t)s3 * 2 * p.Kp;
    }
    int64_t full = (int64_t)s_max * p.Pl * pn;
    s.slab = off; off += need3 > full ? need3 : full;
    full = (int64_t)s_max * p.Pl;
    s.bslab = off; off += needb3 > full ? needb3 : full;
  }
  const int nbf = prereduce_room((p.off_fx >= 0 && !p.cplx ? 2 : 1) * p.S2 * final_bwd_blocks(n1));
  s.fpw = off; off += (int64_t)nbf * p.O * p.P;
  s.fpb = off; off += (int64_t)nbf * p.O + 64;
  s.crp = off; off += (int64_t)prereduce_room((p.off_fxd >= 0 ? 4 : 1) * colreduce_blocks(n)) * (p.cplx ? p.ldu : p.P) * 5 *
                      (p.kind == WIRE_KIND_WIRE2D ? 2 : 1);
  s.gtr = s.cpart = s.crep = off;
  if (p.m2) {
    s.gtr = off; off += n * p.O;
    s.cpart = off; off += (int64_t)m2_comb_blocks(n1) * m2_comb_grad_floats(p.S2, p.O) + M2_COMB_MAXBLK;
    s.crep = off; off += n * p.D;
  }
  s.mh = s.mfp = off;
  if (p.mfn) {
    s.mh = off; off += n * p.P;
    s.mfp = off; off += (int64_t)(mfn_sums_blocks(n) + 1) * 10 * p.K;
  }
  s.total = off;
  return s;
}

CoordLayout coord_layout(const Plan& p, int64_t n) {
  CoordLayout c{};
  int64_t off = (scratch_layout(p, n).total + 63) / 64 * 64;
  c.ntiles = (p.P + 127) / 128;
  c.cgp = off; off += (int64_t)c.ntiles * n * p.S2 * p.D;
  off = (off + 63) / 64 * 64;
  c.gpe = off; if (p.first_gemm) off += n * p.Pin0;
  c.total = off;
  return c;
}

int epi_fwd(int kind) {
  switch (kind) {
    case WIRE_KIND_WIRE: return EPI_GABOR_FWD;
    case WIRE_KIND_WIRE2D: return EPI_GABOR2D_FWD;
    case WIRE_KIND_SIREN: return EPI_SIREN_FWD;
    case WIRE_KIND_GAUSS: return EPI_GAUSS_FWD;
    case WIRE_KIND_BSPLINE: return EPI_BSPLINE_FWD;
    default: return EPI_RELU_FWD;
  }
}
int epi_bwd(int kind) {
  switch (kind) {
    case WIRE_KIND_WIRE: return EPI_GABOR_BWD;
    case WIRE_KIND_WIRE2D: return EPI_GABOR2D_BWD;
    case WIRE_KIND_SIREN: return EPI_SIREN_BWD;
    case WIRE_KIND_GAUSS: return EPI_GAUSS_BWD;
    case WIRE_KIND_BSPLINE: return EPI_BSPLINE_BWD;
    default: return EPI_RELU_BWD;
  }
}

static float act_bound_scale(const Plan& p) {
  double bound = 1.0;
  if (p.cplx) {
    if (!(p.s > 0.f)) return 0.f;
    const double r = (double)p.w / (2.0 * (double)p.s);
    if (!(r * r <= 2.7725887)) return 0.f;
    bound = exp(r * r);
  }
  return ldexpf(1.f, 15 - (ilogb(bound) + 1));
}

Route make_route(const Plan& p, int64_t n, RouteMode mode) {
  Route r{};
  r.mode = mode;
  const bool h16_fwd = gemmx3_nt_is_h16(epi_fwd(p.kind), n);
  const bool x2 = p.x2 && p.L >= 1 && h16_fwd && gemmx3_nt_is_h16(epi_bwd(p.kind), n);
  const bool x2tn = x2 && gemmx2_tn_applies(p.Pl, p.P);
  r.fam = x2 ? FAM_X2 : p.m3 ? FAM_3M : p.x3 ? FAM_X3 : FAM_4M;
  r.fam0 = p.x3 ? FAM_X3 : FAM_4M;
  r.tn0 = r.fam0;
  if (p.ms && x2) {
    r.fam0 = FAM_X2;
    if (p.Pin0 >= p.P && gemmx2_tn_applies(p.Pl, p.Pin0)) { r.tn0 = FAM_X2; r.pe_split = 32768.f; }
  }
  r.tn_fam = p.m3 ? FAM_3M : x2tn ? FAM_X2 : p.x3 ? FAM_X3 : FAM_4M;
  const int64_t nt = n * p.S2;
  const int S_max = scratch_layout(p, n).S;
  r.tn_S = r.tn_fam == FAM_3M ? S_max
         : r.tn_fam == FAM_X2 ? gemmx2_tn_splits(nt, p.Pl, p.P, S_max)
         : r.tn_fam == FAM_X3 ? gemmx3_tn_splits(nt, p.Pl, p.P, S_max) : gemm_tn_splits(nt, p.Pl, p.P, S_max);
  r.recompute_out = p.k_recompute_out && p.x3 && h16_fwd;
  r.act_scale = (p.kind == WIRE_KIND_RELU || p.kind == WIRE_KIND_WIRE2D) ? 0.f : act_bound_scale(p);
  const bool fx = x2 && p.off_fx >= 0 && p.L <= 8 && (r.act_scale != 0.f || p.kind == WIRE_KIND_RELU) &&
                  fused_pre_scale(p.kind, p.w1, p.s) > 0.f && fused_pre_scale(p.kind, p.w, p.s) > 0.f;
  r.fused_fwd = mode == MODE_INFER && fx && p.k_fused_fwd && p.O <= 4;
  const bool ftrain = fx && x2tn && p.k_fused_train && p.k_split_out && p.k_recompute_out &&
                      !(p.kind == WIRE_KIND_WIRE && p.P > 256 && !p.k_fused_train_p384);
  r.fuse = mode == MODE_TRAIN && p.L >= 1 && p.O <= 4 && !p.m2 && final_fused_supported(p.P, p.O);
  r.skip_out_L = r.fuse && r.recompute_out && p.kind != WIRE_KIND_RELU;
  r.fused_train = r.fuse && ftrain && (r.skip_out_L || p.kind == WIRE_KIND_RELU);
  const bool m2_chain = p.m2 && mode == MODE_TRAIN && fx && x2tn;
  r.chain = (r.fused_train || m2_chain) && p.k_fused_bwd && p.off_fxd >= 0;
  r.fused_final = r.chain && r.fused_train && !p.cplx && p.k_fused_final;
  r.rstore = r.chain && r.fused_train && p.k_rstore &&
             (p.kind == WIRE_KIND_SIREN || p.kind == WIRE_KIND_GAUSS || p.kind == WIRE_KIND_BSPLINE);
  const bool split = x2tn && p.k_split_out && p.kind != WIRE_KIND_RELU &&
                     (p.k_recompute_out || p.kind == WIRE_KIND_SIREN || p.kind == WIRE_KIND_BSPLINE);
  for (int l = 1; l < p.L; ++l) r.out_scale[l] = !split ? 0.f : ftrain ? 1.f : act_bound_scale(p);
  const int epi1 = p.kind == WIRE_KIND_WIRE ? EPI_GABOR_BWD_FIRST
                 : p.kind == WIRE_KIND_WIRE2D ? EPI_GABOR2D_BWD_FIRST : epi_bwd(p.kind);
  const bool h16_1 = p.x3 && gemmx3_nt_is_h16(epi1, n);
  r.cg_epi = h16_1 && !p.first_gemm && p.L >= 1 && !p.m2;
  r.first_sums = r.cg_epi && p.k_first_sums;
  r.recompute_out0 = h16_1 && p.kind == WIRE_KIND_WIRE && p.k_recompute_out;
  r.wb_l0 = p.L + 1;
  if (r.chain && p.k_wgrad_batch) {
    const int l0 = (r.rstore || p.kind == WIRE_KIND_RELU) ? 1 : 2, nb = p.L - l0 + 1;
    const int S = nb >= 2 ? gemmx2_tn_batch_splits(n, p.Pl, p.P, S_max, nb) : 0;
    if (S >= 1 && (int64_t)S * nb <= S_max) { r.wb_l0 = l0; r.wb_n = nb; r.wb_S = S; }
  }
  return r;
}

extern "C" int wire_num_param_tensors(const wire_net_desc* d) {
  Plan p; if (make_plan(d, p)) return WIRE_ERR_ARG;
  return p.ntens;
}
extern "C" int64_t wire_param_tensor_floats(const wire_net_desc* d, int t) {
  Plan p; if (make_plan(d, p)) return WIRE_ERR_ARG;
  if (t < 0 || t >= p.ntens) return fail(WIRE_ERR_ARG, "tensor index %d out of range", t);
  return p.tfloats[t];
}
extern "C" int64_t wire_packed_floats(const wire_net_desc* d) {
  Plan p; if (make_plan(d, p)) return WIRE_ERR_ARG;
  return p.total_packed;
}
extern "C" int64_t wire_act_bytes(const wire_net_desc* d, int64_t n, int save_for_bwd) {
  Plan p; if (make_plan(d, p)) return WIRE_ERR_ARG;
  if (n < 0) return fail(WIRE_ERR_ARG, "negative n");
  if (p.hier) return hier_act(p, n, save_for_bwd).total * 4 + 256;
  return act_layout(p, n, save_for_bwd).total * 4 + 256;
}
extern "C" int64_t wire_bwd_scratch_bytes(const wire_net_desc* d, int64_t n) {
  Plan p; if (make_plan(d, p)) return WIRE_ERR_ARG;
  if (n < 0) return fail(WIRE_ERR_ARG, "negative n");
  if (p.hier) return hier_scratch(p, n).total * 4 + 256;
  return scratch_layout(p, n).total * 4 + 256;
}
extern "C" int64_t wire_bwd_coords_scratch_bytes(const wire_net_desc* d, int64_t n) {
  Plan p; if (make_plan(d, p)) return WIRE_ERR_ARG;
  if (n < 0) return fail(WIRE_ERR_ARG, "negative n");
  if (p.hier) return hier_scratch(p, n).total_coords * 4 + 256;
  return coord_layout(p, n).total * 4 + 256;
}
extern "C" int wire_blocked_width(int K) { return rup(2 * K, 64); }
extern "C" int64_t wire_act_out_offset(const wire_net_desc* d, int64_t n, int layer) {
  Plan p; if (make_plan(d, p)) return WIRE_ERR_ARG;
  if (p.hier) return fail(WIRE_ERR_ARG, "wire_act_out_offset: kind %d keeps its activations per stage", (int)WIRE_KIND_BSPLINE_HIER);
  if (n < 0 || layer < 0 || layer > p.L) return fail(WIRE_ERR_ARG, "bad argument to wire_act_out_offset");
  const ActLayout a = act_layout(p, n, 1);
  return a.out0 + (int64_t)layer * a.np * p.P;
}
```

Measured before the change: 45.68 million.

## Add coordinate-dimension-specialized first-layer backward epilogues and lookahead Gabor backward epilogue

```diff
diff --git a/wire_amd/csrc/wire_api.hip b/wire_amd/csrc/wire_api.hip
--- a/wire_amd/csrc/wire_api.hip
+++ b/wire_amd/csrc/wire_api.hip
@@ -505,6 +505,7 @@
       ep.omega = (l - 1 == 0) ? p.w1 : p.w;
       ep.i0 = lin_l(l - 1); ep.o0 = gnext; ep.ld0 = p.Pl;
       ep.recompute_out = r.recompute_out && l >= 2;
+      ep.lookahead = r.bwd_lookahead && ep.recompute_out;
       if (l == 1 && first_sums) { ep.coords = coords; ep.D = p.D; ep.cr_partial = Sx + sc.crp; ep.cr_C = p.K; }
     } else {
       epi = (p.kind == WIRE_KIND_WIRE) ? EPI_GABOR_BWD_FIRST : EPI_GABOR2D_BWD_FIRST;
@@ -512,6 +513,7 @@
       ep.coords = coords; ep.D = p.D; ep.ldu = p.ldu; ep.o0 = Sx + sc.gu;
       if (first_sums) { ep.cr_partial = Sx + sc.crp; ep.cr_C = p.K; ep.cr_set = crp_set(); }
       ep.recompute_out = r.recompute_out0;
+      ep.first_dn = r.first_dn;
       ep.W0 = first(0); ep.b0 = first(1);
       if (pl == 4) { ep.W0b = first(2); ep.b0b = first(3); }
     }
diff --git a/wire_amd/csrc/wire_gemm.h b/wire_amd/csrc/wire_gemm.h
--- a/wire_amd/csrc/wire_gemm.h
+++ b/wire_amd/csrc/wire_gemm.h
@@ -21,8 +21,11 @@
   EPI_BSPLINE_BWD = 14,
   EPI_MFN_FWD = 15,
   EPI_MFN_BWD = 16,
-  EPI_CG = 64
+  EPI_CG = 64,
+  EPI_D2 = 128, EPI_D3 = 256,
+  EPI_LA = 512
 };
+constexpr int EPI_FLAGS = EPI_CG | EPI_D2 | EPI_D3 | EPI_LA;
 
 constexpr bool epi_real_fwd(int e) {
   return e == EPI_SIREN_FWD || e == EPI_GAUSS_FWD || e == EPI_RELU_FWD || e == EPI_BSPLINE_FWD;
@@ -57,6 +60,8 @@
   int64_t cr_set = 0;
   float* cg_partial = nullptr;
   int recompute_out = 0;
+  int lookahead = 0;
+  int first_dn = 0;
   int stagger = 0, stagger_lo = 0, stagger_hi = 0;
   const unsigned* amax_a = nullptr;
   const unsigned* amax_b = nullptr;
diff --git a/wire_amd/csrc/wire_gemmh_epi.h b/wire_amd/csrc/wire_gemmh_epi.h
--- a/wire_amd/csrc/wire_gemmh_epi.h
+++ b/wire_amd/csrc/wire_gemmh_epi.h
@@ -35,12 +35,350 @@
   for (int d = 0; d < ep.D; ++d) dst[d] = cg[d];
 }
 
+template <int DN>
+WIRE_DEVINL void h_cg_add_dn(float (&cg)[4], const float (&t)[DN], const int e, const int lane) {
+#pragma unroll
+  for (int d = 0; d < DN; ++d) {
+    float v = t[d];
+    v += __shfl_xor(v, 8); v += __shfl_xor(v, 16); v += __shfl_xor(v, 32);
+    cg[d] += (lane >> 3) == e ? v : 0.f;
+  }
+}
+template <int DN, int NRB>
+WIRE_DEVINL void h_load_rows_dn(float (&xs)[2 * NRB][DN], const GemmEpiParams& ep, const int M, const int m_w, const int rr) {
+#pragma unroll
+  for (int e = 0; e < 2 * NRB; ++e) {
+    int row = m_w + 8 * e + rr;
+    row = row < M ? row : M - 1;
+#pragma unroll
+    for (int d = 0; d < DN; ++d) xs[e][d] = ep.coords[(size_t)row * DN + d];
+  }
+}
+template <int DN>
+WIRE_DEVINL void h_crs_to_lds_dn(const float (&crs)[4][DN + 1], float* red, const int rr) {
+#pragma unroll
+  for (int q = 0; q < 4; ++q) {
+    float o[5] = {0.f, 0.f, 0.f, 0.f, 0.f};
+#pragma unroll
+    for (int d = 0; d <= DN; ++d) {
+      float v = crs[q][d];
+      v += __shfl_xor(v, 1); v += __shfl_xor(v, 2); v += __shfl_xor(v, 4);
+      o[d < DN ? d : 4] = v;
+    }
+    if (rr == 0) {
+#pragma unroll
+      for (int d = 0; d < 5; ++d) red[q * 5 + d] = o[d];
+    }
+  }
+}
+
+template <bool CG, int DN, int NRB>
+WIRE_DEVINL void h_gabor_bwd_first_dn(const f32x4 (&acc)[NRB][8], const GemmEpiParams& ep, const int M, const int m_w,
+                                      const int n_w, const int Nc, const int lane, unsigned char* lds, const int wave,
+                                      const int rt) {
+  const int rr = lane & 7, cq = 16 * ((lane >> 3) & 1) + 4 * (lane >> 4);
+  const float w0 = ep.omega, m2s2 = -2.f * ep.scale * ep.scale;
+  float xs[2 * NRB][DN];
+  h_load_rows_dn<DN, NRB>(xs, ep, M, m_w, rr);
+  float w[2][4][DN], bb[2][4];
+#pragma unroll
+  for (int G = 0; G < 2; ++G) {
+    const int c0 = n_w + 64 * G + cq;
+    const int f0 = ((c0 >> 6) << 5) + (c0 & 31);
+#pragma unroll
+    for (int q = 0; q < 4; ++q) {
+      const bool valid = f0 + q < ep.kvalid;
+      bb[G][q] = valid ? ep.b0[f0 + q] : 0.f;
+#pragma unroll
+      for (int d = 0; d < DN; ++d) w[G][q][d] = valid ? ep.W0[(f0 + q) * DN + d] : 0.f;
+    }
+  }
+  float cg[4] = {0.f, 0.f, 0.f, 0.f};
+#pragma unroll
+  for (int G = 0; G < 2; ++G) {
+    if (n_w + 64 * G >= Nc) continue;
+    const int c0 = n_w + 64 * G + cq;
+    const int f0 = ((c0 >> 6) << 5) + (c0 & 31);
+    float crs[4][DN + 1];
+#pragma unroll
+    for (int q = 0; q < 4; ++q)
+#pragma unroll
+      for (int d = 0; d <= DN; ++d) crs[q][d] = 0.f;
+#pragma unroll
+    for (int rb = 0; rb < NRB; ++rb) {
+      f32x4 are[2], aim[2];
+      h_pair_rows(acc[rb][4 * G], acc[rb][4 * G + 1], are[0], are[1]);
+      h_pair_rows(acc[rb][4 * G + 2], acc[rb][4 * G + 3], aim[0], aim[1]);
+#pragma unroll
+      for (int hr = 0; hr < 2; ++hr) {
+        const int e = 2 * rb + hr;
+        const int row = m_w + 8 * e + rr;
+        float t[DN];
+#pragma unroll
+        for (int d = 0; d < DN; ++d) t[d] = 0.f;
+        if (row < M) {
+          f32x4 pr = {0.f, 0.f, 0.f, 0.f}, pi = pr;
+          if (!ep.recompute_out) {
+            const float* Op = ep.i1 + (size_t)row * ep.ld1 + c0;
+            pr = *reinterpret_cast<const f32x4*>(Op);
+            pi = *reinterpret_cast<const f32x4*>(Op + 32);
+          }
+          f32x4 gu;
+#pragma unroll
+          for (int q = 0; q < 4; ++q) {
+            float u = bb[G][q];
+#pragma unroll
+            for (int d = 0; d < DN; ++d) u = __builtin_fmaf(xs[e][d], w[G][q][d], u);
+            if (ep.recompute_out) {
+              float a, b;
+              gabor_fwd_real(u, w0, ep.scale, a, b);
+              pr[q] = a; pi[q] = b;
+            }
+            const float v = gabor_bwd_real(are[hr][q], aim[hr][q], u, pr[q], pi[q], w0, m2s2);
+            gu[q] = f0 + q < ep.kvalid ? v : 0.f;
+          }
+          if constexpr (CG) {
+#pragma unroll
+            for (int q = 0; q < 4; ++q)
+#pragma unroll
+              for (int d = 0; d < DN; ++d) t[d] = __builtin_fmaf(gu[q], w[G][q][d], t[d]);
+          }
+          if (ep.cr_partial) {
+#pragma unroll
+            for (int q = 0; q < 4; ++q) {
+#pragma unroll
+              for (int d = 0; d < DN; ++d) crs[q][d] = __builtin_fmaf(gu[q], xs[e][d], crs[q][d]);
+              crs[q][DN] += gu[q];
+            }
+          } else {
+            *reinterpret_cast<f32x4*>(ep.o0 + (size_t)row * ep.ldu + f0) = gu;
+          }
+        }
+        if constexpr (CG) h_cg_add_dn<DN>(cg, t, e, lane);
+      }
+    }
+    if (ep.cr_partial)
+      h_crs_to_lds_dn<DN>(crs, reinterpret_cast<float*>(lds) + (wave * 64 + 32 * G + cq) * 5, rr);
+  }
+  if (ep.cr_partial) {
+    __syncthreads();
+    const float* red = reinterpret_cast<const float*>(lds);
+    const int fbase = (n_w >> 6) << 5;
+    for (int e = threadIdx.x; e < 64 * 5; e += 256) {
+      const int f = e / 5, d = e - 5 * f;
+      const float v = (red[e] + red[64 * 5 + e]) + (red[2 * 64 * 5 + e] + red[3 * 64 * 5 + e]);
+      if (fbase + f < ep.cr_C) ep.cr_partial[((size_t)rt * ep.cr_C + fbase + f) * 5 + d] = v;
+    }
+  }
+  if constexpr (CG) h_cg_store<NRB>(cg, ep, M, m_w, n_w, lane);
+}
+
+template <bool CG, int DN, int NRB>
+WIRE_DEVINL void h_gabor2d_bwd_first_dn(const f32x4 (&acc)[NRB][8], const GemmEpiParams& ep, const int M, const int m_w,
+                                        const int n_w, const int Nc, const int lane, unsigned char* lds, const int wave,
+                                        const int rt) {
+  const int rr = lane & 7, cq = 16 * ((lane >> 3) & 1) + 4 * (lane >> 4);
+  const float m2s2 = -2.f * ep.scale * ep.scale, w0 = ep.omega;
+  float xs[2 * NRB][DN];
+  h_load_rows_dn<DN, NRB>(xs, ep, M, m_w, rr);
+  float w[2][4][DN], wv[2][4][DN], bb[2][4], bv2[2][4];
+#pragma unroll
+  for (int G = 0; G < 2; ++G) {
+    const int c0 = n_w + 64 * G + cq;
+    const int f0 = ((c0 >> 6) << 5) + (c0 & 31);
+#pragma unroll
+    for (int q = 0; q < 4; ++q) {
+      const bool valid = f0 + q < ep.kvalid;
+      bb[G][q] = valid ? ep.b0[f0 + q] : 0.f;
+      bv2[G][q] = valid ? ep.b0b[f0 + q] : 0.f;
+#pragma unroll
+      for (int d = 0; d < DN; ++d) {
+        w[G][q][d] = valid ? ep.W0[(f0 + q) * DN + d] : 0.f;
+        wv[G][q][d] = valid ? ep.W0b[(f0 + q) * DN + d] : 0.f;
+      }
+    }
+  }
+  float cg[4] = {0.f, 0.f, 0.f, 0.f};
+#pragma unroll
+  for (int G = 0; G < 2; ++G) {
+    if (n_w + 64 * G >= Nc) continue;
+    const int c0 = n_w + 64 * G + cq;
+    const int f0 = ((c0 >> 6) << 5) + (c0 & 31);
+    float cru[4][DN + 1], crp2[4][DN + 1];
+#pragma unroll
+    for (int q = 0; q < 4; ++q)
+#pragma unroll
+      for (int d = 0; d <= DN; ++d) { cru[q][d] = 0.f; crp2[q][d] = 0.f; }
+#pragma unroll
+    for (int rb = 0; rb < NRB; ++rb) {
+      f32x4 are[2], aim[2];
+      h_pair_rows(acc[rb][4 * G], acc[rb][4 * G + 1], are[0], are[1]);
+      h_pair_rows(acc[rb][4 * G + 2], acc[rb][4 * G + 3], aim[0], aim[1]);
+      f32x4 pr[2], pi[2];
+#pragma unroll
+      for (int hr = 0; hr < 2; ++hr) {
+        int row = m_w + 16 * rb + 8 * hr + rr;
+        row = row < M ? row : M - 1;
+        const float* Op = ep.i1 + (size_t)row * ep.ld1 + c0;
+        pr[hr] = *reinterpret_cast<const f32x4*>(Op);
+        pi[hr] = *reinterpret_cast<const f32x4*>(Op + 32);
+      }
+#pragma unroll
+      for (int hr = 0; hr < 2; ++hr) {
+        const int e = 2 * rb + hr;
+        const int row = m_w + 8 * e + rr;
+        f32x4 g0, g2;
+#pragma unroll
+        for (int q = 0; q < 4; ++q) {
+          float uu = bb[G][q], p2 = bv2[G][q];
+#pragma unroll
+          for (int d = 0; d < DN; ++d) {
+            uu = __builtin_fmaf(xs[e][d], w[G][q][d], uu);
+            p2 = __builtin_fmaf(xs[e][d], wv[G][q][d], p2);
+          }
+          const float gr = are[hr][q], gi = aim[hr][q];
+          const float c_r = __builtin_fmaf(pr[hr][q], gr, pi[hr][q] * gi);
+          const float c_i = __builtin_fmaf(pr[hr][q], gi, -(pi[hr][q] * gr));
+          const float tt = m2s2 * c_r;
+          g0[q] = __builtin_fmaf(tt, uu, w0 * c_i);
+          g2[q] = tt * p2;
+        }
+        if constexpr (CG) {
+          float t[DN];
+#pragma unroll
+          for (int d = 0; d < DN; ++d) t[d] = 0.f;
+          if (row < M) {
+#pragma unroll
+            for (int q = 0; q < 4; ++q)
+#pragma unroll
+              for (int d = 0; d < DN; ++d)
+                t[d] = __builtin_fmaf(g2[q], wv[G][q][d], __builtin_fmaf(g0[q], w[G][q][d], t[d]));
+          }
+          h_cg_add_dn<DN>(cg, t, e, lane);
+        }
+        if (row < M) {
+#pragma unroll
+          for (int q = 0; q < 4; ++q)
+            if (!(f0 + q < ep.kvalid)) { g0[q] = 0.f; g2[q] = 0.f; }
+          if (ep.cr_partial) {
+#pragma unroll
+            for (int q = 0; q < 4; ++q) {
+#pragma unroll
+              for (int d = 0; d < DN; ++d) {
+                cru[q][d] = __builtin_fmaf(g0[q], xs[e][d], cru[q][d]);
+                crp2[q][d] = __builtin_fmaf(g2[q], xs[e][d], crp2[q][d]);
+              }
+              cru[q][DN] += g0[q];
+              crp2[q][DN] += g2[q];
+            }
+          } else {
+            float* Gp = ep.o0 + (size_t)row * (2 * ep.ldu);
+            *reinterpret_cast<f32x4*>(Gp + f0) = g0;
+            *reinterpret_cast<f32x4*>(Gp + ep.ldu + f0) = g2;
+          }
+        }
+      }
+    }
+    if (ep.cr_partial) {
+      float* red = reinterpret_cast<float*>(lds) + (wave * 64 + 32 * G + cq) * 5;
+      h_crs_to_lds_dn<DN>(cru, red, rr);
+      h_crs_to_lds_dn<DN>(crp2, red + 4 * 64 * 5, rr);
+    }
+  }
+  if (ep.cr_partial) {
+    __syncthreads();
+    const float* red = reinterpret_cast<const float*>(lds);
+    const int fbase = (n_w >> 6) << 5;
+    for (int e = threadIdx.x; e < 2 * 64 * 5; e += 256) {
+      const int set = e / (64 * 5), r = e - set * (64 * 5);
+      const int f = r / 5, d = r - 5 * f;
+      const float* rs = red + set * (4 * 64 * 5);
+      const float v = (rs[r] + rs[64 * 5 + r]) + (rs[2 * 64 * 5 + r] + rs[3 * 64 * 5 + r]);
+      if (fbase + f < ep.cr_C)
+        ep.cr_partial[(size_t)set * ep.cr_set + ((size_t)rt * ep.cr_C + fbase + f) * 5 + d] = v;
+    }
+  }
+  if constexpr (CG) h_cg_store<NRB>(cg, ep, M, m_w, n_w, lane);
+}
+
+template <bool X2, int NRB>
+WIRE_DEVINL void h_gabor_bwd_la(const f32x4 (&acc)[NRB][8], const GemmEpiParams& ep, const int M, const int m_w,
+                                const int n_w, const int Nc, const int lane, float& amx) {
+  const int rr = lane & 7, cq = 16 * ((lane >> 3) & 1) + 4 * (lane >> 4);
+  const float w0 = ep.omega, w0l2e = ep.omega * 1.44269502f, ns2l2e = -(ep.scale * ep.scale) * 1.44269502f;
+  const float m2s2 = -2.f * ep.scale * ep.scale;
+  const int ngrp = n_w + 64 >= Nc ? 1 : 2;
+  auto load_lin = [&](const int i, f32x4 (&u)[2], f32x4 (&v)[2]) {
+    const int G = i / NRB, rb = i % NRB;
+#pragma unroll
+    for (int hr = 0; hr < 2; ++hr) {
+      int row = m_w + 16 * rb + 8 * hr + rr;
+      row = row < M ? row : M - 1;
+      const float* Lp = ep.i0 + (size_t)row * ep.ld0 + n_w + 64 * G + cq;
+      u[hr] = *reinterpret_cast<const f32x4*>(Lp);
+      v[hr] = *reinterpret_cast<const f32x4*>(Lp + 32);
+    }
+  };
+  f32x4 lu[2], lv[2];
+  load_lin(0, lu, lv);
+#pragma unroll
+  for (int i = 0; i < 2 * NRB; ++i) {
+    const int G = i / NRB, rb = i % NRB;
+    if (G >= ngrp) break;
+    const int c0 = n_w + 64 * G + cq;
+    const int f0 = ((c0 >> 6) << 5) + (c0 & 31);
+    f32x4 nu[2] = {lu[0], lu[1]}, nv[2] = {lv[0], lv[1]};
+    const bool more = i + 1 < 2 * NRB && (i + 1) / NRB < ngrp;
+    if (more) load_lin(i + 1, nu, nv);
+    f32x4 are[2], aim[2], pr[2], pi[2];
+    h_pair_rows(acc[rb][4 * G], acc[rb][4 * G + 1], are[0], are[1]);
+    h_pair_rows(acc[rb][4 * G + 2], acc[rb][4 * G + 3], aim[0], aim[1]);
+#pragma unroll
+    for (int hr = 0; hr < 2; ++hr)
+#pragma unroll
+      for (int q = 0; q < 4; ++q) {
+        float a, b;
+        gabor_fwd_lean(lu[hr][q], lv[hr][q], w0, w0l2e, ns2l2e, a, b);
+        const bool valid = f0 + q < ep.kvalid;
+        pr[hr][q] = valid ? a : 0.f;
+        pi[hr][q] = valid ? b : 0.f;
+      }
+#pragma unroll
+    for (int hr = 0; hr < 2; ++hr) {
+      const int row = m_w + 16 * rb + 8 * hr + rr;
+      f32x4 gl_re, gl_im;
+#pragma unroll
+      for (int q = 0; q < 4; ++q) {
+        const float gr = are[hr][q], gi = aim[hr][q];
+        const float c_r = __builtin_fmaf(pr[hr][q], gr, pi[hr][q] * gi);
+        const float c_i = __builtin_fmaf(pr[hr][q], gi, -(pi[hr][q] * gr));
+        const float tt = m2s2 * c_r;
+        gl_re[q] = __builtin_fmaf(tt, lu[hr][q], w0 * c_i);
+        gl_im[q] = __builtin_fmaf(tt, lv[hr][q], -(w0 * c_r));
+      }
+      if constexpr (X2) { h_amax4(amx, gl_re); h_amax4(amx, gl_im); }
+      if (row < M) {
+        float* Gp = ep.o0 + (size_t)row * ep.ld0 + c0;
+        *reinterpret_cast<f32x4*>(Gp) = gl_re;
+        *reinterpret_cast<f32x4*>(Gp + 32) = gl_im;
+      }
+    }
+#pragma unroll
+    for (int hr = 0; hr < 2; ++hr) { lu[hr] = nu[hr]; lv[hr] = nv[hr]; }
+  }
+}
+
 template <int EPIX, bool X2 = false, int NRB = 4>
 WIRE_DEVINL void h_epilogue(f32x4 (&acc)[NRB][8], const GemmEpiParams& ep, const int M, const int m_w, const int n_w,
                             const int Nc, const int lane, unsigned char* lds, const int wave, const int rt,
                             const float acc_scale = 1.f) {
-  constexpr int EPI = EPIX & ~EPI_CG;
+  constexpr int EPI = EPIX & ~EPI_FLAGS;
   constexpr bool CG = (EPIX & EPI_CG) != 0;
+  constexpr int DN = (EPIX & EPI_D2) ? 2 : (EPIX & EPI_D3) ? 3 : 0;
+  constexpr bool LA = (EPIX & EPI_LA) != 0;
+  static_assert(!LA || EPI == EPI_GABOR_BWD, "EPI_LA: the hidden-layer data gradient of the 1-D Gabor net");
+  static_assert(DN == 0 || ((EPI == EPI_GABOR_BWD_FIRST || EPI == EPI_GABOR2D_BWD_FIRST) && NRB == 4),
+                "EPI_D2 / EPI_D3: the layer-1 forms of the complex nets on the 256-row tile");
   const int rr = lane & 7, ch = (lane >> 3) & 1, g = lane >> 4;
   float amx = 0.f;
   if constexpr (X2) {
@@ -302,6 +640,12 @@
         }
       }
     }
+  } else if constexpr (EPI == EPI_GABOR_BWD && LA) {
+    h_gabor_bwd_la<X2, NRB>(acc, ep, M, m_w, n_w, Nc, lane, amx);
+  } else if constexpr (EPI == EPI_GABOR_BWD_FIRST && DN != 0) {
+    h_gabor_bwd_first_dn<CG, DN, NRB>(acc, ep, M, m_w, n_w, Nc, lane, lds, wave, rt);
+  } else if constexpr (EPI == EPI_GABOR2D_BWD_FIRST && DN != 0) {
+    h_gabor2d_bwd_first_dn<CG, DN, NRB>(acc, ep, M, m_w, n_w, Nc, lane, lds, wave, rt);
   } else if constexpr (EPI == EPI_GABOR2D_BWD || EPI == EPI_GABOR2D_BWD_FIRST) {
     const float m2s2 = -2.f * ep.scale * ep.scale, w0 = ep.omega;
     float cg[4] = {0.f, 0.f, 0.f, 0.f};
diff --git a/wire_amd/csrc/wire_gemmx2h.hip b/wire_amd/csrc/wire_gemmx2h.hip
--- a/wire_amd/csrc/wire_gemmx2h.hip
+++ b/wire_amd/csrc/wire_gemmx2h.hip
@@ -364,13 +364,27 @@
       return hipErrorInvalidValue;
     }
   }
+  constexpr int EPI0 = EPI & ~(EPI_D2 | EPI_D3 | EPI_LA);
   if (knob(K_X2_AMODE) == 2)
     hipLaunchKernelGGL((gemmx2h_nt_kernel<EPI, 2, 4>), grid, dim3(256), 0, s, A, lda, Bx2, (int)M, Nc, Kd, tiles_m, tiles_n, ep);
   else if (knob(K_X2_AMODE) == 1)
-    hipLaunchKernelGGL((gemmx2h_nt_kernel<EPI, 1, 4>), grid, dim3(256), 0, s, A, lda, Bx2, (int)M, Nc, Kd, tiles_m, tiles_n, ep);
+    hipLaunchKernelGGL((gemmx2h_nt_kernel<EPI0, 1, 4>), grid, dim3(256), 0, s, A, lda, Bx2, (int)M, Nc, Kd, tiles_m, tiles_n, ep);
   else
-    hipLaunchKernelGGL((gemmx2h_nt_kernel<EPI, 0, 4>), grid, dim3(256), 0, s, A, lda, Bx2, (int)M, Nc, Kd, tiles_m, tiles_n, ep);
+    hipLaunchKernelGGL((gemmx2h_nt_kernel<EPI0, 0, 4>), grid, dim3(256), 0, s, A, lda, Bx2, (int)M, Nc, Kd, tiles_m, tiles_n, ep);
   return hipGetLastError();
+}
+template <int EPI>
+static hipError_t launchx2h_first(hipStream_t s, const float* A, int lda, const unsigned short* Bx2, int64_t M, int Nc,
+                                  int Kd, const GemmEpiParams& ep) {
+  constexpr int E3 = EPI == EPI_GABOR2D_BWD_FIRST ? 0 : EPI_D3;
+  const int dn = ep.first_dn && ep.coords && (ep.D == 2 || (ep.D == 3 && E3)) ? ep.D : 0;
+  if (ep.cg_partial)
+    return dn == 2 ? launchx2h_t<EPI | EPI_CG | EPI_D2>(s, A, lda, Bx2, M, Nc, Kd, ep)
+         : dn == 3 ? launchx2h_t<EPI | EPI_CG | E3>(s, A, lda, Bx2, M, Nc, Kd, ep)
+                   : launchx2h_t<EPI | EPI_CG>(s, A, lda, Bx2, M, Nc, Kd, ep);
+  return dn == 2 ? launchx2h_t<EPI | EPI_D2>(s, A, lda, Bx2, M, Nc, Kd, ep)
+       : dn == 3 ? launchx2h_t<EPI | E3>(s, A, lda, Bx2, M, Nc, Kd, ep)
+                 : launchx2h_t<EPI>(s, A, lda, Bx2, M, Nc, Kd, ep);
 }
 
 hipError_t launch_gemmx2h_nt(hipStream_t s, int epi, const float* A, int lda, const void* Bx2v, int64_t M, int Nc,
@@ -383,10 +397,10 @@
   switch (epi) {
     case EPI_STORE: return launchx2h_t<EPI_STORE>(s, A, lda, Bx2, M, Nc, Kd, ep);
     case EPI_GABOR_FWD: return launchx2h_t<EPI_GABOR_FWD>(s, A, lda, Bx2, M, Nc, Kd, ep);
-    case EPI_GABOR_BWD: return launchx2h_t<EPI_GABOR_BWD>(s, A, lda, Bx2, M, Nc, Kd, ep);
-    case EPI_GABOR_BWD_FIRST:
-      return ep.cg_partial ? launchx2h_t<EPI_GABOR_BWD_FIRST | EPI_CG>(s, A, lda, Bx2, M, Nc, Kd, ep)
-                           : launchx2h_t<EPI_GABOR_BWD_FIRST>(s, A, lda, Bx2, M, Nc, Kd, ep);
+    case EPI_GABOR_BWD:
+      return ep.lookahead && ep.recompute_out ? launchx2h_t<EPI_GABOR_BWD | EPI_LA>(s, A, lda, Bx2, M, Nc, Kd, ep)
+                          : launchx2h_t<EPI_GABOR_BWD>(s, A, lda, Bx2, M, Nc, Kd, ep);
+    case EPI_GABOR_BWD_FIRST: return launchx2h_first<EPI_GABOR_BWD_FIRST>(s, A, lda, Bx2, M, Nc, Kd, ep);
     case EPI_SIREN_FWD: return launchx2h_t<EPI_SIREN_FWD>(s, A, lda, Bx2, M, Nc, Kd, ep);
     case EPI_GAUSS_FWD: return launchx2h_t<EPI_GAUSS_FWD>(s, A, lda, Bx2, M, Nc, Kd, ep);
     case EPI_RELU_FWD: return launchx2h_t<EPI_RELU_FWD>(s, A, lda, Bx2, M, Nc, Kd, ep);
@@ -409,9 +423,7 @@
       if (Nc & 127) return hipErrorInvalidValue;
       return launchx2h_t<EPI_GABOR2D_FWD>(s, A, lda, Bx2, M, Nc, Kd, ep);
     case EPI_GABOR2D_BWD: return launchx2h_t<EPI_GABOR2D_BWD>(s, A, lda, Bx2, M, Nc, Kd, ep);
-    case EPI_GABOR2D_BWD_FIRST:
-      return ep.cg_partial ? launchx2h_t<EPI_GABOR2D_BWD_FIRST | EPI_CG>(s, A, lda, Bx2, M, Nc, Kd, ep)
-                           : launchx2h_t<EPI_GABOR2D_BWD_FIRST>(s, A, lda, Bx2, M, Nc, Kd, ep);
+    case EPI_GABOR2D_BWD_FIRST: return launchx2h_first<EPI_GABOR2D_BWD_FIRST>(s, A, lda, Bx2, M, Nc, Kd, ep);
     default: return hipErrorInvalidValue;
   }
 }
diff --git a/wire_amd/csrc/wire_gemmx3h.hip b/wire_amd/csrc/wire_gemmx3h.hip
--- a/wire_amd/csrc/wire_gemmx3h.hip
+++ b/wire_amd/csrc/wire_gemmx3h.hip
@@ -189,6 +189,20 @@
   return hipGetLastError();
 }
 
+template <int EPI>
+static hipError_t launchx3h_first(hipStream_t s, const float* A, int lda, const unsigned short* Bu, int64_t M, int Nc,
+                                  int Kd, const GemmEpiParams& ep) {
+  constexpr int E3 = EPI == EPI_GABOR2D_BWD_FIRST ? 0 : EPI_D3;
+  const int dn = ep.first_dn && ep.coords && (ep.D == 2 || (ep.D == 3 && E3)) ? ep.D : 0;
+  if (ep.cg_partial)
+    return dn == 2 ? launchx3h_t<EPI | EPI_CG | EPI_D2>(s, A, lda, Bu, M, Nc, Kd, ep)
+         : dn == 3 ? launchx3h_t<EPI | EPI_CG | E3>(s, A, lda, Bu, M, Nc, Kd, ep)
+                   : launchx3h_t<EPI | EPI_CG>(s, A, lda, Bu, M, Nc, Kd, ep);
+  return dn == 2 ? launchx3h_t<EPI | EPI_D2>(s, A, lda, Bu, M, Nc, Kd, ep)
+       : dn == 3 ? launchx3h_t<EPI | E3>(s, A, lda, Bu, M, Nc, Kd, ep)
+                 : launchx3h_t<EPI>(s, A, lda, Bu, M, Nc, Kd, ep);
+}
+
 bool gemmx3h_handles(int epi, int64_t M) {
   const int h16 = knob(K_X3_H16);
   if (!h16 || M < 4096) return false;
@@ -209,10 +223,10 @@
   switch (epi) {
     case EPI_STORE: return launchx3h_t<EPI_STORE>(s, A, lda, Bu, M, Nc, Kd, ep);
     case EPI_GABOR_FWD: return launchx3h_t<EPI_GABOR_FWD>(s, A, lda, Bu, M, Nc, Kd, ep);
-    case EPI_GABOR_BWD: return launchx3h_t<EPI_GABOR_BWD>(s, A, lda, Bu, M, Nc, Kd, ep);
-    case EPI_GABOR_BWD_FIRST:
-      return ep.cg_partial ? launchx3h_t<EPI_GABOR_BWD_FIRST | EPI_CG>(s, A, lda, Bu, M, Nc, Kd, ep)
-                           : launchx3h_t<EPI_GABOR_BWD_FIRST>(s, A, lda, Bu, M, Nc, Kd, ep);
+    case EPI_GABOR_BWD:
+      return ep.lookahead && ep.recompute_out ? launchx3h_t<EPI_GABOR_BWD | EPI_LA>(s, A, lda, Bu, M, Nc, Kd, ep)
+                          : launchx3h_t<EPI_GABOR_BWD>(s, A, lda, Bu, M, Nc, Kd, ep);
+    case EPI_GABOR_BWD_FIRST: return launchx3h_first<EPI_GABOR_BWD_FIRST>(s, A, lda, Bu, M, Nc, Kd, ep);
     case EPI_SIREN_FWD: return launchx3h_t<EPI_SIREN_FWD>(s, A, lda, Bu, M, Nc, Kd, ep);
     case EPI_GAUSS_FWD: return launchx3h_t<EPI_GAUSS_FWD>(s, A, lda, Bu, M, Nc, Kd, ep);
     case EPI_RELU_FWD: return launchx3h_t<EPI_RELU_FWD>(s, A, lda, Bu, M, Nc, Kd, ep);
@@ -235,9 +249,7 @@
       if (Nc & 127) return hipErrorInvalidValue;
       return launchx3h_t<EPI_GABOR2D_FWD>(s, A, lda, Bu, M, Nc, Kd, ep);
     case EPI_GABOR2D_BWD: return launchx3h_t<EPI_GABOR2D_BWD>(s, A, lda, Bu, M, Nc, Kd, ep);
-    case EPI_GABOR2D_BWD_FIRST:
-      return ep.cg_partial ? launchx3h_t<EPI_GABOR2D_BWD_FIRST | EPI_CG>(s, A, lda, Bu, M, Nc, Kd, ep)
-                           : launchx3h_t<EPI_GABOR2D_BWD_FIRST>(s, A, lda, Bu, M, Nc, Kd, ep);
+    case EPI_GABOR2D_BWD_FIRST: return launchx3h_first<EPI_GABOR2D_BWD_FIRST>(s, A, lda, Bu, M, Nc, Kd, ep);
     default: return hipErrorInvalidValue;
   }
 }
diff --git a/wire_amd/csrc/wire_hier_api.hip b/wire_amd/csrc/wire_hier_api.hip
--- a/wire_amd/csrc/wire_hier_api.hip
+++ b/wire_amd/csrc/wire_hier_api.hip
@@ -256,7 +256,7 @@
 Route hier_route(const Plan& p, int64_t n, RouteMode mode) {
   Route r = make_route(p, n, mode);
   r.fused_fwd = r.fuse = r.fused_train = r.fused_final = r.chain = r.rstore = r.skip_out_L = false;
-  r.first_sums = r.cg_epi = false;
+  r.first_sums = r.cg_epi = r.first_dn = r.bwd_lookahead = false;
   r.wb_l0 = p.L + 1; r.wb_n = 0;
   for (float& v : r.out_scale) v = 0.f;
   return r;
diff --git a/wire_amd/csrc/wire_knobs.h b/wire_amd/csrc/wire_knobs.h
--- a/wire_amd/csrc/wire_knobs.h
+++ b/wire_amd/csrc/wire_knobs.h
@@ -2,7 +2,7 @@
 #include <atomic>
 
 enum Knob {
-  K_COMPLEX_3M, K_SPLIT_BF16, K_SPLIT_F16, K_SPLIT_OUT, K_RECOMPUTE_OUT, K_FIRST_SUMS, K_FUSED_RSTORE, K_WGRAD_BATCH,
+  K_COMPLEX_3M, K_SPLIT_BF16, K_SPLIT_F16, K_SPLIT_OUT, K_RECOMPUTE_OUT, K_FIRST_SUMS, K_FIRST_DN, K_BWD_LOOKAHEAD, K_FUSED_RSTORE, K_WGRAD_BATCH,
   K_FUSED_FWD, K_FUSED_TRAIN, K_FUSED_TRAIN_P384, K_FUSED_FINAL, K_FUSED_BWD, K_FUSED_BWD_W,
   K_NT_BK, K_X2_AMODE, K_X2_TN_ROWS, K_X2_TN_P384, K_X3_TALL, K_X3_TALL_REAL, K_X3_TN_TALL, K_X3_TN16, K_X3_H16,
   K_X3H_STAGGER,
diff --git a/wire_amd/csrc/wire_knobs.hip b/wire_amd/csrc/wire_knobs.hip
--- a/wire_amd/csrc/wire_knobs.hip
+++ b/wire_amd/csrc/wire_knobs.hip
@@ -40,6 +40,8 @@
     flag_knob(K_SPLIT_OUT, "split_out", "WIRE_SPLIT_OUT", 1),
     flag_knob(K_RECOMPUTE_OUT, "recompute_out", "WIRE_RECOMPUTE_OUT", 1),
     flag_knob(K_FIRST_SUMS, "first_sums", "WIRE_FIRST_SUMS", 1),
+    flag_knob(K_FIRST_DN, "first_dn", "WIRE_FIRST_DN", 1),
+    flag_knob(K_BWD_LOOKAHEAD, "bwd_lookahead", "WIRE_BWD_LOOKAHEAD", 1),
     flag_knob(K_FUSED_RSTORE, "fused_rstore", "WIRE_FUSED_RSTORE", 1),
     flag_knob(K_WGRAD_BATCH, "wgrad_batch", "WIRE_WGRAD_BATCH", 1),
     range_knob(K_FUSED_FWD, "fused_fwd", "WIRE_FUSED_FWD", 1, 0, 1),
diff --git a/wire_amd/csrc/wire_mfn_api.hip b/wire_amd/csrc/wire_mfn_api.hip
--- a/wire_amd/csrc/wire_mfn_api.hip
+++ b/wire_amd/csrc/wire_mfn_api.hip
@@ -3,7 +3,7 @@
 Route mfn_route(const Plan& p, int64_t n, RouteMode mode) {
   Route r = make_route(p, n, mode);
   r.fused_fwd = r.fuse = r.fused_train = r.fused_final = r.chain = r.rstore = r.skip_out_L = false;
-  r.first_sums = r.cg_epi = r.recompute_out = r.recompute_out0 = false;
+  r.first_sums = r.cg_epi = r.first_dn = r.bwd_lookahead = r.recompute_out = r.recompute_out0 = false;
   r.wb_l0 = p.L + 1; r.wb_n = 0;
   for (float& v : r.out_scale) v = 0.f;
   return r;
diff --git a/wire_amd/csrc/wire_plan.h b/wire_amd/csrc/wire_plan.h
--- a/wire_amd/csrc/wire_plan.h
+++ b/wire_amd/csrc/wire_plan.h
@@ -75,7 +75,7 @@
   std::vector<int64_t> off_fwd, off_dg, off_bias, off_fwd_x3, off_dg_x3, off_fwd_3m, off_dg_3m, off_fwd_x2, off_dg_x2;
   int64_t off_wf, off_bf, off_first, off_wamax, total_packed;
   int64_t off_fx;
-  bool k_split_out, k_recompute_out, k_first_sums, k_rstore, k_wgrad_batch, k_fused_fwd, k_fused_train, k_fused_bwd, k_fused_final,
+  bool k_split_out, k_recompute_out, k_first_sums, k_first_dn, k_bwd_lookahead, k_rstore, k_wgrad_batch, k_fused_fwd, k_fused_train, k_fused_bwd, k_fused_final,
        k_fused_train_p384;
   int64_t off_fxd;
   std::vector<int64_t> tfloats;
@@ -166,6 +166,8 @@
   bool recompute_out0;
   bool first_sums;
   bool cg_epi;
+  bool bwd_lookahead;
+  bool first_dn;
   int wb_l0, wb_n, wb_S;
   float act_scale;
   float out_scale[65];
diff --git a/wire_amd/csrc/wire_plan.hip b/wire_amd/csrc/wire_plan.hip
--- a/wire_amd/csrc/wire_plan.hip
+++ b/wire_amd/csrc/wire_plan.hip
@@ -91,7 +91,8 @@
   p.x2 = p.x3 && knob(K_SPLIT_F16) != 0;
   p.m3 = (p.kind == WIRE_KIND_WIRE) && knob(K_COMPLEX_3M) && !p.x3;
   p.k_split_out = knob(K_SPLIT_OUT) != 0; p.k_recompute_out = knob(K_RECOMPUTE_OUT) != 0;
-  p.k_first_sums = knob(K_FIRST_SUMS) != 0; p.k_rstore = knob(K_FUSED_RSTORE) != 0; p.k_wgrad_batch = knob(K_WGRAD_BATCH) != 0;
+  p.k_first_sums = knob(K_FIRST_SUMS) != 0; p.k_first_dn = knob(K_FIRST_DN) != 0;
+  p.k_bwd_lookahead = knob(K_BWD_LOOKAHEAD) != 0; p.k_rstore = knob(K_FUSED_RSTORE) != 0; p.k_wgrad_batch = knob(K_WGRAD_BATCH) != 0;
   p.k_fused_fwd = knob(K_FUSED_FWD) != 0; p.k_fused_train = p.k_fused_fwd && knob(K_FUSED_TRAIN);
   p.k_fused_train_p384 = knob(K_FUSED_TRAIN_P384) != 0;
   p.k_fused_bwd = p.k_fused_train && knob(K_FUSED_BWD); p.k_fused_final = p.k_fused_train && knob(K_FUSED_FINAL);
@@ -356,6 +357,8 @@
   const bool h16_1 = p.x3 && gemmx3_nt_is_h16(epi1, n);
   r.cg_epi = h16_1 && !p.first_gemm && p.L >= 1 && !p.m2;
   r.first_sums = r.cg_epi && p.k_first_sums;
+  r.first_dn = h16_1 && p.cplx && p.k_first_dn;
+  r.bwd_lookahead = p.kind == WIRE_KIND_WIRE && p.x3 && gemmx3_nt_is_h16(EPI_GABOR_BWD, n) && p.k_bwd_lookahead;
   r.recompute_out0 = h16_1 && p.kind == WIRE_KIND_WIRE && p.k_recompute_out;
   r.wb_l0 = p.L + 1;
   if (r.chain && p.k_wgrad_batch) {
```

After: 46.64 million, median of 6. 1.02x the previous value.
